# MIT-SPARK/Khronos

Hardware: AMD Instinct MI355X
Metric: active-window frames/sec (+ Mvoxel-updates/sec) at 1280x720 RGB-D+labels, 2 cm voxels (higher is better)
Workload: dtype f32

## Files before the change

khronos_amd/csrc/khr_device.h:

```cpp
#pragma once
#include <hip/hip_runtime.h>
#include <stdint.h>

namespace khr {

constexpr uint64_t kEmptyKey = ~0ull;
constexpr uint32_t kInvalidSlot = 0xffffffffu;

constexpr uint32_t BLK_UPDATED = 1u, BLK_MESH_UPDATED = 2u, BLK_TRACKING_UPDATED = 4u, BLK_HAS_ACTIVE = 8u,
                   BLK_LIVE = 16u,
                   BLK_TRACK_DIRTY = 32u,
                   BLK_ANY_KEEP = 64u,
                   BLK_HAS_NEG = 128u;
constexpr uint8_t VOX_ACTIVE = 1, VOX_EVER_FREE = 2, VOX_TO_REMOVE = 4, VOX_SEM_VALID = 8;
constexpr uint8_t VOX_OCC = 16;
constexpr uint8_t VOX_PUBLIC_MASK = 0x0f;

enum Counter : int {
  C_FREE_HEAD = 0,
  C_N_FREE,
  C_MAX_SLOT,
  C_N_VISIBLE,
  C_N_NEW,
  C_N_EF,
  C_N_LIVE,
  C_POOL_EXHAUSTED,
  C_N_UPD_LO,
  C_N_REMOVED,
  C_N_SEEDS,
  C_N_MESH,
  C_N_BAND,
  C_N_TSDF,
  C_BAND_OVERFLOW,
  C_TSDF_CURSOR,
  C_MESH_OVERFLOW,
  C_N_PROC,
  C_N_EF_A,
  C_N_PROC2,
  C_N_EF2,
  C_MP_DONE,
  C_N_ITEMS0,
  C_N_ITEMS1,
  C_N_ITEMS2,
  C_N_ITEMS3,
  C_COUNT = 32
};
enum Stat64 : int { S_UPD = 0 , S_BAND , S_MESH_VERTS, S_PRUNED, S_CUM_UPD, S_CUM_BAND, S_CUM_VISITED, S_CUM_CALLS, S_COUNT = 8 };

struct MeshDesc {
  uint32_t offset;
  uint32_t count;
};

struct DevMap {
  uint64_t* ht_keys;
  uint32_t* ht_vals;
  uint32_t ht_mask;
  uint32_t capacity;
  int4* blk_index;
  uint32_t* blk_flags;
  float* dist;
  float* weight;
  uint32_t* color;
  uint64_t* last_obs;
  ulonglong2* obs;
  uint64_t* last_occ;
  uint64_t* trk_lim;
  uint8_t* vflags;
  uint32_t* sem_label;
  float* lik;
  uint64_t* freebits;
  uint16_t* blk_band;
  uint32_t* free_slots;
  uint32_t* counters;
  unsigned long long* stats;
  MeshDesc* mesh_desc;
};

constexpr int kBandSlots = 32;
constexpr uint16_t kItemTouched = 0x8000u, kItemNeg = 0x4000u, kItemBandMask = 0x3fffu;
struct FuseList {
  uint4* a;
  uint4* b;
  uint32_t cap;
  uint32_t* counts;
};
__device__ inline uint32_t fuseClass(uint32_t band) { return band > 128u ? 0u : (band > 64u ? 1u : (band > 0u ? 2u : 3u)); }
__device__ inline uint4* fuseDescPtr(const FuseList& l, uint32_t cls, uint32_t pos) {
  uint4* const arr = cls < 2u ? l.a : l.b;
  return arr + ((cls & 1u) ? l.cap - 1u - pos : pos);
}

__host__ __device__ inline int likStride(int K) { return K <= 4 ? K : ((K + 31) & ~31); }

struct DevParams {
  float vs, vs_inv, bs, bs_inv, trunc;
  int vps, nvox, K;
  int KS;
  int with_semantics, with_tracking;
  int use_dropoff, const_weight, interp, range_mode, sem_mode;
  float dropoff_eps, max_weight, adaptive_diff, log_match, log_nomatch;
  float occ_thr;
  double temporal_buffer, temporal_window;
  int nn;
  float mesh_min_weight;
  float mesh_eps;
  int mesh_attr_source;
// ... 161 lines not shown
  if (slot != kInvalidSlot && ignore_epoch != 0 && m.blk_index[slot].w == ignore_epoch) slot = kInvalidSlot;
  if (slot == kInvalidSlot) return ~0ull;
  if (m.vflags[static_cast<size_t>(slot) * p.nvox + lin] & VOX_EVER_FREE) key |= kSeedFlag;
  return key;
}

__device__ inline uint64_t lastObserved(const DevMap& m, size_t slot, uint32_t lin, int nvox) {
  const ulonglong2 w = m.obs[slot * static_cast<size_t>(nvox >> 6) + (lin >> 6)];
  return ((w.x >> (lin & 63u)) & 1ull) ? w.y : m.last_obs[slot * static_cast<size_t>(nvox) + lin];
}

__device__ inline double toSeconds(uint64_t ns) { return static_cast<double>(ns) / 1e9; }

__device__ inline uint32_t laneId() { return __lane_id(); }

__device__ inline uint32_t waveAggInc(uint32_t* counter, bool pred) {
  const unsigned long long mask = __ballot(pred);
  if (mask == 0) return 0;
  const uint32_t lane = laneId();
  const uint32_t rank = __popcll(mask & ((1ull << lane) - 1ull));
  const int leader = __ffsll(static_cast<long long>(mask)) - 1;
  uint32_t base = 0;
  if (lane == static_cast<uint32_t>(leader)) base = atomicAdd(counter, static_cast<uint32_t>(__popcll(mask)));
  base = __shfl(base, leader);
  return base + rank;
}

__device__ inline uint8_t toU8(float f) {
  float r = floorf(f + 0.5f);
  r = fminf(255.f, fmaxf(0.f, r));
  return static_cast<uint8_t>(r);
}

__device__ inline void publishSeedCount(const DevMap& m, volatile uint32_t* host_seed, uint32_t ticket) {
  host_seed[0] = atomicAdd(&m.counters[C_N_SEEDS], 0u);
  __threadfence_system();
  host_seed[1] = ticket;
  __threadfence_system();
}

constexpr int kUpdateStatSlots = 2048;

__device__ inline void beginIntegrate(DevMap m, int nvox, uint32_t* wg_stats) {
  unsigned long long u = 0, b = 0;
  uint2* __restrict__ st = reinterpret_cast<uint2*>(wg_stats);
#pragma unroll 4
  for (int i = threadIdx.x; i < kUpdateStatSlots; i += blockDim.x) {
    const uint2 v = st[i];
    u += v.x;
    b += v.y;
    if (v.x | v.y) st[i] = make_uint2(0u, 0u);
  }
#pragma unroll
  for (int o = 32; o > 0; o >>= 1) {
    u += __shfl_down(u, o);
    b += __shfl_down(b, o);
  }
  if ((threadIdx.x & 63) == 0 && (u | b)) {
    atomicAdd(&m.stats[S_CUM_UPD], u);
    atomicAdd(&m.stats[S_CUM_BAND], b);
  }
  if (threadIdx.x == 0) {
    m.stats[S_CUM_VISITED] += static_cast<unsigned long long>(m.counters[C_N_VISIBLE]) * nvox;
    m.stats[S_CUM_CALLS] += 1ull;
    m.counters[C_N_VISIBLE] = 0u;
    m.counters[C_N_NEW] = 0u;
    m.counters[C_N_TSDF] = 0u;
    m.counters[C_N_ITEMS0] = 0u;
    m.counters[C_N_ITEMS1] = 0u;
    m.counters[C_N_ITEMS2] = 0u;
    m.counters[C_N_ITEMS3] = 0u;
  }
}

__device__ inline uint32_t ufLoad(const uint32_t* parent, uint32_t x) { return __atomic_load_n(parent + x, __ATOMIC_RELAXED); }
__device__ inline uint32_t ufFind(uint32_t* parent, uint32_t x) {
  uint32_t p = ufLoad(parent, x);
  while (p != x) {
    const uint32_t gp = ufLoad(parent, p);
    if (gp != p) atomicMin(parent + x, gp);
    x = p;
    p = gp;
  }
  return x;
}
__device__ inline uint32_t ufFind(const uint32_t* parent, uint32_t x) {
  while (true) {
    const uint32_t p = ufLoad(parent, x);
    if (p == x) return x;
    x = p;
  }
}
__device__ inline void ufUnion(uint32_t* parent, uint32_t a, uint32_t b) {
  a = ufFind(parent, a);
  b = ufFind(parent, b);
  while (a != b) {
    if (a < b) { const uint32_t t = a; a = b; b = t; }
    const uint32_t old = atomicCAS(parent + a, a, b);
    if (old == a) return;
    a = ufFind(parent, old);
  }
}

}
// ... 1 lines not shown
```

khronos_amd/csrc/khr_kernels_aux.h:

```cpp
#pragma once
#include <cstring>

#include "khr_device.h"

namespace khr {

#include "mc_table.inc"
__device__ int8_t g_mc_tri[256][16];
__device__ uint8_t g_mc_ntri[256];

constexpr uint64_t kSeedBit = kSeedFlag;

__global__ __launch_bounds__(256) void k_motion_pixels(DevMap m, DevParams p, DevFrame f, float md_max_range,
                                                      float min_z_world, uint64_t* __restrict__ keys, int ignore_epoch,
                                                      uint32_t* __restrict__ begin_band_count) {
  if (begin_band_count && blockIdx.x == 0) beginIntegrate(m, p.nvox, begin_band_count);
  const int i = blockIdx.x * blockDim.x + threadIdx.x;
  const bool in = i < f.W * f.H;
  uint64_t key = ~0ull;
  if (in)
    key = motionPixelKey(m, p, f.range[i], f.depth[i], i % f.W, i / f.W, f.fx, f.fy, f.cx, f.cy, f.Rw, f.tw, md_max_range,
                         min_z_world, ignore_epoch);
  if (in) keys[i] = key;
  const bool seed = (key != ~0ull) && (key & kSeedBit);
  const int any = __syncthreads_count(seed ? 1 : 0);
  if (any && threadIdx.x == 0) atomicAdd(&m.counters[C_N_SEEDS], static_cast<uint32_t>(any));
}

__global__ __launch_bounds__(1024) void k_publish(const uint32_t* __restrict__ src, volatile uint32_t* __restrict__ dst_host,
                                                 uint32_t rec_words, uint32_t max_recs, volatile uint32_t* __restrict__ ticket_host,
                                                 uint32_t ticket, uint32_t* __restrict__ counters_to_zero) {
  const uint32_t n_words = 4u + min(src[0], max_recs) * rec_words;
  for (uint32_t i = threadIdx.x; i < n_words; i += blockDim.x) dst_host[i] = src[i];
  __threadfence_system();
  __syncthreads();
  if (threadIdx.x < 4) counters_to_zero[threadIdx.x] = 0u;
  if (threadIdx.x == 0) {
    *ticket_host = ticket;
    __threadfence_system();
  }
}

__global__ void k_publish_seed(DevMap m, volatile uint32_t* host_seed, uint32_t ticket) {
  if (blockIdx.x == 0 && threadIdx.x == 0) publishSeedCount(m, host_seed, ticket);
}

__global__ __launch_bounds__(256) void k_md_keys_export(const uint64_t* __restrict__ keys, int n, uint64_t* __restrict__ out) {
  const int i = blockIdx.x * blockDim.x + threadIdx.x;
  if (i < n) out[i] = keys[i] == ~0ull ? 0ull : keys[i];
}
__global__ __launch_bounds__(256) void k_md_keys_import(const uint64_t* __restrict__ in, int n, uint64_t* __restrict__ keys,
                                                       uint32_t* __restrict__ n_seed_px) {
  const int i = blockIdx.x * blockDim.x + threadIdx.x;
  uint64_t k = ~0ull;
  if (i < n) {
    k = in[i] == 0ull ? ~0ull : in[i];
    keys[i] = k;
  }
  const unsigned long long b = __ballot(k != ~0ull && (k & kSeedBit));
  if (b && laneId() == static_cast<uint32_t>(__ffsll(static_cast<long long>(b)) - 1))
    atomicAdd(n_seed_px, static_cast<uint32_t>(__popcll(b)));
}

__global__ __launch_bounds__(256) void k_md_bits_export(const uint64_t* __restrict__ keys, int n, unsigned long long* __restrict__ bits) {
  const int i = blockIdx.x * blockDim.x + threadIdx.x;
  const uint64_t k = i < n ? keys[i] : ~0ull;
  const unsigned long long ex = __ballot(k != ~0ull), sd = __ballot(k != ~0ull && (k & kSeedBit));
  if (laneId() == 0 && (i & ~63) < n) {
    bits[2 * (i >> 6)] = ex;
    bits[2 * (i >> 6) + 1] = sd;
  }
}
__global__ __launch_bounds__(256) void k_md_keys_from_bits(DevParams p, DevFrame f, float md_max_range, float min_z_world,
                                                          const unsigned long long* __restrict__ bits, uint64_t* __restrict__ keys,
                                                          uint32_t* __restrict__ n_seed_px) {
  const int i = blockIdx.x * blockDim.x + threadIdx.x;
  const int n = f.W * f.H;
// ... 1456 lines not shown
}

__global__ __launch_bounds__(256) void k_rehash_clear(DevMap m) {
  if (m.counters[C_N_REMOVED] == 0u) return;
  const uint32_t i = blockIdx.x * blockDim.x + threadIdx.x;
  if (i <= m.ht_mask) m.ht_keys[i] = kEmptyKey;
  if (i == 0) {
    m.counters[C_N_FREE] = 0u;
    m.counters[C_FREE_HEAD] = 0u;
  }
}

__global__ __launch_bounds__(256) void k_rehash(DevMap m) {
  if (m.counters[C_N_REMOVED] == 0u) return;
  const uint32_t s = blockIdx.x * blockDim.x + threadIdx.x;
  const bool live = s < m.counters[C_MAX_SLOT] && (m.blk_flags[s] & BLK_LIVE);
  if (live) {
    const int4 bi = m.blk_index[s];
    htInsertUnique(m, packKey(bi.x, bi.y, bi.z), s);
  }
  const bool is_free = s < m.capacity && !live;
  const uint32_t idx = waveAggInc(&m.counters[C_N_FREE], is_free);
  if (is_free) m.free_slots[idx] = s;
}

__global__ __launch_bounds__(256) void k_reset_map(DevMap m) {
  const uint32_t i = blockIdx.x * blockDim.x + threadIdx.x;
  if (i <= m.ht_mask) m.ht_keys[i] = kEmptyKey;
  if (i < m.capacity) {
    m.blk_flags[i] = 0u;
    m.mesh_desc[i] = MeshDesc{0u, 0u};
    m.free_slots[i] = i;
  }
  if (i < C_COUNT) m.counters[i] = i == C_N_FREE ? m.capacity : 0u;
  if (i < S_COUNT) m.stats[i] = 0ull;
}

__global__ __launch_bounds__(256) void k_block_flag_op(DevMap m, uint32_t and_mask, uint32_t or_mask) {
  const uint32_t s = blockIdx.x * blockDim.x + threadIdx.x;
  if (s >= m.counters[C_MAX_SLOT]) return;
  const uint32_t fl = m.blk_flags[s];
  if (fl & BLK_LIVE) m.blk_flags[s] = (fl & and_mask) | or_mask;
}

struct PackOut {
  float* dist;
  float* weight;
  uint32_t* color;
  uint64_t* last_obs;
  uint8_t* vflags;
  uint32_t* sem_label;
  uint64_t* last_occ;
  float* lik;
  int K, KS;
  uint64_t track_stamp;
};
template <int VPS>
__global__ __launch_bounds__(256) void k_pack_blocks(DevMap m, const uint32_t* __restrict__ slots, int n, PackOut o) {
  constexpr int NV = VPS * VPS * VPS;
  for (int b = blockIdx.x; b < n; b += gridDim.x) {
    const size_t src = static_cast<size_t>(slots[b]) * NV, dst = static_cast<size_t>(b) * NV;
    auto copy16 = [&](const void* s, void* d, size_t bytes) {
      const uint4* s4 = reinterpret_cast<const uint4*>(s);
      uint4* d4 = reinterpret_cast<uint4*>(d);
      for (size_t i = threadIdx.x; i < bytes / 16; i += 256) d4[i] = s4[i];
    };
    if (o.dist) copy16(m.dist + src, o.dist + dst, NV * 4);
// ... 180 lines not shown
```

khronos_amd/csrc/khr_kernels_fusion.h:

```cpp
#pragma once
#include "khr_device.h"

namespace khr {


constexpr int kTile = 16;
constexpr int kMaxTick = 8;

__device__ inline void ingestTile(const float* __restrict__ depth_in, const uint8_t* __restrict__ rgb_in,
                                  const int32_t* __restrict__ label_in, float* __restrict__ depth, float* __restrict__ range,
                                  uint32_t* __restrict__ rgba, int32_t* __restrict__ label, int32_t* __restrict__ dyn,
                                  float* __restrict__ tile_max, int tile, int tw, int W, int H, float fx, float fy, float cx,
                                  float cy, int range_mode, float* d_out, float* r_out) {
  const int tx = tile % tw, ty = tile / tw;
  const int u = tx * kTile + (threadIdx.x & 15), v = ty * kTile + (threadIdx.x >> 4);
  float r = 0.f, d = 0.f;
  if (u < W && v < H) {
    const int i = v * W + u;
    d = depth_in[i];
    if (d > 0.f && isfinite(d)) {
      if (range_mode == 0) {
        r = d;
      } else {
        const float x = (static_cast<float>(u) - cx) / fx, y = (static_cast<float>(v) - cy) / fy;
        r = d * sqrtf((x * x + y * y) + 1.f);
      }
    }
    depth[i] = d;
    range[i] = r;
    dyn[i] = 0;
    if (rgb_in)
      rgba[i] = static_cast<uint32_t>(rgb_in[3 * i]) | (static_cast<uint32_t>(rgb_in[3 * i + 1]) << 8) |
                (static_cast<uint32_t>(rgb_in[3 * i + 2]) << 16) | 0xff000000u;
    if (label_in) label[i] = label_in[i];
  }
  *d_out = d;
  *r_out = r;
  float rm = r;
#pragma unroll
  for (int o = 32; o > 0; o >>= 1) rm = fmaxf(rm, __shfl_down(rm, o));
  __shared__ float s[4];
  if ((threadIdx.x & 63) == 0) s[threadIdx.x >> 6] = rm;
  __syncthreads();
  if (threadIdx.x == 0) tile_max[tile] = fmaxf(fmaxf(s[0], s[1]), fmaxf(s[2], s[3]));
}

__global__ __launch_bounds__(256) void k_frame_ingest(const float* __restrict__ depth_in,
                                                     const uint8_t* __restrict__ rgb_in,
                                                     const int32_t* __restrict__ label_in, float* __restrict__ depth,
                                                     float* __restrict__ range, uint32_t* __restrict__ rgba,
                                                     int32_t* __restrict__ label, int32_t* __restrict__ dyn,
                                                     float* __restrict__ tile_max, int tw, int W, int H, float fx,
                                                     float fy, float cx, float cy, int range_mode, DevMap m, int nvox,
                                                     uint32_t* __restrict__ wg_stats, int do_begin) {
  if (blockIdx.x == 0 && threadIdx.x == 0) m.counters[C_N_SEEDS] = 0u;
  if (do_begin && blockIdx.x == 0) beginIntegrate(m, nvox, wg_stats);
  float d, r;
  ingestTile(depth_in, rgb_in, label_in, depth, range, rgba, label, dyn, tile_max, blockIdx.x, tw, W, H, fx, fy, cx, cy,
             range_mode, &d, &r);
}

struct TickIngest {
  const float* depth_in[kMaxTick];
  const uint8_t* rgb_in[kMaxTick];
  const int32_t* label_in[kMaxTick];
  float* depth[kMaxTick];
  float* range[kMaxTick];
  uint32_t* rgba[kMaxTick];
  int32_t* label[kMaxTick];
  int32_t* dyn[kMaxTick];
  float* tile_max[kMaxTick];
  float Rw[kMaxTick][9], tw[kMaxTick][3], min_z_world[kMaxTick];
};
__global__ __launch_bounds__(256) void k_tick_ingest(TickIngest t, int tw, int W, int H, float fx, float fy, float cx, float cy,
                                                    int range_mode, DevMap m, DevParams p, float md_max_range, int count_seeds,
                                                    uint32_t* __restrict__ seed_counts) {
  const int cam = blockIdx.y;
  if (blockIdx.x == 0 && cam == 0 && threadIdx.x == 0) m.counters[C_N_SEEDS] = 0u;
  float d, r;
  ingestTile(t.depth_in[cam], t.rgb_in[cam], t.label_in[cam], t.depth[cam], t.range[cam], t.rgba[cam], t.label[cam], t.dyn[cam],
             t.tile_max[cam], blockIdx.x, tw, W, H, fx, fy, cx, cy, range_mode, &d, &r);
  if (!count_seeds) return;
  const int u = (blockIdx.x % tw) * kTile + (threadIdx.x & 15), v = (blockIdx.x / tw) * kTile + (threadIdx.x >> 4);
  bool seed = false;
  if (u < W && v < H) {
    const uint64_t key = motionPixelKey(m, p, r, d, u, v, fx, fy, cx, cy, t.Rw[cam], t.tw[cam], md_max_range, t.min_z_world[cam]);
    seed = key != ~0ull && (key & kSeedFlag);
  }
  const unsigned long long b = __ballot(seed);
// ... 66 lines not shown
    dst[i] = depth[i];
    dst[n4 + i] = range[i];
    dst[2 * n4 + i] = rgba ? rgba[i] : z;
    dst[3 * n4 + i] = label ? label[i] : z;
  }
}
__global__ __launch_bounds__(256) void k_rgba_to_rgb(const uint32_t* __restrict__ rgba, uint8_t* __restrict__ rgb, uint32_t n) {
  const uint32_t i = blockIdx.x * blockDim.x + threadIdx.x;
  if (i >= n) return;
  const uint32_t c = rgba[i];
  rgb[3 * i] = static_cast<uint8_t>(c);
  rgb[3 * i + 1] = static_cast<uint8_t>(c >> 8);
  rgb[3 * i + 2] = static_cast<uint8_t>(c >> 16);
}

__global__ __launch_bounds__(256) void k_vertex_map(DevFrame f, float* __restrict__ vertex) {
  const int i = blockIdx.x * blockDim.x + threadIdx.x;
  if (i >= f.W * f.H) return;
  float o[3] = {0.f, 0.f, 0.f};
  if (f.range[i] > 0.f) {
    const float d = f.depth[i];
    const int u = i % f.W, v = i / f.W;
    const float x = ((static_cast<float>(u) - f.cx) / f.fx) * d;
    const float y = ((static_cast<float>(v) - f.cy) / f.fy) * d;
    xform(f.Rw, f.tw, x, y, d, o);
  }
  vertex[3 * i] = o[0];
  vertex[3 * i + 1] = o[1];
  vertex[3 * i + 2] = o[2];
}

__global__ __launch_bounds__(256) void k_alloc_visible(DevMap m, DevParams p, DevFrame f, DevFrustum fr,
                                                      uint32_t* __restrict__ work, uint32_t* __restrict__ new_list,
                                                      volatile uint32_t* host_seed, uint32_t seed_ticket,
                                                      uint32_t* __restrict__ list_count, int epoch) {
  if (seed_ticket && blockIdx.x == 0 && threadIdx.x == 0) publishSeedCount(m, host_seed, seed_ticket);
  const int S = 2 * fr.n_steps + 1;
  const int total = S * S * S;
  const int i = blockIdx.x * blockDim.x + threadIdx.x;
  bool visible = false;
  int bx = 0, by = 0, bz = 0;
  if (i < total) {
    const int dx = i % S - fr.n_steps, dy = (i / S) % S - fr.n_steps, dz = i / (S * S) - fr.n_steps;
    bx = fr.bc.x + dx;
    by = fr.bc.y + dy;
    bz = fr.bc.z + dz;
    const bool in = blockIsCandidate(p, fr, f.R, f.t, f.max_range, bx, by, bz);
    visible = in && ownerOf(bx, by, bz, p.world) == p.rank;
  }
  uint32_t slot = kInvalidSlot;
  const uint64_t key = packKey(bx, by, bz);
  if (visible) slot = htLookup(m, key);
  const bool need = visible && slot == kInvalidSlot;
  const uint32_t fidx = waveAggInc(&m.counters[C_FREE_HEAD], need);
  bool got = false;
  if (need) {
    if (fidx < m.counters[C_N_FREE]) {
      slot = m.free_slots[fidx];
      got = true;
      m.blk_index[slot] = make_int4(bx, by, bz, epoch);
      m.blk_flags[slot] = BLK_LIVE | BLK_TRACK_DIRTY | BLK_ANY_KEEP;
      m.mesh_desc[slot] = MeshDesc{0u, 0u};
      htInsertUnique(m, key, slot);
      atomicMax(&m.counters[C_MAX_SLOT], slot + 1);
    } else {
      atomicAdd(&m.counters[C_POOL_EXHAUSTED], 1u);
      slot = kInvalidSlot;
    }
  }
  const uint32_t nidx = waveAggInc(&m.counters[C_N_NEW], got);
  if (got) new_list[nidx] = slot;
  const bool emit = visible && slot != kInvalidSlot;
  const uint32_t widx = waveAggInc(list_count, emit);
  if (emit) work[widx] = slot;
  if (list_count != &m.counters[C_N_VISIBLE]) waveAggInc(&m.counters[C_N_VISIBLE], emit);
}

struct TickFrusta {
  float R[kMaxTick][9], t[kMaxTick][3], max_range[kMaxTick];
  DevFrustum fr[kMaxTick];
};
constexpr int kTickAllocThreads = 1024;
__global__ __launch_bounds__(kTickAllocThreads) void k_tick_alloc(DevMap m, DevParams p, TickFrusta tf, int ncam, int3 lo, int3 dim,
                                                   uint32_t* __restrict__ work, uint32_t list_stride,
                                                   uint32_t* __restrict__ new_list, uint32_t* __restrict__ tick_counts, int epoch) {
  const int total = dim.x * dim.y * dim.z;
  const int i = blockIdx.x * blockDim.x + threadIdx.x;
  uint32_t seen = 0u;
  int bx = 0, by = 0, bz = 0;
  if (i < total) {
    bx = lo.x + i % dim.x;
    by = lo.y + (i / dim.x) % dim.y;
    bz = lo.z + i / (dim.x * dim.y);
    if (ownerOf(bx, by, bz, p.world) == p.rank) {
      for (int k = 0; k < ncam; ++k) {
        const DevFrustum& fr = tf.fr[k];
        if (abs(bx - fr.bc.x) > fr.n_steps || abs(by - fr.bc.y) > fr.n_steps || abs(bz - fr.bc.z) > fr.n_steps) continue;
        const bool in = blockIsCandidate(p, fr, tf.R[k], tf.t[k], tf.max_range[k], bx, by, bz);
        if (in) seen |= 1u << k;
      }
    }
  }
  const bool visible = seen != 0u;
  uint32_t slot = kInvalidSlot;
  const uint64_t key = packKey(bx, by, bz);
  if (visible) slot = htLookup(m, key);
  const bool need = visible && slot == kInvalidSlot;
  const uint32_t fidx = waveAggInc(&m.counters[C_FREE_HEAD], need);
  bool got = false;
  if (need) {
    if (fidx < m.counters[C_N_FREE]) {
      slot = m.free_slots[fidx];
      got = true;
      m.blk_index[slot] = make_int4(bx, by, bz, epoch);
      m.blk_flags[slot] = BLK_LIVE | BLK_TRACK_DIRTY | BLK_ANY_KEEP;
      m.mesh_desc[slot] = MeshDesc{0u, 0u};
      htInsertUnique(m, key, slot);
      atomicMax(&m.counters[C_MAX_SLOT], slot + 1);
    } else {
      atomicAdd(&m.counters[C_POOL_EXHAUSTED], 1u);
      slot = kInvalidSlot;
    }
  }
  const uint32_t nidx = waveAggInc(&m.counters[C_N_NEW], got);
  if (got) new_list[nidx] = slot;
  if (slot == kInvalidSlot) seen = 0u;
  __shared__ uint32_t s_cnt[kMaxTick], s_base[kMaxTick];
  if (threadIdx.x < kMaxTick) s_cnt[threadIdx.x] = 0u;
  __syncthreads();
  uint32_t loff[kMaxTick];
#pragma unroll
  for (int k = 0; k < kMaxTick; ++k) {
    loff[k] = 0u;
    if (k < ncam) loff[k] = waveAggInc(&s_cnt[k], ((seen >> k) & 1u) != 0u);
  }
  __syncthreads();
  if (threadIdx.x < static_cast<uint32_t>(ncam)) {
    const uint32_t n = s_cnt[threadIdx.x];
    s_base[threadIdx.x] = n ? atomicAdd(&tick_counts[2 * threadIdx.x], n) : 0u;
  }
  if (threadIdx.x == 64) {
    uint32_t tot = 0u;
    for (int k = 0; k < ncam; ++k) tot += s_cnt[k];
    if (tot) atomicAdd(&m.counters[C_N_VISIBLE], tot);
  }
  __syncthreads();
#pragma unroll
  for (int k = 0; k < kMaxTick; ++k)
    if (k < ncam && ((seen >> k) & 1u)) work[static_cast<size_t>(k) * list_stride + s_base[k] + loff[k]] = slot;
}

__global__ void k_begin_integrate(DevMap m, int nvox, uint32_t* wg_stats) {
  if (blockIdx.x == 0) beginIntegrate(m, nvox, wg_stats);
}
__global__ void k_tick_begin(DevMap m, int nvox, uint32_t* wg_stats, uint32_t* tick_counts, uint32_t extra_calls) {
  beginIntegrate(m, nvox, wg_stats);
  if (threadIdx.x < 6 * kMaxTick) tick_counts[threadIdx.x] = 0u;
  if (threadIdx.x == 0) m.stats[S_CUM_CALLS] += extra_calls;
}

__device__ inline void cullBlocks(const DevMap& m, const DevParams& p, const DevFrame& f, const uint32_t* __restrict__ work,
                                  const uint32_t* __restrict__ n_work, FuseList out, uint32_t wpb,
                                  uint32_t* __restrict__ n_tsdf, const float* __restrict__ tile_max, int tw, int th,
                                  uint32_t bid, uint32_t nblk, uint32_t* __restrict__ item_mask = nullptr, uint32_t cam = 0u) {
  constexpr int kPerWg = 8;
  __shared__ uint4 s_blk[kPerWg];
  __shared__ uint16_t s_item[4][kPerWg * kBandSlots];
  __shared__ uint32_t s_nkeep, s_ccnt[4], s_off[4];
  const uint32_t n = *n_work;
  const uint32_t lane = threadIdx.x & 63;
  for (uint32_t base = bid * kPerWg; base < n; base += nblk * kPerWg) {
  if (threadIdx.x == 0) s_nkeep = 0;
  if (threadIdx.x < 4) s_ccnt[threadIdx.x] = 0;
  __syncthreads();
  for (uint32_t wi = base + (threadIdx.x >> 6); wi < min(n, base + kPerWg); wi += 4) {
    const uint32_t slot = work[wi];
    const int4 bi = m.blk_index[slot];
// ... 102 lines not shown
      }
      if (ikeep && sub == 0 && item_mask) {
        const size_t mi = static_cast<size_t>(slot) * wpb + item;
        const uint32_t sh = 8u * static_cast<uint32_t>(mi & 3);
        const uint32_t old = atomicOr(&item_mask[mi >> 2], (1u << cam) << sh);
        if ((old >> sh) & 0xffu) ikeep = false;
      }
      if (ikeep && sub == 0) {
        const uint32_t cls = fuseClass(m.blk_band[static_cast<size_t>(slot) * kBandSlots + item] & kItemBandMask);
        s_item[cls][atomicAdd(&s_ccnt[cls], 1u)] = static_cast<uint16_t>((kslot << 8) | item);
      }
    }
  }
  __syncthreads();
  if (threadIdx.x < 4) s_off[threadIdx.x] = s_ccnt[threadIdx.x] ? atomicAdd(&out.counts[threadIdx.x], s_ccnt[threadIdx.x]) : 0u;
  if (threadIdx.x == 0 && s_nkeep) atomicAdd(n_tsdf, s_nkeep);
  __syncthreads();
#pragma unroll
  for (uint32_t cls = 0; cls < 4; ++cls) {
    for (uint32_t i = threadIdx.x; i < s_ccnt[cls]; i += blockDim.x) {
      const uint32_t it = s_item[cls][i];
      uint4 d = s_blk[it >> 8];
      d.x |= (it & 0xffu) << 24;
      *fuseDescPtr(out, cls, s_off[cls] + i) = d;
    }
  }
  __syncthreads();
  }
}

__global__ __launch_bounds__(256) void k_cull_blocks(DevMap m, DevParams p, DevFrame f,
                                                    const uint32_t* __restrict__ work, FuseList out, uint32_t wpb,
                                                    const float* __restrict__ tile_max, int tw, int th) {
  cullBlocks(m, p, f, work, &m.counters[C_N_VISIBLE], out, wpb, &m.counters[C_N_TSDF], tile_max, tw, th, blockIdx.x, gridDim.x);
}

struct TickFrames {
  DevFrame f[kMaxTick];
  const float* tile_max[kMaxTick];
};
__global__ __launch_bounds__(256) void k_tick_cull(DevMap m, DevParams p, TickFrames t, const uint32_t* __restrict__ work,
                                                  uint32_t list_stride, uint4* __restrict__ desc, uint32_t desc_stride, uint32_t wpb,
                                                  uint32_t* __restrict__ tick_counts, int use_tiles, int tw, int th,
                                                  uint32_t* __restrict__ item_mask) {
  const int cam = blockIdx.y;
  const int lc = item_mask ? 0 : cam;
  FuseList out{desc + static_cast<size_t>(2 * lc) * desc_stride, desc + static_cast<size_t>(2 * lc + 1) * desc_stride, desc_stride,
               &tick_counts[2 * kMaxTick + 4 * lc]};
  cullBlocks(m, p, t.f[cam], work + static_cast<size_t>(cam) * list_stride, &tick_counts[2 * cam], out, wpb, &tick_counts[2 * cam + 1],
             use_tiles ? t.tile_max[cam] : nullptr, tw, th, blockIdx.x, gridDim.x, item_mask, static_cast<uint32_t>(cam));
}

__global__ __launch_bounds__(256) void k_alloc_list(DevMap m, const int* __restrict__ idx, int n,
                                                   uint32_t* __restrict__ new_list) {
  const int i = blockIdx.x * blockDim.x + threadIdx.x;
  bool need = false;
  int bx = 0, by = 0, bz = 0;
  if (i < n) {
    bx = idx[3 * i];
    by = idx[3 * i + 1];
    bz = idx[3 * i + 2];
    need = htLookup(m, packKey(bx, by, bz)) == kInvalidSlot;
  }
  const uint32_t fidx = waveAggInc(&m.counters[C_FREE_HEAD], need);
  bool got = false;
  uint32_t slot = kInvalidSlot;
  if (need) {
    if (fidx < m.counters[C_N_FREE]) {
      slot = m.free_slots[fidx];
      got = true;
      m.blk_index[slot] = make_int4(bx, by, bz, 0);
      m.blk_flags[slot] = BLK_LIVE | BLK_TRACK_DIRTY | BLK_ANY_KEEP;
      m.mesh_desc[slot] = MeshDesc{0u, 0u};
      htInsertUnique(m, packKey(bx, by, bz), slot);
      atomicMax(&m.counters[C_MAX_SLOT], slot + 1);
    } else {
      atomicAdd(&m.counters[C_POOL_EXHAUSTED], 1u);
    }
  }
  const uint32_t nidx = waveAggInc(&m.counters[C_N_NEW], got);
  if (got) new_list[nidx] = slot;
}

__global__ __launch_bounds__(256) void k_list_live(DevMap m, uint32_t* __restrict__ work, uint32_t* counter,
                                                  uint32_t require_flags, FuseList out = FuseList{nullptr, nullptr, 0u, nullptr},
                                                  uint32_t wpb = 0u) {
  const uint32_t s = blockIdx.x * blockDim.x + threadIdx.x;
  bool live = false;
  if (s < m.counters[C_MAX_SLOT]) {
    const uint32_t fl = m.blk_flags[s];
    live = (fl & BLK_LIVE) && ((fl & require_flags) == require_flags);
  }
  const uint32_t idx = waveAggInc(counter, live);
  if (live) work[idx] = s;
  if (out.a) {
    const unsigned long long mask = __ballot(live);
    if (mask) {
      const uint32_t lane = laneId();
      const int leader = __ffsll(static_cast<long long>(mask)) - 1;
      uint32_t base = 0;
      if (lane == static_cast<uint32_t>(leader)) base = atomicAdd(&out.counts[3], static_cast<uint32_t>(__popcll(mask)) * wpb);
      base = __shfl(base, leader) + static_cast<uint32_t>(__popcll(mask & ((1ull << lane) - 1ull))) * wpb;
      if (live) {
        const int4 bi = m.blk_index[s];
        for (uint32_t it = 0; it < wpb; ++it)
          *fuseDescPtr(out, 3u, base + it) =
              make_uint4(s | (it << 24), static_cast<uint32_t>(bi.x), static_cast<uint32_t>(bi.y), static_cast<uint32_t>(bi.z));
      }
    }
  }
}

__device__ inline void initBlocks(const DevMap& m, const DevParams& p, const uint32_t* __restrict__ new_list, uint32_t bid,
                                  uint32_t nblk) {
  const uint32_t n = m.counters[C_N_NEW];
  const int nv = p.nvox;
  for (uint32_t b = bid; b < n; b += nblk) {
    const size_t slot = new_list[b];
    const uint4 z = make_uint4(0, 0, 0, 0);
    uint4* d4 = reinterpret_cast<uint4*>(m.dist + slot * nv);
    uint4* w4 = reinterpret_cast<uint4*>(m.weight + slot * nv);
    uint4* c4 = reinterpret_cast<uint4*>(m.color + slot * nv);
    uint4* l4 = reinterpret_cast<uint4*>(m.sem_label + slot * nv);
    for (int i = threadIdx.x; i < nv / 4; i += blockDim.x) {
      d4[i] = z;
      w4[i] = z;
      c4[i] = z;
      if (p.with_semantics) l4[i] = z;
    }
    uint4* f4 = reinterpret_cast<uint4*>(m.vflags + slot * nv);
    for (int i = threadIdx.x; i < nv / 16; i += blockDim.x) f4[i] = z;
    if (threadIdx.x < kBandSlots) m.blk_band[slot * kBandSlots + threadIdx.x] = 0;
    if (p.with_tracking) {
      uint4* o4 = reinterpret_cast<uint4*>(m.last_obs + slot * nv);
      uint4* q4 = reinterpret_cast<uint4*>(m.last_occ + slot * nv);
      for (int i = threadIdx.x; i < nv / 2; i += blockDim.x) {
        o4[i] = z;
        q4[i] = z;
      }
      uint64_t* fb = m.freebits + slot * (nv / 64);
      for (int i = threadIdx.x; i < nv / 64; i += blockDim.x) {
        fb[i] = 0ull;
        m.obs[slot * (nv / 64) + i] = make_ulonglong2(0ull, 0ull);
      }
    }
  }
}

__global__ __launch_bounds__(256) void k_init_blocks(DevMap m, DevParams p, const uint32_t* __restrict__ new_list) {
  initBlocks(m, p, new_list, blockIdx.x, gridDim.x);
}

__global__ __launch_bounds__(256) void k_init_cull(DevMap m, DevParams p, DevFrame f, const uint32_t* __restrict__ new_list,
                                                  const uint32_t* __restrict__ work, FuseList out, uint32_t wpb,
                                                  const float* __restrict__ tile_max, int tw, int th, uint32_t n_cull) {
  if (blockIdx.x < n_cull)
    cullBlocks(m, p, f, work, &m.counters[C_N_VISIBLE], out, wpb, &m.counters[C_N_TSDF], tile_max, tw, th, blockIdx.x, n_cull);
  else
    initBlocks(m, p, new_list, blockIdx.x - n_cull, gridDim.x - n_cull);
}

__device__ inline uint32_t foldItemRecords(uint32_t* __restrict__ blk_flags, uint16_t* __restrict__ blk_band, uint32_t s) {
  static_assert(kBandSlots == 32, "record row = 4 x 16 bytes");
  uint4* const row = reinterpret_cast<uint4*>(blk_band + static_cast<size_t>(s) * kBandSlots);
  uint32_t any = 0u;
  uint4 r[4];
#pragma unroll
  for (int i = 0; i < 4; ++i) {
    r[i] = row[i];
    any |= r[i].x | r[i].y | r[i].z | r[i].w;
  }
  const uint32_t tm = static_cast<uint32_t>(kItemTouched) * 0x00010001u, nm = static_cast<uint32_t>(kItemNeg) * 0x00010001u;
  uint32_t fl = blk_flags[s];
  if ((any & tm) == 0u) return fl;
  fl |= BLK_UPDATED | BLK_MESH_UPDATED | BLK_TRACKING_UPDATED | ((any & nm) ? BLK_HAS_NEG : 0u);
  blk_flags[s] = fl;
  const uint32_t keep = static_cast<uint32_t>(kItemBandMask) * 0x00010001u;
#pragma unroll
  for (int i = 0; i < 4; ++i) row[i] = make_uint4(r[i].x & keep, r[i].y & keep, r[i].z & keep, r[i].w & keep);
  return fl;
}
__global__ __launch_bounds__(256) void k_tracking_select(DevMap m, uint64_t lim_active, uint64_t lim_free, int force_full,
                                                        uint32_t* __restrict__ proc, uint32_t* __restrict__ ef_list,
                                                        uint32_t* __restrict__ cnt ,
                                                        uint32_t* __restrict__ cnt_next, uint16_t* __restrict__ fold_band) {
  const uint32_t s = blockIdx.x * blockDim.x + threadIdx.x;
  if (s == 0) { cnt_next[0] = 0u; cnt_next[1] = 0u; }
  bool need = false, touched = false, reload = false;
  if (s < m.counters[C_MAX_SLOT]) {
    const uint32_t fl = fold_band ? foldItemRecords(m.blk_flags, fold_band, s) : m.blk_flags[s];
// ... 163 lines not shown

__constant__ int8_t c_nbr26[26][3] = {
    {-1, 0, 0}, {1, 0, 0}, {0, -1, 0}, {0, 1, 0}, {0, 0, -1}, {0, 0, 1},
    {-1, -1, 0}, {-1, 1, 0}, {1, -1, 0}, {1, 1, 0}, {-1, 0, -1}, {-1, 0, 1}, {1, 0, -1}, {1, 0, 1},
    {0, -1, -1}, {0, -1, 1}, {0, 1, -1}, {0, 1, 1},
    {-1, -1, -1}, {-1, -1, 1}, {-1, 1, -1}, {-1, 1, 1}, {1, -1, -1}, {1, -1, 1}, {1, 1, -1}, {1, 1, 1}};

constexpr int kHaloRecWords = 66;

struct RemoteHalo {
  const uint64_t* recs;
  const uint64_t* ht_keys;
  const uint32_t* ht_vals;
  uint32_t ht_mask;
};

template <int VPS>
__global__ __launch_bounds__(256) void k_ever_free(DevMap m, DevParams p, const uint32_t* __restrict__ ef_list,
                                                  const uint32_t* __restrict__ ef_count, RemoteHalo rh) {
  constexpr int NV = VPS * VPS * VPS;
  constexpr int NW = NV / 64;
  constexpr int T = VPS + 2;
  __shared__ uint32_t s_row[T * T];
  __shared__ uint64_t s_bits[27][NW];
  __shared__ const uint64_t* s_src[27];
  const uint32_t n = *ef_count;
  for (uint32_t b = blockIdx.x; b < n; b += gridDim.x) {
    const size_t slot = ef_list[b];
    const int4 bi = m.blk_index[slot];
    __syncthreads();
    if (threadIdx.x < 27) {
      const int dx = threadIdx.x % 3 - 1, dy = (threadIdx.x / 3) % 3 - 1, dz = threadIdx.x / 9 - 1;
      const uint64_t key = packKey(bi.x + dx, bi.y + dy, bi.z + dz);
      const uint32_t ns = (threadIdx.x == 13) ? static_cast<uint32_t>(slot) : htLookup(m, key);
      const uint64_t* src = nullptr;
      if (ns != kInvalidSlot) {
        src = m.freebits + static_cast<size_t>(ns) * NW;
      } else if (rh.recs) {
        uint32_t h = hashKey(key) & rh.ht_mask;
        while (true) {
          const uint64_t k = rh.ht_keys[h];
          if (k == key) {
            src = rh.recs + static_cast<size_t>(rh.ht_vals[h]) * kHaloRecWords + 2;
            break;
          }
          if (k == kEmptyKey) break;
          h = (h + 1) & rh.ht_mask;
        }
      }
      s_src[threadIdx.x] = src;
    }
    __syncthreads();
    for (int i = threadIdx.x; i < 27 * NW; i += 256) {
      const uint64_t* src = s_src[i / NW];
      s_bits[i / NW][i % NW] = src ? src[i % NW] : 0ull;
    }
    __syncthreads();
    for (int r = threadIdx.x; r < T * T; r += 256) {
      const int ty = r % T, tz = r / T;
      int y = ty - 1, z = tz - 1, sy = 1, sz = 1;
      if (y < 0) { y += VPS; sy = 0; } else if (y >= VPS) { y -= VPS; sy = 2; }
      if (z < 0) { z += VPS; sz = 0; } else if (z >= VPS) { z -= VPS; sz = 2; }
      const int lin0 = VPS * (y + VPS * z);
      const uint32_t mid = static_cast<uint32_t>((s_bits[1 + 3 * sy + 9 * sz][lin0 >> 6] >> (lin0 & 63)) & ((1u << VPS) - 1u));
      const uint32_t left = static_cast<uint32_t>((s_bits[0 + 3 * sy + 9 * sz][(lin0 + VPS - 1) >> 6] >> ((lin0 + VPS - 1) & 63)) & 1u);
      const uint32_t right = static_cast<uint32_t>((s_bits[2 + 3 * sy + 9 * sz][lin0 >> 6] >> (lin0 & 63)) & 1u);
      s_row[r] = left | (mid << 1) | (right << (VPS + 1));
// ... 90 lines not shown
```

khronos_amd/csrc/khronos_amd.hip:

```cpp
#include <hip/hip_runtime.h>
#include <hip/hip_ext.h>
#include <hipcub/hipcub.hpp>

#include <algorithm>
#include <array>
#include <atomic>
#include <chrono>
#include <memory>
#include <mutex>
#include <cmath>
#include <cstdarg>
#include <cstdio>
#include <climits>
#include <cstring>
#include <cstdlib>
#include <functional>
#include <map>
#include <string>
#include <thread>
#include <tuple>
#include <unordered_map>
#include <vector>

#include "../../include/khronos_amd.h"
// ... 59 lines not shown
  uint64_t aux_seq = 0;
  std::vector<khr_cluster> sem_clusters;
  std::vector<khr_cluster> clusters;
};

struct TimingRec {
  int which;
  hipEvent_t a, b;
};

constexpr int kNumTimers = 13;
constexpr uint32_t kObjHead = 512;
constexpr uint32_t kCvHead = 8192;
constexpr uint32_t kCompCap = 1024, kCompHead = 64;

}

struct khr_ctx {
  khr_config cfg{};
  DevParams p{};
  DevMap m{};
  int device = 0;
  hipStream_t stream = nullptr;
  bool own_stream = false;
  hipStream_t aux_stream = nullptr;
  hipEvent_t ev_aux = nullptr, ev_aux_done = nullptr;
  uint64_t aux_seq_issued = 0, aux_seq_done = 0, obj_seq = 0, cv_seq[2] = {0, 0};
  std::vector<void*> allocs;
  std::vector<FrameSlot> slots;
  int next_slot = 0;
  std::unique_ptr<std::atomic<int>[]> slot_leases;
  uint32_t* d_work = nullptr;
  uint32_t* d_new = nullptr;
  uint32_t* d_ef = nullptr;
  uint32_t* d_trk_proc = nullptr;
  uint32_t* d_tick_work = nullptr;
  uint32_t* d_tick_counts = nullptr;
  uint32_t* d_tick_seeds = nullptr;
  uint32_t* h_tick = nullptr;
  uint32_t* d_tick_host = nullptr;
  uint32_t tick_ticket = 0;
  std::vector<uint32_t> tick_seed_host;
  int tick_seed_n = 0, tick_seed_collected = 0;
  int tick_epoch = 0, motion_ignore_epoch = 0;
  unsigned long long* d_dbg = nullptr;
  unsigned long long* d_digest = nullptr;
  uint32_t* d_wg_stats = nullptr;
  bool defer_fold = false, fold_pending = false;
  int stream_priority = 0;
  unsigned char* d_fuse_sink = nullptr;
  uint32_t* d_pix_scratch = nullptr;
  size_t pix_words = 0;
  uint8_t* d_inst = nullptr;
  size_t inst_bytes = 0;
  uint4* d_work4 = nullptr;
  uint4* d_tick_work4 = nullptr;
  FuseFrame* d_tick_frames = nullptr;
  uint32_t* d_tick_mask = nullptr;
  bool tick_mask_dirty = false;
  uint32_t item_cap = 0;
  struct SnapArena { uint8_t* ptr; size_t bytes; volatile uint32_t* h_count; uint32_t* d_count_host_view; };
  struct SnapPool {
    std::mutex mu;
    std::vector<SnapArena> free;
    bool dead = false;
  };
// ... 11 lines not shown
  hipEvent_t ev_snap_fork = nullptr, ev_snap_join = nullptr;
  hipStream_t mc_stream = nullptr;
  hipEvent_t ev_mc_fork = nullptr, ev_mc_join = nullptr;
  bool fork_after_select = false;
  uint64_t explicit_blocks = 0;
  uint4* d_multi_list = nullptr;
  uint32_t* d_frame_bits = nullptr;
  size_t frame_bits_words = 0;
  FuseFrame* h_frames = nullptr;
  FuseFrame* d_frames = nullptr;
  hipEvent_t ev_frames = nullptr;
  uint32_t snap_ticket = 0;
  uint32_t wpb = 0;
  int fuse_zsplit = 2;
  uint64_t* d_halo_recs = nullptr;
  const uint64_t* halo_view = nullptr;
  uint64_t* d_halo_keys = nullptr;
  uint32_t* d_halo_vals = nullptr;
  uint32_t halo_cap_total = 0, halo_recs_cap = 0, halo_mask = 0, halo_n = 0;
  uint32_t* d_mh_recs = nullptr;
  const uint32_t* mh_view = nullptr;
  uint64_t* d_mh_keys = nullptr;
  uint32_t* d_mh_vals = nullptr;
  uint32_t mh_cap_total = 0, mh_mask = 0, mh_n = 0;
  uint8_t* d_mh_flag = nullptr;
  uint32_t* d_mh2_scratch = nullptr;
  uint64_t* d_mh2_keys = nullptr;
  uint32_t* d_mh2_offs = nullptr;
  uint32_t mh2_ht = 0;
  bool mh_compact = false;
  uint32_t* h_pinned = nullptr;
  uint32_t* d_pinned = nullptr;
  uint32_t seed_ticket = 0;
  bool seed_publish_pending = false;
  bool seed_by_ticket = false;
  bool begin_in_ingest = false, begun = false;
  uint32_t fetch_ticket = 0;
  bool fetch_pending = false;
  uint32_t* d_fetch_done = nullptr;
  std::vector<uint32_t> fm_order;
  size_t fm_total = 0;
  uint64_t map_gen = 1, counters_gen = 0;
  int last_frame_slot = -1;
  void* h_stage = nullptr;
  size_t h_stage_bytes = 0;
  uint32_t* h_totals = nullptr;
  void* h_up = nullptr;
  size_t h_up_bytes = 0;
  hipEvent_t ev_ingest = nullptr;
  hipEvent_t ev_up = nullptr;
  hipStream_t ingest_stream = nullptr;
  struct AheadEntry { int slot; int ev; bool host; };
  std::vector<AheadEntry> ahead_q;
  hipEvent_t ev_ahead[2] = {nullptr, nullptr};
  hipEvent_t ev_ahead_h2d[2] = {nullptr, nullptr};
  int ahead_ev_next = 0;
  hipEvent_t* h2d_ev_target = nullptr;
  hipStream_t h2d_stream = nullptr;
  hipEvent_t ev_h2d = nullptr;
  bool h2d_pending = false;
  bool host_input_pinned = false;
  uint64_t h2d_bytes = 0;
  int ef_parity = 0, ef_cur = 0;
  hipEvent_t ev_seed = nullptr;
  uint32_t last_removed = 0;
  khr_ctx* dep_src = nullptr;
  hipEvent_t ev_dep = nullptr, ev_dep_aux = nullptr;
  uint64_t last_track_stamp = 0;
  bool removed_pending = false;
// ... 92 lines not shown
  uint32_t* d_slice_count = nullptr;
  uint8_t* d_slice_stage = nullptr;
  uint8_t* h_slice_stage = nullptr;
  uint32_t slice_cap = 0, slice_hint = 0;
  unsigned long long* d_render_stats = nullptr;
  uint8_t* d_render_stage = nullptr;
  uint8_t* h_render_stage = nullptr;
  size_t render_stage_bytes = 0;
  unsigned long long* d_query_stats = nullptr;
  uint8_t* d_query_stage = nullptr;
  uint8_t* h_query_stage = nullptr;
  size_t query_stage_bytes = 0;
  uint8_t* d_ckpt[2] = {nullptr, nullptr};
  uint8_t* h_ckpt[2] = {nullptr, nullptr};
  size_t ckpt_stage_bytes = 0;
  uint32_t* d_ckpt_slots[2] = {nullptr, nullptr};
  uint32_t ckpt_slots_cap = 0;
  uint32_t* d_ckpt_err = nullptr;
  hipEvent_t ev_ckpt_filled[2] = {nullptr, nullptr}, ev_ckpt_drained[2] = {nullptr, nullptr};
  uint32_t timing = 0;
  std::vector<TimingRec> pending;
  std::vector<hipEvent_t> event_pool;
  double t_ms[kNumTimers] = {0};
  uint64_t t_n[kNumTimers] = {0};
};

namespace {

struct ScopedTimer {
  khr_ctx* c;
  int which;
  hipEvent_t a = nullptr, b = nullptr;
  bool on = false;
  ScopedTimer(khr_ctx* ctx, int w) : c(ctx), which(w) {
    on = w >= 0 && ((c->timing >> w) & 1u);
    if (on) {
      auto get = [&]() {
        hipEvent_t e = nullptr;
        if (!c->event_pool.empty()) {
          e = c->event_pool.back();
          c->event_pool.pop_back();
        } else {
          hipEventCreate(&e);
        }
        return e;
      };
      a = get();
      b = get();
      hipEventRecord(a, c->stream);
    }
  }
  ~ScopedTimer() {
    if (on) {
      hipEventRecord(b, c->stream);
      c->pending.push_back({which, a, b});
    }
  }
};

hipEvent_t takeEvent(khr_ctx* c) {
  hipEvent_t e = nullptr;
  if (!c->event_pool.empty()) {
    e = c->event_pool.back();
    c->event_pool.pop_back();
  } else {
    hipEventCreate(&e);
  }
  return e;
}
#define KHR_LAUNCH_TIMED_ON(which, strm, kernel, grid, block, ...)                                     \
  do {                                                                                                 \
    if ((c->timing >> (which)) & 1u) {                                                                 \
      hipEvent_t ev_a = takeEvent(c), ev_b = takeEvent(c);                                             \
      hipExtLaunchKernelGGL(kernel, grid, block, 0, strm, ev_a, ev_b, 0, __VA_ARGS__);                 \
      c->pending.push_back({(which), ev_a, ev_b});                                                     \
    } else {                                                                                           \
      hipLaunchKernelGGL(kernel, grid, block, 0, strm, __VA_ARGS__);                                   \
    }                                                                                                  \
  } while (0)
#define KHR_LAUNCH_TIMED(which, kernel, grid, block, ...) KHR_LAUNCH_TIMED_ON(which, c->stream, kernel, grid, block, __VA_ARGS__)

void resolveTimers(khr_ctx* c) {
  for (auto& r : c->pending) {
    hipEventSynchronize(r.b);
    float ms = 0.f;
    hipEventElapsedTime(&ms, r.a, r.b);
    if (r.which >= 0) {
// ... 76 lines not shown
  return f;
}

DevFrustum makeFrustum(const khr_ctx* c, const DevFrame& f) {
  DevFrustum fr{};
  const float xl = (0.f - f.cx) / f.fx, xr = (static_cast<float>(f.W) - f.cx) / f.fx;
  const float yt = (0.f - f.cy) / f.fy, yb = (static_cast<float>(f.H) - f.cy) / f.fy;
  const float tl[3] = {xl, yt, 1.f}, tr[3] = {xr, yt, 1.f}, bl[3] = {xl, yb, 1.f}, br[3] = {xr, yb, 1.f};
  crossn(bl, tl, fr.n[0]);
  crossn(tr, br, fr.n[1]);
  crossn(tl, tr, fr.n[2]);
  crossn(br, bl, fr.n[3]);
  fr.infl = 0.8660254f * c->p.bs;
  fr.n_steps = static_cast<int>(std::ceil(f.max_range * c->p.bs_inv)) + 1;
  fr.max_steps = static_cast<int>(std::floor((f.max_range + fr.infl) * c->p.bs_inv));
  for (int a = 0; a < 3; ++a) fr.tw[a] = f.tw[a];
  fr.bc = make_int3(static_cast<int>(std::floor(f.tw[0] * c->p.bs_inv)),
                    static_cast<int>(std::floor(f.tw[1] * c->p.bs_inv)),
                    static_cast<int>(std::floor(f.tw[2] * c->p.bs_inv)));
  return fr;
}

int ensureStage(khr_ctx* c, size_t bytes) {
  if (bytes <= c->h_stage_bytes) return KHR_OK;
  if (c->h_stage) HIP_TRY(hipHostFree(c->h_stage));
  c->h_stage = nullptr;
  c->h_stage_bytes = 0;
  const size_t want = std::max<size_t>(bytes + bytes / 2, 1u << 20);
  if (hipHostMalloc(&c->h_stage, want, hipHostMallocDefault) != hipSuccess) return fail(KHR_ENOMEM, "pinned staging of %zu bytes", want);
  c->h_stage_bytes = want;
  return KHR_OK;
}

int readCounters(khr_ctx* c) {
  c->h_counters.resize(C_COUNT);
  HIP_TRY(hipMemcpyAsync(c->h_counters.data(), c->m.counters, sizeof(uint32_t) * C_COUNT, hipMemcpyDeviceToHost,
                         c->stream));
  HIP_TRY(hipStreamSynchronize(c->stream));
  return KHR_OK;
}

int ensureHostIndex(khr_ctx* c) {
  if (c->host_index_valid) return KHR_OK;
  int rc = readCounters(c);
  if (rc) return rc;
  const uint32_t n = c->h_counters[C_MAX_SLOT];
  std::vector<int4> idx(n);
  c->host_flags.resize(n);
  if (n) {
    HIP_TRY(hipMemcpyAsync(idx.data(), c->m.blk_index, sizeof(int4) * n, hipMemcpyDeviceToHost, c->stream));
    HIP_TRY(hipMemcpyAsync(c->host_flags.data(), c->m.blk_flags, sizeof(uint32_t) * n, hipMemcpyDeviceToHost,
                           c->stream));
    HIP_TRY(hipStreamSynchronize(c->stream));
  }
  c->host_index.clear();
  for (uint32_t s = 0; s < n; ++s)
    if (c->host_flags[s] & BLK_LIVE) c->host_index[{idx[s].x, idx[s].y, idx[s].z}] = s;
  c->host_index_valid = true;
  return KHR_OK;
}

inline int gridFor(size_t n, int block = 256) { return static_cast<int>((n + block - 1) / block); }

template <typename F>
int dispatchVps(khr_ctx* c, F&& f) {
  if (c->cfg.voxels_per_side == 16) return f(std::integral_constant<int, 16>());
  if (c->cfg.voxels_per_side == 8) return f(std::integral_constant<int, 8>());
  return fail(KHR_EINVAL, "voxels_per_side must be 8 or 16");
}

constexpr int kUpdateWavesPerCu = 16;
// ... 270 lines not shown
  p.rank = cfg->rank;
  p.world = cfg->world_size;
  p.dbg = std::getenv("KHR_DEBUG") ? std::atoi(std::getenv("KHR_DEBUG")) : 0;

  DevMap& m = c->m;
  const size_t cap = cfg->max_blocks, nv = p.nvox;
  uint32_t ht = 1;
  while (ht < cap * 4) ht <<= 1;
  m.ht_mask = ht - 1;
  m.capacity = static_cast<uint32_t>(cap);
  int rc = KHR_OK;
  auto A = [&](int r) { if (rc == KHR_OK) rc = r; };
  A(devAlloc(c, &m.ht_keys, ht, false));
  A(devAlloc(c, &m.ht_vals, ht));
  A(devAlloc(c, &m.blk_index, cap));
  A(devAlloc(c, &m.blk_flags, cap));
  A(devAlloc(c, &m.dist, cap * nv, false));
  A(devAlloc(c, &m.weight, cap * nv, false));
  A(devAlloc(c, &m.color, cap * nv, false));
  A(devAlloc(c, &m.vflags, cap * nv, false));
  A(devAlloc(c, &m.sem_label, cfg->with_semantics ? cap * nv : 1, false));
  if (devAlloc(c, &m.lik, cfg->with_semantics ? cap * nv * p.KS : 1, false) != KHR_OK) {
    fail(KHR_ENOMEM, "the label-likelihood layer of %zu blocks needs %.2f GB (%d floats per voxel%s); khr_config.packed_likelihood_rows = 1 "
                     "stores %d per voxel, a smaller max_blocks less of everything", static_cast<size_t>(cap),
         1e-9 * static_cast<double>(cap) * nv * p.KS * 4, p.KS, p.KS != p.K ? ": rows padded to 128-byte lines" : "", p.K);
    A(KHR_ENOMEM);
  }
  A(devAlloc(c, &m.last_obs, cfg->with_tracking ? cap * nv : 1, false));
  A(devAlloc(c, &m.last_occ, cfg->with_tracking ? cap * nv : 1, false));
  A(devAlloc(c, &m.trk_lim, cfg->with_tracking ? cap * 2 : 2));
  A(devAlloc(c, &m.freebits, cfg->with_tracking ? cap * (nv / 64) : 1, false));
  A(devAlloc(c, &m.obs, cfg->with_tracking ? cap * (nv / 64) : 1, false));
  A(devAlloc(c, &m.free_slots, cap, false));
  A(devAlloc(c, &m.counters, C_COUNT));
  A(devAlloc(c, &m.stats, S_COUNT));
  A(devAlloc(c, &m.mesh_desc, cap));
  A(devAlloc(c, &c->d_work, cap));
  A(devAlloc(c, &c->d_new, cap));
  A(devAlloc(c, &c->d_ef, cap));
  A(devAlloc(c, &c->d_trk_proc, cap));
  A(devAlloc(c, &c->d_dbg, 4096 * 4 * 12));
  A(devAlloc(c, &c->d_digest, kDigestWords));
  A(devAlloc(c, &c->d_wg_stats, 2 * kUpdateStatSlots));
  A(devAlloc(c, &c->d_fuse_sink, static_cast<size_t>(kUpdateStatSlots) * 16 * 256, false));
  A(devAlloc(c, &c->d_fetch_done, 4));
  {
    const int zs = (cfg->voxels_per_side != 8 && (cfg->world_size >= 4 || cfg->max_frame_pixels <= 640u * 480u)) ? 8 : 4;
    c->fuse_zsplit = zs;
    c->wpb = static_cast<uint32_t>((cfg->voxels_per_side * cfg->voxels_per_side / 64) * zs);
    c->item_cap = static_cast<uint32_t>(cap) * c->wpb;
  }
  A(devAlloc(c, &c->d_work4, 2 * static_cast<size_t>(c->item_cap), false));
  if (cfg->voxels_per_side == 8 && rc == KHR_OK) {
    const size_t bits_words = static_cast<size_t>(c->item_cap) * 4;
    if (hipHostMalloc(reinterpret_cast<void**>(&c->h_frames), sizeof(FuseFrame) * kMaxMultiFrames, hipHostMallocDefault) != hipSuccess ||
        hipMalloc(reinterpret_cast<void**>(&c->d_frames), sizeof(FuseFrame) * kMaxMultiFrames) != hipSuccess ||
        hipEventCreateWithFlags(&c->ev_frames, hipEventDisableTiming) != hipSuccess ||
        hipEventRecord(c->ev_frames, c->stream) != hipSuccess ||
        hipMalloc(reinterpret_cast<void**>(&c->d_frame_bits), bits_words * sizeof(uint32_t)) != hipSuccess ||
        hipMalloc(reinterpret_cast<void**>(&c->d_multi_list), sizeof(uint4) * 2 * c->item_cap + 16) != hipSuccess)
      rc = fail(KHR_ENOMEM, "buffers of the multi-frame update");
    else
      c->frame_bits_words = bits_words;
    if (rc == KHR_OK && (hipHostMalloc(reinterpret_cast<void**>(&c->h_totals), sizeof(uint32_t) * (C_COUNT + 2), hipHostMallocDefault) != hipSuccess ||
                         hipEventCreateWithFlags(&c->ev_up, hipEventDisableTiming) != hipSuccess || hipEventRecord(c->ev_up, c->stream) != hipSuccess ||
                         hipEventCreateWithFlags(&c->ev_dep, hipEventDisableTiming) != hipSuccess ||
                         hipEventCreateWithFlags(&c->ev_dep_aux, hipEventDisableTiming) != hipSuccess))
      rc = fail(KHR_ENOMEM, "page-locked words / events of an object mini-map");
  }
  A(devAlloc(c, &m.blk_band, cap * kBandSlots));
  A(devAlloc(c, &c->d_removed, cap));
  A(devAlloc(c, &c->d_mesh_count, cap + 1));
  A(devAlloc(c, &c->d_mesh_offset, cap + 1));
  A(devAlloc(c, &c->d_regen, cap));
  A(devAlloc(c, &c->d_mesh_old_off, cap + 1));
  A(devAlloc(c, &c->d_mh_flag, cap));
  A(devAlloc(c, &c->d_mesh_nwork, 8));
  const size_t npx = cfg->max_frame_pixels;
  A(devAlloc(c, &c->d_keys, npx, false));
  A(devAlloc(c, &c->d_pix, npx, false));
  {
    uint32_t ts = 1;
    while (ts < 2 * npx) ts <<= 1;
    c->md_mask = ts - 1;
    c->md_list_cap = static_cast<uint32_t>(std::min<size_t>(npx, 1u << 20));
    A(devAlloc(c, &c->d_md_keys, 3 * static_cast<size_t>(ts), false));
    A(devAlloc(c, &c->d_md_counts, 3 * static_cast<size_t>(ts), false));
    A(devAlloc(c, &c->d_md_ids, 3 * static_cast<size_t>(ts), false));
    {
      uint8_t* head = nullptr;
      A(devAlloc(c, &head, 16 + sizeof(CompAcc) * kCompCap));
      c->d_md_n = reinterpret_cast<uint32_t*>(head);
    }
    A(devAlloc(c, &c->d_md_parent, c->md_list_cap, false));
    A(devAlloc(c, &c->d_md_rootidx, c->md_list_cap, false));
    A(devAlloc(c, &c->d_md_edges, c->md_list_cap, false));
    A(devAlloc(c, &c->d_md_comp_acc, c->md_list_cap, false));
// ... 159 lines not shown
    c->snap_pool->free.clear();
  }
  {
    std::lock_guard<std::mutex> lock(c->frame_pool->mu);
    c->frame_pool->dead = true;
    for (auto& b : c->frame_pool->free) hipFree(b.first);
    c->frame_pool->free.clear();
  }
  if (c->d_frame_bits) hipFree(c->d_frame_bits);
  if (c->d_multi_list) hipFree(c->d_multi_list);
  if (c->h_frames) hipHostFree(c->h_frames);
  if (c->d_frames) hipFree(c->d_frames);
  if (c->ev_frames) hipEventDestroy(c->ev_frames);
  if (c->h_pinned) hipHostFree(c->h_pinned);
  if (c->h_removed_early) hipHostFree(c->h_removed_early);
  if (c->h_stage) hipHostFree(c->h_stage);
  if (c->h_totals) hipHostFree(c->h_totals);
  if (c->h_up) hipHostFree(c->h_up);
  if (c->ev_up) hipEventDestroy(c->ev_up);
  if (c->ev_ingest) hipEventDestroy(c->ev_ingest);
  if (c->h_tick) hipHostFree(c->h_tick);
  if (c->h_obj_head) hipHostFree(c->h_obj_head);
  if (c->h_md_acc_pinned) hipHostFree(c->h_md_acc_pinned);
  if (c->ev_obj) hipEventDestroy(c->ev_obj);
  for (int w = 0; w < 2; ++w) {
    if (c->h_cv[w]) hipHostFree(c->h_cv[w]);
    if (c->ev_cv[w]) hipEventDestroy(c->ev_cv[w]);
  }
  if (c->ev_seed) hipEventDestroy(c->ev_seed);
  if (c->ev_dep) hipEventDestroy(c->ev_dep);
  if (c->ev_dep_aux) hipEventDestroy(c->ev_dep_aux);
  if (c->ev_aux) hipEventDestroy(c->ev_aux);
  if (c->ev_aux_done) hipEventDestroy(c->ev_aux_done);
  if (c->aux_stream) hipStreamDestroy(c->aux_stream);
  if (c->own_stream && c->stream) hipStreamDestroy(c->stream);
  delete c;
}

int khr_set_stream(khr_ctx* c, void* hip_stream) {
  if (!c) return fail(KHR_EINVAL, "null ctx");
  HIP_TRY(hipStreamSynchronize(c->stream));
  HIP_TRY(hipStreamSynchronize(c->aux_stream));
  if (c->own_stream) {
    hipStreamDestroy(c->stream);
    c->own_stream = false;
  }
  if (hip_stream) {
    c->stream = static_cast<hipStream_t>(hip_stream);
  } else {
    HIP_TRY(createStream(c, &c->stream));
    c->own_stream = true;
  }
  return KHR_OK;
}

int khr_sync(khr_ctx* c) {
  if (!c) return fail(KHR_EINVAL, "null ctx");
  HIP_TRY(hipStreamSynchronize(c->stream));
  HIP_TRY(hipStreamSynchronize(c->aux_stream));
  return KHR_OK;
}

static int auxAfterMain(khr_ctx* c) {
  HIP_TRY(hipEventRecord(c->ev_aux, c->stream));
  HIP_TRY(hipStreamWaitEvent(c->aux_stream, c->ev_aux, 0));
  return KHR_OK;
// ... 63 lines not shown
    if (pinned) {
      if (!c->h2d_stream) HIP_TRY(createStream(c, &c->h2d_stream));
      hipEvent_t& evh0 = c->h2d_ev_target ? *c->h2d_ev_target : c->ev_h2d;
      if (!evh0) HIP_TRY(hipEventCreateWithFlags(&evh0, hipEventDisableTiming));
      cs = c->h2d_stream;
      if (ist == c->stream) {
        if (!c->ev_ingest) HIP_TRY(hipEventCreateWithFlags(&c->ev_ingest, hipEventDisableTiming));
        HIP_TRY(hipEventRecord(c->ev_ingest, c->stream));
        HIP_TRY(hipStreamWaitEvent(cs, c->ev_ingest, 0));
      }
    }
    HIP_TRY(hipMemcpyAsync(s.depth, frame->depth, n * sizeof(float), kind, cs));
    depth_src = s.depth;
    if (frame->color) {
      HIP_TRY(hipMemcpyAsync(s.rgb_staging, frame->color, n * 3, kind, cs));
      rgb_src = s.rgb_staging;
    }
    if (frame->label) {
      HIP_TRY(hipMemcpyAsync(s.label, frame->label, n * sizeof(int32_t), kind, cs));
      label_src = s.label;
    }
    if (pinned) {
      hipEvent_t& evh = c->h2d_ev_target ? *c->h2d_ev_target : c->ev_h2d;
      HIP_TRY(hipEventRecord(evh, cs));
      HIP_TRY(hipStreamWaitEvent(ist, evh, 0));
      if (!c->h2d_ev_target) c->h2d_pending = true;
      c->h2d_bytes += n * (4u + (frame->color ? 3u : 0u) + (frame->label ? 4u : 0u));
    }
  }
  s.tw = (sensor->width + kTile - 1) / kTile;
  s.th = (sensor->height + kTile - 1) / kTile;
  hipLaunchKernelGGL(k_frame_ingest, dim3(s.tw * s.th), dim3(256), 0, ist, depth_src, rgb_src, label_src, s.depth,
                     s.range, s.rgba, s.label, s.dyn, s.tile_max, s.tw, sensor->width, sensor->height, sensor->fx, sensor->fy,
                     sensor->cx, sensor->cy, c->p.range_mode, c->m, c->p.nvox, c->d_wg_stats, c->begin_in_ingest ? 1 : 0);
  HIP_TRY(hipGetLastError());
  c->begun = c->begin_in_ingest;
  c->begin_in_ingest = false;
  if (!on_device && !pinned) HIP_TRY(hipStreamSynchronize(c->stream));
  s.valid = true;
  s.dyn_clean = true, s.dynw_valid = false;
  return slot;
}

int khr_set_frame_image(khr_ctx* c, int slot, int which, const int32_t* image, int on_device) {
  if (!c || slot < 0 || slot >= static_cast<int>(c->slots.size()) || !c->slots[slot].valid) return fail(KHR_EINVAL, "bad slot");
  FrameSlot& s = c->slots[slot];
  const size_t n = static_cast<size_t>(s.sensor.width) * s.sensor.height;
  int32_t* dst = which == 0 ? s.dyn : s.obj;
  if (image) {
    HIP_TRY(hipMemcpyAsync(dst, image, n * sizeof(int32_t), on_device ? hipMemcpyDeviceToDevice : hipMemcpyHostToDevice, c->stream));
    if (!on_device) HIP_TRY(hipStreamSynchronize(c->stream));
  } else {
    HIP_TRY(hipMemsetAsync(dst, 0, n * sizeof(int32_t), c->stream));
  }
  if (which == 1) s.has_obj = image != nullptr;
  if (which == 0) s.dyn_clean = image == nullptr;
  if (which == 0) s.dynw_valid = false;
  if (which == 1) {
    const int rca = auxAfterMain(c);
    if (rca) return rca;
  }
  return KHR_OK;
}

int khr_download_frame(khr_ctx* c, int slot, float* range, float* vertex_map, int32_t* dynamic_image) {
  if (!c || slot < 0 || slot >= static_cast<int>(c->slots.size()) || !c->slots[slot].valid) return fail(KHR_EINVAL, "bad slot");
  FrameSlot& s = c->slots[slot];
  const size_t n = static_cast<size_t>(s.sensor.width) * s.sensor.height;
  if (range) HIP_TRY(hipMemcpyAsync(range, s.vRange(), n * sizeof(float), hipMemcpyDeviceToHost, c->stream));
// ... 111 lines not shown
int khr_copy_frame_image(khr_ctx* c, int slot, int which, void* device_dst) {
  if (!c || !device_dst || slot < 0 || slot >= static_cast<int>(c->slots.size()) || !c->slots[slot].valid) return fail(KHR_EINVAL, "bad argument");
  if (which != 0 && which != 1) return fail(KHR_EINVAL, "which must be 0 (dynamic) or 1 (object)");
  HIP_TRY(hipSetDevice(c->device));
  FrameSlot& s = c->slots[slot];
  const size_t n = static_cast<size_t>(s.sensor.width) * s.sensor.height;
  if (which == 1 && !s.has_obj) {
    HIP_TRY(hipMemsetAsync(device_dst, 0, n * sizeof(int32_t), c->stream));
    return KHR_OK;
  }
  if (which == 1) {
    HIP_TRY(hipEventRecord(c->ev_aux_done, c->aux_stream));
    HIP_TRY(hipStreamWaitEvent(c->stream, c->ev_aux_done, 0));
  }
  HIP_TRY(hipMemcpyAsync(device_dst, which == 0 ? s.dyn : s.obj, n * sizeof(int32_t), hipMemcpyDeviceToDevice, c->stream));
  return KHR_OK;
}

int khr_download_frame_image(khr_ctx* c, int slot, int which, int32_t* image) {
  if (!c || !image || slot < 0 || slot >= static_cast<int>(c->slots.size()) || !c->slots[slot].valid) return fail(KHR_EINVAL, "bad argument");
  if (which != 0 && which != 1) return fail(KHR_EINVAL, "which must be 0 (dynamic) or 1 (object)");
  FrameSlot& s = c->slots[slot];
  const size_t n = static_cast<size_t>(s.sensor.width) * s.sensor.height;
  if (which == 1 && !s.has_obj) {
    std::memset(image, 0, n * sizeof(int32_t));
    return KHR_OK;
  }
  if (which == 1) HIP_TRY(hipStreamSynchronize(c->aux_stream));
  HIP_TRY(hipMemcpyAsync(image, which == 0 ? s.dyn : s.obj, n * sizeof(int32_t), hipMemcpyDeviceToHost, c->stream));
  HIP_TRY(hipStreamSynchronize(c->stream));
  return KHR_OK;
}

static int integrateAlloc(khr_ctx* c, FrameSlot& s, const DevFrame& f, int allocate_blocks) {
  DevMap& m = c->m;
  if (!c->begun) hipLaunchKernelGGL(k_begin_integrate, dim3(1), dim3(256), 0, c->stream, m, c->p.nvox, c->d_wg_stats);
  c->begun = false;
  if (allocate_blocks) {
    ScopedTimer tm(c, 3);
    const DevFrustum fr = makeFrustum(c, f);
    const int S = 2 * fr.n_steps + 1;
    const size_t total = static_cast<size_t>(S) * S * S;
    hipLaunchKernelGGL(k_alloc_visible, dim3(gridFor(total)), dim3(256), 0, c->stream, m, c->p, f, fr, c->d_work, c->d_new,
                       c->d_pinned + 2, c->seed_publish_pending ? c->seed_ticket : 0u, &m.counters[C_N_VISIBLE], 0);
    c->seed_publish_pending = false;
    hipLaunchKernelGGL(k_init_cull, dim3(1024 + 1024), dim3(256), 0, c->stream, m, c->p, f, c->d_new, c->d_work,
                       FuseList{c->d_work4, c->d_work4 + c->item_cap, c->item_cap, &m.counters[C_N_ITEMS0]}, c->wpb,
                       c->cfg.disable_culling ? nullptr : s.vTileMax(), s.tw, s.th, 1024u);
    c->host_index_valid = false, ++c->map_gen;
  } else {
    hipLaunchKernelGGL(k_list_live, dim3(gridFor(m.capacity)), dim3(256), 0, c->stream, m, c->d_work,
                       &m.counters[C_N_VISIBLE], 0u, FuseList{c->d_work4, c->d_work4 + c->item_cap, c->item_cap, &m.counters[C_N_ITEMS0]},
                       c->wpb);
  }
  HIP_TRY(hipGetLastError());
  return KHR_OK;
}

struct UpdateLists {
  FuseList list{nullptr, nullptr, 0u, nullptr};
};

static int fuseGrid(khr_ctx* c, const void* kernel, int group, int block) {
  static std::map<std::pair<int, const void*>, int> cache;
  static std::mutex cache_mu;
  std::lock_guard<std::mutex> lock(cache_mu);
  const std::pair<int, const void*> key{c->device, kernel};
  auto it = cache.find(key);
  if (it != cache.end()) return it->second;
  int per_cu = 0, cus = 256;
  if (hipOccupancyMaxActiveBlocksPerMultiprocessor(&per_cu, kernel, block, 0) != hipSuccess || per_cu < 1) per_cu = 1;
  per_cu = std::min(per_cu, std::max(1, kUpdateWavesPerCu / (block / 64)));
  hipDeviceProp_t prop;
  if (hipGetDeviceProperties(&prop, c->device) == hipSuccess && prop.multiProcessorCount > 0) cus = prop.multiProcessorCount;
  per_cu = std::min(per_cu, 8);
  int grid = std::min(kUpdateStatSlots, per_cu * cus);
  grid = std::max(8 * group, grid / (8 * group) * (8 * group));
  cache[key] = grid;
  return grid;
}

static int fuse2Grid(khr_ctx* c, const void* kern, int wpw) {
  static std::map<std::pair<int, const void*>, int> cache;
  static std::mutex mu;
  std::lock_guard<std::mutex> lock(mu);
// ... 61 lines not shown
  {
    void* hf_dev = nullptr;
    HIP_TRY(hipHostGetDevicePointer(&hf_dev, c->h_frames, 0));
    const uint32_t n_words = static_cast<uint32_t>(sizeof(FuseFrame) / 4) * static_cast<uint32_t>(n_frames);
    hipLaunchKernelGGL(k_copy_words, dim3((n_words + 255) / 256), dim3(256), 0, c->stream, static_cast<const uint32_t*>(hf_dev),
                       reinterpret_cast<uint32_t*>(c->d_frames), n_words);
  }
  HIP_TRY(hipEventRecord(c->ev_frames, c->stream));
  static_cast<FuseFrame&>(a) = c->h_frames[0];
  a.frames = c->d_frames;
  a.n_frames = n_frames;
  if (c->item_cap > 0) {
    const int n_words = (n_frames + 31) / 32;
    const size_t need = static_cast<size_t>(c->item_cap) * static_cast<size_t>(n_words);
    if (need > c->frame_bits_words) {
      const size_t want = static_cast<size_t>(c->item_cap) * static_cast<size_t>((n_words + 3) / 4 * 4);
      HIP_TRY(hipStreamSynchronize(c->stream));
      if (c->d_frame_bits) HIP_TRY(hipFree(c->d_frame_bits));
      c->d_frame_bits = nullptr;
      c->frame_bits_words = 0;
      if (hipMalloc(reinterpret_cast<void**>(&c->d_frame_bits), want * sizeof(uint32_t)) != hipSuccess)
        return fail(KHR_ENOMEM, "frame bits of the multi-frame update (%zu bytes)", want * sizeof(uint32_t));
      c->frame_bits_words = want;
    }
    const uint64_t tests = static_cast<uint64_t>(c->explicit_blocks > 0 ? std::min<uint64_t>(c->explicit_blocks, c->m.capacity) : c->m.capacity) *
                           c->wpb * static_cast<uint64_t>(n_words) * 32u;
    const unsigned grid = static_cast<unsigned>(std::min<uint64_t>((tests + 255) / 256, 8192));
    hipLaunchKernelGGL((k_multi_cull<8>), dim3(std::max(1u, grid)), dim3(256), 0, c->stream, c->m.blk_flags, c->m.blk_index, &c->m.counters[C_MAX_SLOT],
                       c->p.vs, c->p.bs, c->p.trunc, static_cast<const FuseFrame*>(c->d_frames), n_frames, n_words, c->wpb, BLK_LIVE, c->d_frame_bits);
    HIP_TRY(hipGetLastError());
    a.frame_bits = c->d_frame_bits;
    a.frame_words = n_words;
  }
  FuseList list{c->d_work4, c->d_work4 + c->item_cap, c->item_cap, &c->m.counters[C_N_ITEMS0]};
  if (a.frame_bits != nullptr) {
    if (!c->d_multi_list) {
      HIP_TRY(hipStreamSynchronize(c->stream));
      if (hipMalloc(reinterpret_cast<void**>(&c->d_multi_list), sizeof(uint4) * 2 * c->item_cap + 16) != hipSuccess)
        return fail(KHR_ENOMEM, "item list of the multi-frame update");
    }
    uint32_t* const counts = reinterpret_cast<uint32_t*>(c->d_multi_list + 2 * static_cast<size_t>(c->item_cap));
    HIP_TRY(hipMemsetAsync(counts, 0, 16, c->stream));
    list = FuseList{c->d_multi_list, c->d_multi_list + c->item_cap, c->item_cap, counts};
    const uint64_t n_it = static_cast<uint64_t>(c->explicit_blocks > 0 ? std::min<uint64_t>(c->explicit_blocks, c->m.capacity) : c->m.capacity) * c->wpb;
    hipLaunchKernelGGL(k_multi_order, dim3(static_cast<unsigned>((n_it + 1023) / 1024)), dim3(1024), 0, c->stream, c->m.blk_flags, c->m.blk_index,
                       &c->m.counters[C_MAX_SLOT], static_cast<const uint32_t*>(c->d_frame_bits), a.frame_words, n_frames, c->wpb, BLK_LIVE, list);
    HIP_TRY(hipGetLastError());
  }
  constexpr int WPW = 8;
  auto go = [&](auto kern) {
    static std::map<std::pair<int, const void*>, std::pair<int, int>> per_cu_of;
    static std::mutex per_cu_mu;
    int per_cu = 0, cus = 256;
    {
      std::lock_guard<std::mutex> lock(per_cu_mu);
      const std::pair<int, const void*> key{c->device, reinterpret_cast<const void*>(kern)};
      auto it = per_cu_of.find(key);
      if (it != per_cu_of.end()) {
        per_cu = it->second.first;
        cus = it->second.second;
      } else {
        if (hipOccupancyMaxActiveBlocksPerMultiprocessor(&per_cu, kern, 64 * WPW, 0) != hipSuccess || per_cu < 1) per_cu = 1;
        hipDeviceProp_t prop;
        if (hipGetDeviceProperties(&prop, c->device) == hipSuccess && prop.multiProcessorCount > 0) cus = prop.multiProcessorCount;
        per_cu_of[key] = {per_cu, cus};
      }
    }
    int grid = std::min(kUpdateStatSlots, per_cu * cus) / 8 * 8;
    if (c->explicit_blocks > 0) {
      const uint64_t items = c->explicit_blocks * c->wpb;
      grid = std::max(8, static_cast<int>(std::min<uint64_t>(static_cast<uint64_t>(grid), (items + WPW - 1) / WPW) + 7) / 8 * 8);
    }
    for (int k0 = 0; k0 < n_frames; k0 += kMultiChunk) {
      a.frames = c->d_frames + k0;
      a.n_frames = std::min(kMultiChunk, n_frames - k0);
      a.frame_bit0 = k0;
      KHR_LAUNCH_TIMED(0, kern, dim3(grid), dim3(64 * WPW), a, list);
    }
  };
  if (exactArithmetic(c)) go(&k_fuse2<8, 4, true, true, WPW, 4>);
  else go(&k_fuse2<8, 4, true, false, WPW, 4>);
  HIP_TRY(hipGetLastError());
  return KHR_OK;
}

static int integrateUpdate(khr_ctx* c, FrameSlot& s, const DevFrame& f, int allocate_blocks, int use_mask,
                           int object_id, const UpdateLists* lists = nullptr, const uint32_t* gate = nullptr) {
  DevMap& m = c->m;
  FuseList list{c->d_work4, c->d_work4 + c->item_cap, c->item_cap, &m.counters[C_N_ITEMS0]};
  if (lists) list = lists->list;
  FuseArgs a{};
  fillFuseMap(c, &a);
  fillFuseFrame(c, s, f, use_mask, object_id, &a);
  const bool defcfg = a.range_mode == 0 && a.interp == 2 && a.use_dropoff && !a.const_weight;
  const bool exact = exactArithmetic(c);
  int rc = dispatchVps(c, [&](auto vps) {
    constexpr int V = decltype(vps)::value;
    auto launch = [&](auto zsplit) {
      constexpr int ZS = decltype(zsplit)::value;
      constexpr int G = 1;
      auto go = [&](auto kern, int wpw) {
        int grid = fuseGrid(c, reinterpret_cast<const void*>(kern), G, 64 * wpw);
        if (!allocate_blocks && c->explicit_blocks > 0) {
          const uint64_t items = c->explicit_blocks * c->wpb;
          const int want = static_cast<int>(std::min<uint64_t>(static_cast<uint64_t>(grid), (items + wpw - 1) / wpw));
          grid = std::max(8, (want + 7) / 8 * 8);
        }
        static bool said = false;
        if (!said && std::getenv("KHR_VERBOSE")) { said = true; std::fprintf(stderr, "[khr] k_fuse<%d,%d> %d waves / workgroup, grid %d\n", V, ZS, wpw, grid); }
        KHR_LAUNCH_TIMED(0, kern, dim3(grid), dim3(64 * wpw), a, list);
        if (c->defer_fold) c->fold_pending = true;
        else hipLaunchKernelGGL(k_fuse_fold, dim3((c->m.capacity + 255) / 256), dim3(256), 0, c->stream, m.blk_flags, m.blk_band,
                                &m.counters[C_MAX_SLOT], gate);
      };
      a.gate = gate;
      constexpr int WD = kUpdateWpw;
      if (defcfg && !exact) {
        go(&k_fuse<V, ZS, true, false, WD>, WD);
      } else if (defcfg) {
        go(&k_fuse<V, ZS, true, true, WD>, WD);
      } else {
        go(&k_fuse<V, ZS, false, true, WD>, WD);
// ... 446 lines not shown
  HIP_TRY(hipGetLastError());
  return KHR_OK;
}

int khr_tick_integrate(khr_ctx* c, const int* slots, int n_frames, int use_mask, int object_id, int phases) {
  if (!c || !slots || n_frames < 1 || (phases & 15) == 0) return fail(KHR_EINVAL, "bad argument");
  if (phases & 1) phases |= 12;
  if ((phases & 14) != 14 && n_frames > kMaxTick) return fail(KHR_EINVAL, "split phases take at most %d frames", kMaxTick);
  for (int i = 0; i < n_frames; ++i) {
    if (slots[i] < 0 || slots[i] >= static_cast<int>(c->slots.size()) || !c->slots[slots[i]].valid) return fail(KHR_EINVAL, "bad slot");
    const khr_sensor &a = c->slots[slots[i]].sensor, &b = c->slots[slots[0]].sensor;
    if (a.width != b.width || a.height != b.height) return fail(KHR_EINVAL, "the frames of a tick must come from sensors of one image size");
  }
  HIP_TRY(hipSetDevice(c->device));
  int rc = ensureTick(c);
  if (rc) return rc;
  DevMap& m = c->m;
  const uint32_t cap = m.capacity;
  const bool one_launch = tickUnion(c);
  for (int base = 0; base < n_frames; base += kMaxTick) {
    const int nb = std::min(kMaxTick, n_frames - base);
    TickFrames t{};
    for (int k = 0; k < nb; ++k) {
      FrameSlot& s = c->slots[slots[base + k]];
      t.f[k] = makeDevFrame(c, s);
      t.tile_max[k] = s.vTileMax();
    }
    if (phases & 4) {
      if (++c->tick_epoch <= 0) c->tick_epoch = 1;
      c->motion_ignore_epoch = c->tick_epoch;
      if (std::getenv("KHR_DEBUG_TICK_NO_EPOCH")) c->motion_ignore_epoch = 0;
      hipLaunchKernelGGL(k_tick_begin, dim3(1), dim3(256), 0, c->stream, m, c->p.nvox, c->d_wg_stats, c->d_tick_counts,
                         static_cast<uint32_t>(nb - 1));
      c->begun = false;
      ScopedTimer tm(c, 3);
      TickFrusta tf{};
      int lo[3] = {INT_MAX, INT_MAX, INT_MAX}, hi[3] = {INT_MIN, INT_MIN, INT_MIN};
      size_t cubes = 0;
      for (int k = 0; k < nb; ++k) {
        const DevFrustum fr = makeFrustum(c, t.f[k]);
        tf.fr[k] = fr;
        std::memcpy(tf.R[k], t.f[k].R, sizeof(tf.R[k]));
        std::memcpy(tf.t[k], t.f[k].t, sizeof(tf.t[k]));
        tf.max_range[k] = t.f[k].max_range;
        const int bc[3] = {fr.bc.x, fr.bc.y, fr.bc.z};
        for (int a = 0; a < 3; ++a) lo[a] = std::min(lo[a], bc[a] - fr.n_steps), hi[a] = std::max(hi[a], bc[a] + fr.n_steps);
        const size_t S = static_cast<size_t>(2 * fr.n_steps + 1);
        cubes += S * S * S;
      }
      const size_t box = static_cast<size_t>(hi[0] - lo[0] + 1) * static_cast<size_t>(hi[1] - lo[1] + 1) * static_cast<size_t>(hi[2] - lo[2] + 1);
      if (nb > 1 && box <= cubes && box < (1ull << 31)) {
        hipLaunchKernelGGL(k_tick_alloc, dim3(static_cast<unsigned>((box + kTickAllocThreads - 1) / kTickAllocThreads)), dim3(kTickAllocThreads), 0, c->stream, m, c->p, tf, nb, make_int3(lo[0], lo[1], lo[2]),
                           make_int3(hi[0] - lo[0] + 1, hi[1] - lo[1] + 1, hi[2] - lo[2] + 1), c->d_tick_work, cap, c->d_new,
                           c->d_tick_counts, c->motion_ignore_epoch);
      } else {
        for (int k = 0; k < nb; ++k) {
          const int S = 2 * tf.fr[k].n_steps + 1;
          const size_t total = static_cast<size_t>(S) * S * S;
          hipLaunchKernelGGL(k_alloc_visible, dim3(gridFor(total)), dim3(256), 0, c->stream, m, c->p, t.f[k], tf.fr[k],
                             c->d_tick_work + static_cast<size_t>(k) * cap, c->d_new, c->d_pinned + 2, 0u, &c->d_tick_counts[2 * k],
                             c->motion_ignore_epoch);
        }
      }
      HIP_TRY(hipGetLastError());
    }
    if (phases & 8) {
      ScopedTimer tm(c, 3);
      hipLaunchKernelGGL(k_init_blocks, dim3(2048), dim3(256), 0, c->stream, m, c->p, c->d_new);
      const FrameSlot& s0 = c->slots[slots[base]];
      if (one_launch && c->tick_mask_dirty)
        HIP_TRY(hipMemsetAsync(c->d_tick_mask, 0, sizeof(uint32_t) * (c->item_cap / 4 + 1), c->stream));
      c->tick_mask_dirty = one_launch;
      hipLaunchKernelGGL(k_tick_cull, dim3(256, nb), dim3(256), 0, c->stream, m, c->p, t, c->d_tick_work, cap, c->d_tick_work4, c->item_cap, c->wpb,
                         c->d_tick_counts, c->cfg.disable_culling ? 0 : 1, s0.tw, s0.th, one_launch ? c->d_tick_mask : nullptr);
      c->host_index_valid = false, ++c->map_gen;
      HIP_TRY(hipGetLastError());
    }
    if ((phases & 2) && one_launch) {
      rc = tickUpdateUnion(c, slots + base, t.f, nb, use_mask, object_id);
      if (rc) return rc;
    }
    for (int k = 0; k < nb && (phases & 2) && !one_launch; ++k) {
      FrameSlot& s = c->slots[slots[base + k]];
      UpdateLists lists;
      lists.list = FuseList{c->d_tick_work4 + static_cast<size_t>(2 * k) * c->item_cap, c->d_tick_work4 + static_cast<size_t>(2 * k + 1) * c->item_cap,
                            c->item_cap, &c->d_tick_counts[2 * kMaxTick + 4 * k]};
      rc = integrateUpdate(c, s, t.f[k], 1, use_mask, object_id, &lists);
      if (rc) return rc;
    }
    if (phases & 2) c->motion_ignore_epoch = 0;
  }
  return KHR_OK;
}
// ... 48 lines not shown
    if (c->d_halo_keys) { hipFree(c->d_halo_keys); hipFree(c->d_halo_vals); }
    c->d_halo_keys = nullptr;
    c->d_halo_vals = nullptr;
    c->halo_cap_total = 0;
    HIP_TRY(hipMalloc(&c->d_halo_keys, sizeof(uint64_t) * ht));
    HIP_TRY(hipMalloc(&c->d_halo_vals, sizeof(uint32_t) * ht));
    c->halo_cap_total = static_cast<uint32_t>(n_records);
  }
  if (!on_device && static_cast<uint64_t>(n_records) > c->halo_recs_cap) {
    HIP_TRY(hipStreamSynchronize(c->stream));
    if (c->d_halo_recs) hipFree(c->d_halo_recs);
    c->d_halo_recs = nullptr;
    c->halo_recs_cap = 0;
    HIP_TRY(hipMalloc(&c->d_halo_recs, static_cast<size_t>(n_records) * kHaloRecWords * sizeof(uint64_t)));
    c->halo_recs_cap = static_cast<uint32_t>(n_records);
  }
  c->halo_mask = ht - 1;
  if (on_device) {
    c->halo_view = static_cast<const uint64_t*>(records);
  } else {
    HIP_TRY(hipMemcpyAsync(c->d_halo_recs, records, static_cast<size_t>(n_records) * kHaloRecWords * sizeof(uint64_t),
                           hipMemcpyHostToDevice, c->stream));
    c->halo_view = c->d_halo_recs;
  }
  HIP_TRY(hipMemsetAsync(c->d_halo_keys, 0xff, sizeof(uint64_t) * (static_cast<size_t>(c->halo_mask) + 1), c->stream));
  hipLaunchKernelGGL(k_import_halo, dim3(gridFor(n_records)), dim3(256), 0, c->stream, c->halo_view,
                     static_cast<uint32_t>(n_records), c->cfg.rank, c->cfg.world_size, c->d_halo_keys, c->d_halo_vals, c->halo_mask);
  HIP_TRY(hipGetLastError());
  if (!on_device) HIP_TRY(hipStreamSynchronize(c->stream));
  c->halo_n = static_cast<uint32_t>(n_records);
  return KHR_OK;
}

static int motionLaunch(khr_ctx* c, FrameSlot& s, bool fresh_slot, bool do_begin = false) {
  const size_t n = static_cast<size_t>(s.sensor.width) * s.sensor.height;
  if (!fresh_slot) {
    if (!s.dyn_clean) HIP_TRY(hipMemsetAsync(s.dyn, 0, n * sizeof(int32_t), c->stream));
    HIP_TRY(hipMemsetAsync(&c->m.counters[C_N_SEEDS], 0, sizeof(uint32_t), c->stream));
  }
  c->stats.n_seeds = 0;
  c->h_pinned[0] = 0;
  c->seed_by_ticket = false;
  if (!c->cfg.with_tracking) return KHR_OK;
  DevMap& m = c->m;
  const DevFrame f = makeDevFrame(c, s);
  const float min_z_world = static_cast<float>(s.meta.world_T_sensor[11] + static_cast<double>(c->cfg.md_min_z_coordinate));
  {
    ScopedTimer tm(c, 4);
    ++c->seed_ticket;
    if (c->seed_ticket == 0) ++c->seed_ticket;
    hipLaunchKernelGGL(k_motion_pixels, dim3(gridFor(n)), dim3(256), 0, c->stream, m, c->p, f, c->cfg.md_max_range,
                       min_z_world, c->d_keys, c->motion_ignore_epoch, do_begin ? c->d_wg_stats : nullptr);
    if (do_begin) c->begun = true;
  }
  HIP_TRY(hipGetLastError());
  c->seed_by_ticket = true;
  c->seed_publish_pending = true;
  return KHR_OK;
}

static void seedWaitDone(khr_ctx* c, std::chrono::steady_clock::time_point t0, bool event_path) {
  const uint64_t us = static_cast<uint64_t>(std::chrono::duration_cast<std::chrono::microseconds>(std::chrono::steady_clock::now() - t0).count());
  ++c->n_seed_waits;
  c->seed_wait_max_us = std::max(c->seed_wait_max_us, us);
  static const uint64_t edge[7] = {50, 100, 200, 500, 1000, 2000, 5000};
  int b = 0;
  while (b < 7 && us >= edge[b]) ++b;
  ++c->seed_wait_hist[b];
  if (us > 500) {
    ++c->n_seed_waits_late;
    c->seed_wait_late_us = us;
    c->seed_wait_late_frame = c->n_seed_waits;
    uint64_t st = 0;
    if (hipStreamQuery(c->stream) == hipErrorNotReady) st |= 1u;
    if (c->aux_stream && hipStreamQuery(c->aux_stream) == hipErrorNotReady) st |= 2u;
    if (c->h2d_stream && hipStreamQuery(c->h2d_stream) == hipErrorNotReady) st |= 4u;
    if (c->last_ingest_on_aux) st |= 8u;
    if (event_path) st |= 16u;
    st |= static_cast<uint64_t>(c->ahead_q.size()) << 8;
    c->seed_wait_late_state = st;
  }
}

static int waitSeedCount(khr_ctx* c) {
  const auto t_wait0 = std::chrono::steady_clock::now();
  if (!c->seed_by_ticket) {
    HIP_TRY(hipEventSynchronize(c->ev_seed));
    seedWaitDone(c, t_wait0, true);
    return KHR_OK;
  }
  if (c->seed_publish_pending) {
    hipLaunchKernelGGL(k_publish_seed, dim3(1), dim3(1), 0, c->stream, c->m, c->d_pinned + 2, c->seed_ticket);
    HIP_TRY(hipGetLastError());
    c->seed_publish_pending = false;
  }
  volatile uint32_t* hp = c->h_pinned;
  uint64_t spins = 0;
  while (hp[3] != c->seed_ticket) {
    __builtin_ia32_pause();
    if ((++spins & 0xffffu) == 0) {
      const hipError_t q = hipStreamQuery(c->stream);
      if (q != hipSuccess && q != hipErrorNotReady) return fail(KHR_EDEVICE, "stream failed while waiting for the seed count: %s", hipGetErrorString(q));
      if (q == hipSuccess && hp[3] != c->seed_ticket) return fail(KHR_EDEVICE, "seed count was never published");
    }
  }
  c->h_pinned[0] = hp[2];
  seedWaitDone(c, t_wait0, false);
  return KHR_OK;
}

static int waitTicket(khr_ctx* c, int word, uint32_t ticket, const char* what, hipStream_t stream = nullptr) {
  volatile uint32_t* hp = c->h_pinned;
  uint64_t spins = 0;
  if (!stream) stream = c->stream;
  while (hp[word] != ticket) {
    __builtin_ia32_pause();
    if ((++spins & 0xffffu) == 0) {
      const hipError_t q = hipStreamQuery(stream);
      if (q != hipSuccess && q != hipErrorNotReady) return fail(KHR_EDEVICE, "stream failed while waiting for %s: %s", what, hipGetErrorString(q));
      if (q == hipSuccess && hp[word] != ticket) return fail(KHR_EDEVICE, "%s was never published", what);
    }
  }
  return KHR_OK;
}

static int clusterSummaryLaunch(khr_ctx* c, FrameSlot& s, int max_id) {
  if (c->md_defer_summary) {
// ... 439 lines not shown
  }
  lap("filter + paint launch");
  return n_out;
}

int khr_detect_motion(khr_ctx* c, int slot) {
  if (!c || slot < 0 || slot >= static_cast<int>(c->slots.size()) || !c->slots[slot].valid) return fail(KHR_EINVAL, "bad slot");
  HIP_TRY(hipSetDevice(c->device));
  FrameSlot& s = c->slots[slot];
  int rc = motionLaunch(c, s, false);
  if (rc) return rc;
  return motionFinish(c, s);
}

int khr_motion_keys(khr_ctx* c, int slot, void* keys_out, int on_device, uint32_t* n_seed_pixels) {
  if (!c || !keys_out || slot < 0 || slot >= static_cast<int>(c->slots.size()) || !c->slots[slot].valid) return fail(KHR_EINVAL, "bad argument");
  HIP_TRY(hipSetDevice(c->device));
  FrameSlot& s = c->slots[slot];
  const int n = s.sensor.width * s.sensor.height;
  int rc = motionLaunch(c, s, false);
  if (rc) return rc;
  uint64_t* dst = static_cast<uint64_t*>(keys_out);
  DevTemp holder;
  if (!on_device) {
    HIP_TRY(hipMalloc(&holder.p, sizeof(uint64_t) * n));
    dst = holder.as<uint64_t>();
  }
  hipLaunchKernelGGL(k_md_keys_export, dim3(gridFor(n)), dim3(256), 0, c->stream, c->d_keys, n, dst);
  if (!on_device) {
    HIP_TRY(hipMemcpyAsync(keys_out, dst, sizeof(uint64_t) * n, hipMemcpyDeviceToHost, c->stream));
    HIP_TRY(hipStreamSynchronize(c->stream));
  }
  if (!n_seed_pixels && on_device) {
    c->seed_publish_pending = false;
    c->seed_by_ticket = false;
    return KHR_OK;
  }
  { const int rcw = waitSeedCount(c); if (rcw) return rcw; }
  if (n_seed_pixels) *n_seed_pixels = c->h_pinned[0];
  return KHR_OK;
}

int khr_detect_motion_from_keys(khr_ctx* c, int slot, const void* keys, int on_device) {
  if (!c || !keys || slot < 0 || slot >= static_cast<int>(c->slots.size()) || !c->slots[slot].valid) return fail(KHR_EINVAL, "bad argument");
  HIP_TRY(hipSetDevice(c->device));
  FrameSlot& s = c->slots[slot];
  const int n = s.sensor.width * s.sensor.height;
  const uint64_t* src = static_cast<const uint64_t*>(keys);
  DevTemp holder;
  if (!on_device) {
    HIP_TRY(hipMalloc(&holder.p, sizeof(uint64_t) * n));
    HIP_TRY(hipMemcpyAsync(holder.p, keys, sizeof(uint64_t) * n, hipMemcpyHostToDevice, c->stream));
    src = holder.as<uint64_t>();
  }
  if (!s.dyn_clean) HIP_TRY(hipMemsetAsync(s.dyn, 0, sizeof(int32_t) * n, c->stream));
  s.dyn_clean = true, s.dynw_valid = false;
  HIP_TRY(hipMemsetAsync(&c->m.counters[C_N_SEEDS], 0, sizeof(uint32_t), c->stream));
  hipLaunchKernelGGL(k_md_keys_import, dim3(gridFor(n)), dim3(256), 0, c->stream, src, n, c->d_keys, &c->m.counters[C_N_SEEDS]);
  HIP_TRY(hipMemcpyAsync(&c->h_pinned[0], &c->m.counters[C_N_SEEDS], sizeof(uint32_t), hipMemcpyDeviceToHost, c->stream));
  HIP_TRY(hipEventRecord(c->ev_seed, c->stream));
  c->seed_by_ticket = false;
  return motionFinish(c, s);
}

size_t khr_motion_bits_bytes(int64_t n_pixels) { return n_pixels > 0 ? 16u * static_cast<size_t>((n_pixels + 63) / 64) : 0u; }

int khr_motion_bits(khr_ctx* c, int slot, void* bits_device) {
  if (!c || !bits_device || slot < 0 || slot >= static_cast<int>(c->slots.size()) || !c->slots[slot].valid) return fail(KHR_EINVAL, "bad argument");
  HIP_TRY(hipSetDevice(c->device));
  FrameSlot& s = c->slots[slot];
  const int n = s.sensor.width * s.sensor.height;
  int rc = motionLaunch(c, s, false);
  if (rc) return rc;
  hipLaunchKernelGGL(k_md_bits_export, dim3(gridFor((static_cast<size_t>(n) + 63) / 64 * 64)), dim3(256), 0, c->stream, c->d_keys, n,
                     static_cast<unsigned long long*>(bits_device));
  HIP_TRY(hipGetLastError());
  c->seed_publish_pending = false;
  c->seed_by_ticket = false;
  return KHR_OK;
}

int khr_detect_motion_from_bits(khr_ctx* c, int slot, const void* bits_device) {
  if (!c || !bits_device || slot < 0 || slot >= static_cast<int>(c->slots.size()) || !c->slots[slot].valid) return fail(KHR_EINVAL, "bad argument");
  HIP_TRY(hipSetDevice(c->device));
  FrameSlot& s = c->slots[slot];
  const int n = s.sensor.width * s.sensor.height;
  if (!s.dyn_clean) HIP_TRY(hipMemsetAsync(s.dyn, 0, sizeof(int32_t) * n, c->stream));
  s.dyn_clean = true, s.dynw_valid = false;
  HIP_TRY(hipMemsetAsync(&c->m.counters[C_N_SEEDS], 0, sizeof(uint32_t), c->stream));
  const float min_z_world = static_cast<float>(s.meta.world_T_sensor[11] + static_cast<double>(c->cfg.md_min_z_coordinate));
  hipLaunchKernelGGL(k_md_keys_from_bits, dim3(gridFor(n)), dim3(256), 0, c->stream, c->p, makeDevFrame(c, s), c->cfg.md_max_range, min_z_world,
                     static_cast<const unsigned long long*>(bits_device), c->d_keys, &c->m.counters[C_N_SEEDS]);
  HIP_TRY(hipMemcpyAsync(&c->h_pinned[0], &c->m.counters[C_N_SEEDS], sizeof(uint32_t), hipMemcpyDeviceToHost, c->stream));
  HIP_TRY(hipEventRecord(c->ev_seed, c->stream));
  c->seed_by_ticket = false;
  return motionFinish(c, s);
}

int khr_dynamic_pack_bytes(khr_ctx* c, int slot, void* dst_device) {
  if (!c || !dst_device || slot < 0 || slot >= static_cast<int>(c->slots.size()) || !c->slots[slot].valid) return fail(KHR_EINVAL, "bad argument");
  HIP_TRY(hipSetDevice(c->device));
  FrameSlot& s = c->slots[slot];
  const int n4 = (s.sensor.width * s.sensor.height + 3) / 4;
  hipLaunchKernelGGL(k_dyn_pack_u8, dim3(gridFor(n4)), dim3(256), 0, c->stream, s.dyn, n4, static_cast<uint32_t*>(dst_device));
  HIP_TRY(hipGetLastError());
  return KHR_OK;
}

int khr_dynamic_unpack_bytes(khr_ctx* c, int slot, const void* src_device) {
  if (!c || !src_device || slot < 0 || slot >= static_cast<int>(c->slots.size()) || !c->slots[slot].valid) return fail(KHR_EINVAL, "bad argument");
// ... 472 lines not shown
  HIP_TRY(hipGetLastError());
  std::vector<ObjAcc> acc(n_acc);
  uint32_t flags = 0;
  HIP_TRY(hipMemcpyAsync(acc.data(), d_acc, sizeof(ObjAcc) * n_acc, hipMemcpyDeviceToHost, c->stream));
  HIP_TRY(hipMemcpyAsync(&flags, d_flags, sizeof(flags), hipMemcpyDeviceToHost, c->stream));
  HIP_TRY(hipStreamSynchronize(c->stream));
  s.has_obj = true;
  s.objects_done = true;
  s.sem_clusters.clear();
  if (flags & 1u) return fail(KHR_EINVAL, "an instance id of the label image is outside 1..%d", max_id);
  int present = 0;
  for (size_t id = 0; id < n_acc; ++id) {
    khr_cluster k{};
    const ObjAcc& a = acc[id];
    k.id = static_cast<int32_t>(id);
    k.num_pixels_listed = a.n_pixels;
    k.num_pixels_painted = a.n_pixels;
    k.semantic_id = static_cast<int32_t>(id);
    if (a.n_pixels) {
      ++present;
      for (int d = 0; d < 3; ++d) {
        k.bbox_min[d] = orderedToFloat(a.bmin[d]);
        k.bbox_max[d] = orderedToFloat(a.bmax[d]);
        k.centroid[d] = a.sum[d] / static_cast<float>(a.n_pixels);
      }
    }
    out[id] = k;
  }
  return present;
}

int khr_generate_mesh(khr_ctx* c, int only_mesh_updated, int clear_flag) {
  if (!c) return fail(KHR_EINVAL, "null ctx");
  HIP_TRY(hipSetDevice(c->device));
  DevMap& m = c->m;
  const size_t cap = m.capacity;
  ScopedTimer tm(c, 5);
  HIP_TRY(hipMemsetAsync(c->d_mesh_nwork, 0, sizeof(uint32_t), c->stream));
  hipLaunchKernelGGL(k_mesh_prepare, dim3(gridFor(cap + 1)), dim3(256), 0, c->stream, m, only_mesh_updated ? BLK_MESH_UPDATED : 0u,
                     c->d_work, c->d_mesh_nwork, c->d_regen, c->d_mesh_count, c->d_mesh_old_off);
  MeshBuffers src = c->mesh[c->mesh_cur], dst = c->mesh[c->mesh_cur ^ 1];
  RemoteMeshHalo rmh{};
  if (c->mh_n) {
    rmh.recs = c->mh_view;
    rmh.ht_keys = c->d_mh_keys;
    rmh.ht_vals = c->d_mh_vals;
    rmh.ht_mask = c->mh_mask;
    if (c->mh_compact) {
      rmh.ht_keys = c->d_mh2_keys;
      rmh.ht_offs = c->d_mh2_offs;
    }
  }
  const uint32_t maxv = static_cast<uint32_t>(std::min<uint64_t>(c->cfg.max_mesh_vertices, 0xfffffff0ull));
  int rc = dispatchVps(c, [&](auto vps) {
    constexpr int V = decltype(vps)::value;
    KHR_LAUNCH_TIMED(8, (k_marching_cubes<V, false>), dim3(kStreamGrid), dim3(256), m, c->p, c->d_work,
                     c->d_mesh_nwork, c->d_mesh_count, c->d_mesh_offset, dst, clear_flag, maxv, rmh, 0xffffffffu,
                     static_cast<const uint8_t*>(nullptr), MeshBuffers{}, static_cast<const uint32_t*>(nullptr));
    size_t tb = c->cub_temp_bytes;
    HIP_TRY(hipcub::DeviceScan::ExclusiveSum(c->d_cub_temp, tb, c->d_mesh_count, c->d_mesh_offset,
                                             static_cast<int>(cap + 1), c->stream));
    constexpr uint32_t kMoveWgs = 1024;
    KHR_LAUNCH_TIMED(9, (k_marching_cubes<V, true>), dim3(kStreamGrid + kMoveWgs), dim3(256), m, c->p, c->d_work,
                     c->d_mesh_nwork, c->d_mesh_count, c->d_mesh_offset, dst, clear_flag, maxv, rmh, static_cast<uint32_t>(kStreamGrid),
                     static_cast<const uint8_t*>(c->d_regen), src, static_cast<const uint32_t*>(c->d_mesh_old_off));
    return KHR_OK;
// ... 50 lines not shown
      std::sort(tmp.begin(), tmp.end(), [](const int4& a, const int4& b) {
        return a.x != b.x ? a.x < b.x : (a.y != b.y ? a.y < b.y : a.z < b.z);
      });
      for (int64_t i = 0; i < std::min<int64_t>(ne, cap); ++i) {
        removed[3 * i] = tmp[i].x;
        removed[3 * i + 1] = tmp[i].y;
        removed[3 * i + 2] = tmp[i].z;
      }
    }
    return KHR_OK;
  }
  uint32_t n = 0;
  HIP_TRY(hipMemcpyAsync(&n, &c->m.counters[C_N_REMOVED], sizeof(uint32_t), hipMemcpyDeviceToHost, c->stream));
  HIP_TRY(hipStreamSynchronize(c->stream));
  c->removed_pending = false;
  if (n_removed) *n_removed = n;
  if (n && removed && cap > 0) {
    std::vector<int4> tmp(n);
    HIP_TRY(hipMemcpy(tmp.data(), c->d_removed, sizeof(int4) * n, hipMemcpyDeviceToHost));
    std::sort(tmp.begin(), tmp.end(), [](const int4& a, const int4& b) {
      return a.x != b.x ? a.x < b.x : (a.y != b.y ? a.y < b.y : a.z < b.z);
    });
    for (int64_t i = 0; i < std::min<int64_t>(n, cap); ++i) {
      removed[3 * i] = tmp[i].x;
      removed[3 * i + 1] = tmp[i].y;
      removed[3 * i + 2] = tmp[i].z;
    }
  }
  return KHR_OK;
}

int khr_mesh_halo_requests(khr_ctx* c, void* keys_out, int64_t cap, int only_mesh_updated, int on_device) {
  if (!c || !keys_out || cap < 1) return fail(KHR_EINVAL, "bad argument");
  HIP_TRY(hipSetDevice(c->device));
  DevMap& m = c->m;
  uint64_t* dst = static_cast<uint64_t*>(keys_out);
  DevTemp holder;
  uint64_t* tmp = nullptr;
  if (!on_device) {
    HIP_TRY(hipMalloc(&holder.p, sizeof(uint64_t) * cap));
    dst = tmp = holder.as<uint64_t>();
  }
  HIP_TRY(hipMemsetAsync(dst, 0, sizeof(uint64_t) * cap, c->stream));
  HIP_TRY(hipMemsetAsync(c->d_mesh_nwork + 1, 0, sizeof(uint32_t) * 2, c->stream));
  hipLaunchKernelGGL(k_list_live, dim3(gridFor(m.capacity)), dim3(256), 0, c->stream, m, c->d_work, c->d_mesh_nwork + 1,
                     only_mesh_updated ? BLK_MESH_UPDATED : 0u);
  hipLaunchKernelGGL(k_mesh_halo_requests, dim3(512), dim3(256), 0, c->stream, m, c->p, c->d_work, c->d_mesh_nwork + 1, dst,
                     static_cast<uint32_t>(cap), c->d_mesh_nwork + 2);
  uint32_t n_req = 0;
  HIP_TRY(hipMemcpyAsync(&n_req, c->d_mesh_nwork + 2, sizeof(uint32_t), hipMemcpyDeviceToHost, c->stream));
  if (!on_device) HIP_TRY(hipMemcpyAsync(keys_out, tmp, sizeof(uint64_t) * cap, hipMemcpyDeviceToHost, c->stream));
  HIP_TRY(hipStreamSynchronize(c->stream));
  if (n_req > cap) return fail(KHR_ENOMEM, "%u mesh halo requests exceed the capacity %lld", n_req, static_cast<long long>(cap));
  return static_cast<int>(n_req);
}

int khr_mesh_halo_export(khr_ctx* c, const void* requests, int64_t n_requests, void* records, int64_t cap_records, int on_device) {
  if (!c || !records || cap_records < 1 || n_requests < 0 || (!requests && n_requests > 0)) return fail(KHR_EINVAL, "bad argument");
  HIP_TRY(hipSetDevice(c->device));
  DevMap& m = c->m;
  const size_t words = c->p.vps == 16 ? MeshHalo<16>::kWords : MeshHalo<8>::kWords;
  const size_t bytes = static_cast<size_t>(cap_records) * words * 4;
  const uint64_t* req = static_cast<const uint64_t*>(requests);
  uint32_t* dst = static_cast<uint32_t*>(records);
  DevTemp req_holder, rec_holder;
  uint32_t* rec_tmp = nullptr;
  if (!on_device) {
    if (n_requests) {
      HIP_TRY(hipMalloc(&req_holder.p, sizeof(uint64_t) * n_requests));
      HIP_TRY(hipMemcpyAsync(req_holder.p, requests, sizeof(uint64_t) * n_requests, hipMemcpyHostToDevice, c->stream));
      req = req_holder.as<uint64_t>();
    }
    HIP_TRY(hipMalloc(&rec_holder.p, bytes));
    dst = rec_tmp = rec_holder.as<uint32_t>();
  }
  HIP_TRY(hipMemsetAsync(c->d_mh_flag, 0, m.capacity, c->stream));
  HIP_TRY(hipMemsetAsync(c->d_mesh_nwork + 3, 0, sizeof(uint32_t), c->stream));
  if (n_requests)
    hipLaunchKernelGGL(k_mesh_halo_mark, dim3(gridFor(n_requests)), dim3(256), 0, c->stream, m, c->p, req,
                       static_cast<uint32_t>(n_requests), c->d_mh_flag);
  hipLaunchKernelGGL(k_list_marked, dim3(gridFor(m.capacity)), dim3(256), 0, c->stream, m, c->d_mh_flag, c->d_new, c->d_mesh_nwork + 3);
  int rc = dispatchVps(c, [&](auto vps) {
    hipLaunchKernelGGL((k_mesh_halo_export<decltype(vps)::value>), dim3(static_cast<unsigned>(std::min<int64_t>(cap_records, 2048))),
                       dim3(256), 0, c->stream, m, c->p, c->d_new, c->d_mesh_nwork + 3, dst, static_cast<uint32_t>(cap_records));
    return KHR_OK;
  });
  hipError_t e = hipSuccess;
  uint32_t n_rec = 0;
  if (rc == KHR_OK) e = hipMemcpyAsync(&n_rec, c->d_mesh_nwork + 3, sizeof(uint32_t), hipMemcpyDeviceToHost, c->stream);
  if (e == hipSuccess && rc == KHR_OK && !on_device) e = hipMemcpyAsync(records, rec_tmp, bytes, hipMemcpyDeviceToHost, c->stream);
  if (e == hipSuccess) e = hipStreamSynchronize(c->stream);
// ... 36 lines not shown
                     static_cast<uint32_t>(n_records), static_cast<int>(words), c->cfg.rank, c->cfg.world_size, c->d_mh_keys,
                     c->d_mh_vals, c->mh_mask);
  HIP_TRY(hipGetLastError());
  if (!on_device) HIP_TRY(hipStreamSynchronize(c->stream));
  c->mh_n = static_cast<uint32_t>(n_records);
  return KHR_OK;
}

int khr_mesh_halo_plan(int world, int rank, int vps, const uint64_t* headers, uint64_t* sendcounts, uint64_t* sdispls,
                       uint64_t* recvcounts, uint64_t* rdispls) {
  if (world < 1 || world > kMeshHaloMaxWorld || rank < 0 || rank >= world || (vps != 8 && vps != 16) || !headers || !sendcounts || !sdispls ||
      !recvcounts || !rdispls)
    return fail(KHR_EINVAL, "khr_mesh_halo_plan: bad argument (world <= %d)", kMeshHaloMaxWorld);
  uint64_t so = 0, ro = 0;
  for (int q = 0; q < world; ++q) {
    uint64_t sw = 0, rw = 0;
    for (int sel = 1; sel < 8; ++sel) {
      const uint64_t aw = static_cast<uint64_t>(meshHaloAnswerWords(sel, vps));
      sw += headers[static_cast<size_t>(q) * 8 * world + static_cast<size_t>(rank) * 8 + sel] * aw;
      rw += headers[static_cast<size_t>(rank) * 8 * world + static_cast<size_t>(q) * 8 + sel] * aw;
    }
    sendcounts[q] = sw;
    sdispls[q] = so;
    so += sw;
    recvcounts[q] = rw;
    rdispls[q] = ro;
    ro += rw;
  }
  return KHR_OK;
}

int khr_mesh_halo_requests_sorted(khr_ctx* c, void* requests_device, int64_t cap, int only_mesh_updated) {
  if (!c || !requests_device || cap < 1) return fail(KHR_EINVAL, "bad argument");
  const int world = c->cfg.world_size;
  if (world > kMeshHaloMaxWorld) return fail(KHR_EINVAL, "the compact mesh halo is laid out for at most %d ranks", kMeshHaloMaxWorld);
  HIP_TRY(hipSetDevice(c->device));
  DevMap& m = c->m;
  constexpr int NB = 8 * kMeshHaloMaxWorld;
  if (!c->d_mh2_scratch) HIP_TRY(hipMalloc(reinterpret_cast<void**>(&c->d_mh2_scratch), sizeof(uint32_t) * (3 * NB + 1)));
  uint32_t* const cnt = c->d_mh2_scratch;
  uint32_t* const base = cnt + NB;
  uint32_t* const cursor = base + NB;
  uint32_t* const total = cursor + NB;
  uint64_t* const req = static_cast<uint64_t*>(requests_device);
  const uint32_t hw = 8u * static_cast<uint32_t>(world);
  HIP_TRY(hipMemsetAsync(cnt, 0, sizeof(uint32_t) * NB, c->stream));
  HIP_TRY(hipMemsetAsync(c->d_mesh_nwork + 1, 0, sizeof(uint32_t), c->stream));
  hipLaunchKernelGGL(k_list_live, dim3(gridFor(m.capacity)), dim3(256), 0, c->stream, m, c->d_work, c->d_mesh_nwork + 1,
                     only_mesh_updated ? BLK_MESH_UPDATED : 0u);
  hipLaunchKernelGGL((k_mesh_halo_req_sorted<false>), dim3(512), dim3(256), 0, c->stream, m, c->p, c->d_work, c->d_mesh_nwork + 1, cnt,
                     base, cursor, req, hw, static_cast<uint32_t>(cap));
  hipLaunchKernelGGL(k_mesh_halo_req_plan, dim3(1), dim3(64), 0, c->stream, cnt, base, cursor, req, world, total);
  hipLaunchKernelGGL((k_mesh_halo_req_sorted<true>), dim3(512), dim3(256), 0, c->stream, m, c->p, c->d_work, c->d_mesh_nwork + 1, cnt,
                     base, cursor, req, hw, static_cast<uint32_t>(cap));
  uint32_t n_req = 0;
  HIP_TRY(hipMemcpyAsync(&n_req, total, sizeof(uint32_t), hipMemcpyDeviceToHost, c->stream));
  HIP_TRY(hipStreamSynchronize(c->stream));
  if (n_req > cap) return fail(KHR_ENOMEM, "%u mesh halo requests exceed the capacity %lld", n_req, static_cast<long long>(cap));
  return static_cast<int>(n_req);
}

namespace {
uint64_t bucketBase(const uint64_t* header, int owner, int sel) {
  uint64_t b = 0;
  for (int i = 1; i < owner * 8 + sel; ++i) b += header[i];
  return b;
}
}

int khr_mesh_halo_answer(khr_ctx* c, const void* all_requests_device, int64_t cap, const uint64_t* headers, void* records_device,
                         int64_t cap_words) {
  if (!c || !all_requests_device || cap < 1 || !headers || !records_device || cap_words < 1) return fail(KHR_EINVAL, "bad argument");
  const int world = c->cfg.world_size, rank = c->cfg.rank;
  if (world > kMeshHaloMaxWorld) return fail(KHR_EINVAL, "the compact mesh halo is laid out for at most %d ranks", kMeshHaloMaxWorld);
  HIP_TRY(hipSetDevice(c->device));
  const int vps = c->p.vps;
  const uint64_t stride = 8ull * world + static_cast<uint64_t>(cap);
  MeshHaloRuns runs{};
  uint64_t words = 0, items = 0;
  for (int q = 0; q < world; ++q) {
    const uint64_t* hq = headers + static_cast<size_t>(q) * 8 * world;
    if (hq[0] > static_cast<uint64_t>(cap)) return fail(KHR_ENOMEM, "rank %d listed %llu mesh halo requests, capacity %lld", q,
                                                        static_cast<unsigned long long>(hq[0]), static_cast<long long>(cap));
    for (int sel = 1; sel < 8; ++sel) {
      const uint64_t n = hq[rank * 8 + sel];
      if (!n) continue;
      const uint32_t r = runs.n_runs++;
      runs.first[r] = static_cast<uint32_t>(items);
      runs.req_off[r] = static_cast<uint32_t>(static_cast<uint64_t>(q) * stride + 8ull * world + bucketBase(hq, rank, sel));
      runs.rec_off[r] = static_cast<uint32_t>(words);
      runs.sel[r] = static_cast<uint8_t>(sel);
      if (static_cast<uint64_t>(q) * stride + 8ull * world + bucketBase(hq, rank, sel) >= 0xffffffffull)
        return fail(KHR_EINVAL, "mesh halo: the gathered request lists exceed 2^32 - 1 entries (capacity %lld x %d ranks)", static_cast<long long>(cap), world);
      items += n;
      words += n * static_cast<uint64_t>(meshHaloAnswerWords(sel, vps));
      if (words >= 0xffffffffull || items >= 0xffffffffull)
        return fail(KHR_ENOMEM, "mesh halo: the answers of this output exceed 2^32 - 1 words");
    }
  }
  runs.first[runs.n_runs] = static_cast<uint32_t>(items);
  runs.n_items = static_cast<uint32_t>(items);
  if (words > static_cast<uint64_t>(cap_words))
    return fail(KHR_ENOMEM, "the mesh halo answers of this output need %llu words, the buffer holds %lld", static_cast<unsigned long long>(words),
                static_cast<long long>(cap_words));
  if (!items) return 0;
// ... 165 lines not shown
  if (n_clusters) *n_clusters = 0;
  const bool motion = (flags & KHR_PF_MOTION) != 0;
  const bool objects = (flags & KHR_PF_OBJECTS) != 0;
  const bool ahead = (flags & KHR_PF_INGESTED) != 0;
  if (ahead && (c->ahead_q.empty() || !frame || !motion || !(flags & KHR_PF_INPUT_READY) ||
                c->slots[c->ahead_q.front().slot].meta.timestamp_ns != frame->timestamp_ns)) {
    cancelAhead(c);
    return fail(KHR_ESTATE, "KHR_PF_INGESTED: the oldest frame handed over by khr_ingest_ahead does not carry this stamp (or flags are missing); the handed-over frames were dropped");
  }
  if (!ahead && !c->ahead_q.empty()) return fail(KHR_ESTATE, "the frames handed over by khr_ingest_ahead have to be processed first (khr_ingest_cancel drops them)");
  const bool pinned_in = !on_device && (flags & KHR_PF_INPUT_PINNED) != 0;
  if (pinned_in && !ahead && frame && (!pointerIs(frame->depth, 0) || !pointerIs(frame->color, 0) || !pointerIs(frame->label, 0)))
    return fail(KHR_EINVAL, "KHR_PF_INPUT_PINNED: the frame's buffers must be page-locked host memory (hipHostMalloc / hipHostRegister)");
  struct Leave {
    khr_ctx* c;
    bool ok = false;
    ~Leave() {
      c->defer_fold = false;
      if (!ok && c->fold_pending) {
        hipLaunchKernelGGL(k_fuse_fold, dim3((c->m.capacity + 255) / 256), dim3(256), 0, c->stream, c->m.blk_flags, c->m.blk_band,
                           &c->m.counters[C_MAX_SLOT], static_cast<const uint32_t*>(nullptr));
        c->fold_pending = false;
      }
      if (c->h2d_pending) {
        hipEventSynchronize(c->ev_h2d);
        c->h2d_pending = false;
      }
      if (own_h2d) hipEventSynchronize(own_h2d);
    }
    hipEvent_t own_h2d = nullptr;
  } leave{c};
  const bool early = ahead || ((flags & KHR_PF_INPUT_READY) && (on_device || pinned_in) && motion && c->cfg.with_tracking &&
                               c->slots.size() >= (pinned_in ? 3u : 2u) && peekSlot(c) != c->last_frame_slot);
  int slot;
  int ahead_ev = 0;
  if (ahead) {
    const khr_ctx::AheadEntry e = c->ahead_q.front();
    c->ahead_q.erase(c->ahead_q.begin());
    slot = e.slot;
    ahead_ev = e.ev;
    if (e.host) leave.own_h2d = c->ev_ahead_h2d[e.ev];
    c->slot_leases[slot].fetch_sub(1, std::memory_order_acq_rel);
  } else {
    c->begin_in_ingest = !early;
    c->last_ingest_on_aux = early;
    c->ingest_stream = early ? c->aux_stream : nullptr;
    c->host_input_pinned = pinned_in;
    slot = khr_upload_frame(c, sensor, frame, on_device);
    c->host_input_pinned = false;
    c->ingest_stream = nullptr;
    c->begin_in_ingest = false;
    if (slot < 0) return slot;
  }
  c->last_frame_slot = slot;
  FrameSlot& s = c->slots[slot];
  const DevFrame f = makeDevFrame(c, s);
  int rc = KHR_OK;
  if (ahead) {
    c->begun = false;
    HIP_TRY(hipStreamWaitEvent(c->stream, c->ev_ahead[ahead_ev], 0));
  } else if (early) {
    c->begun = false;
    s.aux_seq = ++c->aux_seq_issued;
    HIP_TRY(hipEventRecord(c->ev_aux_done, c->aux_stream));
    HIP_TRY(hipStreamWaitEvent(c->stream, c->ev_aux_done, 0));
  }
  if (objects && !c->obj_configured) return fail(KHR_ESTATE, "KHR_PF_OBJECTS needs khr_configure_object_detector");
  if (objects && !early) {
    if (!c->ev_ingest) HIP_TRY(hipEventCreateWithFlags(&c->ev_ingest, hipEventDisableTiming));
    HIP_TRY(hipEventRecord(c->ev_ingest, c->stream));
  }
  if (motion && (rc = motionLaunch(c, s, true, early))) return rc;
  if ((rc = integrateAlloc(c, s, f, 1))) return rc;
  HT("pf_alloc_launched");
  if (objects) {
    if (!(ahead && c->obj_pending_slot == slot)) {
      if (!early) HIP_TRY(hipStreamWaitEvent(c->aux_stream, c->ev_ingest, 0));
      if (ahead) HIP_TRY(hipStreamWaitEvent(c->aux_stream, c->ev_ahead[ahead_ev], 0));
      if ((rc = objectsLaunch(c, slot))) return rc;
    }
    HT("pf_objects_launched");
  }
  bool speculated = false;
  size_t spec_timer = static_cast<size_t>(-1), spec_end = 0;
  c->defer_fold = (flags & KHR_PF_TRACKING) && c->cfg.with_tracking;
  if (motion && c->cfg.with_tracking && !(c->md_seed_run && std::getenv("KHR_MD_NO_PRELAUNCH") == nullptr)) {
    const size_t n_pending = c->pending.size();
    rc = integrateUpdate(c, s, f, 1, 0, -1, nullptr, &c->m.counters[C_N_SEEDS]);
    if (rc) return rc;
    if (c->pending.size() > n_pending) spec_timer = n_pending;
    spec_end = c->pending.size();
    speculated = true;
  }
  bool have_seeds = false;
  if (motion) {
    c->md_defer_summary = true;
    c->md_summary_pending = -1;
    const int nc = motionFinish(c, s);
    c->md_defer_summary = false;
    if (nc < 0) return nc;
    if (n_clusters) *n_clusters = nc;
    have_seeds = c->cfg.with_tracking && c->h_pinned[0] != 0;
  }
  HT("pf_motion_done");
  if (speculated && have_seeds && spec_timer != static_cast<size_t>(-1))
    for (size_t i = spec_timer; i < spec_end && i < c->pending.size(); ++i) c->pending[i].which = -1;
// ... 78 lines not shown
  if (!c) return fail(KHR_EINVAL, "null ctx");
  hipLaunchKernelGGL(k_block_flag_op, dim3(gridFor(c->m.capacity)), dim3(256), 0, c->stream, c->m, ~BLK_UPDATED, 0u);
  HIP_TRY(hipGetLastError());
  c->host_index_valid = false, ++c->map_gen;
  return KHR_OK;
}

int khr_allocate_blocks(khr_ctx* c, const int32_t* indices, int64_t n) {
  if (!c || (!indices && n > 0)) return fail(KHR_EINVAL, "null argument");
  if (n <= 0) return KHR_OK;
  HIP_TRY(hipSetDevice(c->device));
  std::vector<std::array<int32_t, 3>> v(n);
  for (int64_t i = 0; i < n; ++i) v[i] = {indices[3 * i], indices[3 * i + 1], indices[3 * i + 2]};
  std::sort(v.begin(), v.end());
  v.erase(std::unique(v.begin(), v.end()), v.end());
  const size_t bytes = sizeof(int32_t) * 3 * v.size();
  HT("ab_enter");
  if (!c->ev_up) HIP_TRY(hipEventCreateWithFlags(&c->ev_up, hipEventDisableTiming));
  else HIP_TRY(hipEventSynchronize(c->ev_up));
  HT("ab_prev_upload_consumed");
  if (bytes > c->h_up_bytes) {
    HIP_TRY(hipStreamSynchronize(c->stream));
    if (c->h_up) hipHostFree(c->h_up);
    c->h_up = nullptr;
    c->h_up_bytes = 0;
    const size_t want = std::max<size_t>(2 * bytes, 1u << 16);
    if (hipHostMalloc(&c->h_up, want, hipHostMallocDefault) != hipSuccess)
      return fail(KHR_ENOMEM, "block index staging of %zu bytes", want);
    c->h_up_bytes = want;
  }
  std::memcpy(c->h_up, v.data(), bytes);
  void* up_dev = nullptr;
  HIP_TRY(hipHostGetDevicePointer(&up_dev, c->h_up, 0));
  HIP_TRY(hipMemsetAsync(&c->m.counters[C_N_NEW], 0, sizeof(uint32_t), c->stream));
  c->explicit_blocks += v.size();
  hipLaunchKernelGGL(k_alloc_list, dim3(gridFor(v.size())), dim3(256), 0, c->stream, c->m, static_cast<const int*>(up_dev),
                     static_cast<int>(v.size()), c->d_new);
  HIP_TRY(hipEventRecord(c->ev_up, c->stream));
  hipLaunchKernelGGL(k_init_blocks, dim3(2048), dim3(256), 0, c->stream, c->m, c->p, c->d_new);
  HIP_TRY(hipGetLastError());
  c->host_index_valid = false, ++c->map_gen;
  return KHR_OK;
}

int khr_object_prune(khr_ctx* c, float min_confidence, float min_observations, int64_t* n_pruned) {
  if (!c) return fail(KHR_EINVAL, "null ctx");
  if (!c->cfg.with_semantics || c->p.K < 2) return fail(KHR_ESTATE, "object pruning needs a binary semantic layer");
  HIP_TRY(hipMemsetAsync(&c->m.stats[S_PRUNED], 0, sizeof(unsigned long long), c->stream));
  int rc = dispatchVps(c, [&](auto vps) {
    hipLaunchKernelGGL((k_object_prune<decltype(vps)::value>), dim3(kStreamGrid), dim3(256), 0, c->stream, c->m, c->p,
                       min_confidence, min_observations);
    return KHR_OK;
  });
  if (rc) return rc;
  if (n_pruned) {
    unsigned long long np = 0;
    HIP_TRY(hipMemcpyAsync(&np, &c->m.stats[S_PRUNED], sizeof(np), hipMemcpyDeviceToHost, c->stream));
    HIP_TRY(hipStreamSynchronize(c->stream));
    *n_pruned = static_cast<int64_t>(np);
  }
  return KHR_OK;
}

static int refreshMeshTotals(khr_ctx* c);

int64_t khr_pool_exhausted(khr_ctx* c) {
  if (!c) return fail(KHR_EINVAL, "null ctx");
// ... 190 lines not shown
  for (uint32_t k = 2 * kSliceSortTile; k <= sort_len; k <<= 1) {
    for (uint32_t j = k / 2; j >= kSliceSortTile; j >>= 1) {
      hipLaunchKernelGGL(k_slice_sort_step, dim3(std::min(gridFor(sort_len / 2), 1024)), dim3(256), 0, c->stream, c->d_slice_keys,
                         c->d_slice_count, k, j);
      HIP_TRY(hipGetLastError());
    }
    hipLaunchKernelGGL(k_slice_sort_tile, dim3(sort_len / kSliceSortTile), dim3(kSliceSortThreads), 0, c->stream, c->d_slice_keys,
                       c->d_slice_count, k);
    HIP_TRY(hipGetLastError());
  }
  return KHR_OK;
}

static int sliceGrow(khr_ctx* c, uint32_t need) {
  const uint32_t cap = std::min<uint32_t>(std::max<uint32_t>(need + need / 2, 64u), c->m.capacity);
  const SliceLayout L(cap, static_cast<size_t>(c->p.vps) * c->p.vps);
  if (c->d_slice_stage) HIP_TRY(hipFree(c->d_slice_stage));
  if (c->h_slice_stage) HIP_TRY(hipHostFree(c->h_slice_stage));
  c->d_slice_stage = c->h_slice_stage = nullptr;
  c->slice_cap = 0;
  if (hipMalloc(reinterpret_cast<void**>(&c->d_slice_stage), L.bytes) != hipSuccess) return fail(KHR_ENOMEM, "slice staging of %zu bytes", L.bytes);
  if (hipHostMalloc(reinterpret_cast<void**>(&c->h_slice_stage), L.bytes, hipHostMallocDefault) != hipSuccess) {
    hipFree(c->d_slice_stage);
    c->d_slice_stage = nullptr;
    return fail(KHR_ENOMEM, "page-locked slice staging of %zu bytes", L.bytes);
  }
  c->slice_cap = cap;
  return KHR_OK;
}

int khr_map_slice(khr_ctx* c, int64_t voxel_z, int64_t cap, int32_t* block_xy, float* positions, float* distance, float* weight,
                  uint64_t* last_observed, uint8_t* voxel_flags, int64_t* n_voxels) {
  if (!c || !n_voxels || cap < 0) return fail(KHR_EINVAL, "bad argument");
  *n_voxels = 0;
  HIP_TRY(hipSetDevice(c->device));
  if (c->m.capacity >= (1u << kSliceSlotBits)) return fail(KHR_EINVAL, "map slices need max_blocks < %u", 1u << kSliceSlotBits);
  const int64_t vps = c->p.vps, np = vps * vps;
  const int64_t bz = (voxel_z >= 0 ? voxel_z : voxel_z - (vps - 1)) / vps, lz = voxel_z - bz * vps;
  if (bz < -(1 << 20) || bz >= (1 << 20)) return KHR_OK;
  {
    const int rc = ensureSortKeys(c);
    if (rc) return rc;
  }
  if (!c->d_slice_stage) {
    const int rc = sliceGrow(c, 64u);
    if (rc) return rc;
  }
  const bool want[6] = {block_xy != nullptr, positions != nullptr, distance != nullptr, weight != nullptr, last_observed != nullptr,
                        voxel_flags != nullptr};
  auto outFor = [&]() {
    const SliceLayout L(c->slice_cap, static_cast<size_t>(np));
    uint8_t* d = c->d_slice_stage;
    SliceOut o{};
    o.block_xy = want[0] ? reinterpret_cast<int32_t*>(d + L.xy) : nullptr;
    o.pos = want[1] ? reinterpret_cast<float*>(d + L.pos) : nullptr;
    o.dist = want[2] ? reinterpret_cast<float*>(d + L.dist) : nullptr;
    o.weight = want[3] ? reinterpret_cast<float*>(d + L.weight) : nullptr;
    o.last_obs = want[4] ? reinterpret_cast<uint64_t*>(d + L.obs) : nullptr;
    o.vflags = want[5] ? d + L.flags : nullptr;
    o.cap_blocks = c->slice_cap;
    return o;
  };
  const int gather_grid = static_cast<int>(std::min<uint32_t>(c->m.capacity, 2048u));
  auto gather = [&]() {
    return dispatchVps(c, [&](auto vps_c) {
      constexpr int V = decltype(vps_c)::value;
// ... 25 lines not shown
  uint32_t n_copied = std::min(c->slice_cap, c->slice_hint);
  HIP_TRY(hipMemcpyAsync(c->h_slice_stage, c->d_slice_count, sizeof(uint32_t), hipMemcpyDeviceToHost, c->stream));
  if ((rc = copies(0, n_copied))) return rc;
  HIP_TRY(hipStreamSynchronize(c->stream));
  const uint32_t n = *reinterpret_cast<const uint32_t*>(c->h_slice_stage);
  if (n > c->slice_cap) {
    if ((rc = sliceGrow(c, n))) return rc;
    if ((rc = gather())) return rc;
    n_copied = 0;
  }
  if (n > n_copied) {
    if ((rc = copies(n_copied, n))) return rc;
    HIP_TRY(hipStreamSynchronize(c->stream));
  }
  c->slice_hint = n + n / 4 + 16;
  *n_voxels = static_cast<int64_t>(n) * np;
  if (*n_voxels > cap)
    return fail(KHR_ENOMEM, "the slice holds %lld voxels, cap %lld", static_cast<long long>(*n_voxels), static_cast<long long>(cap));
  const SliceLayout L(c->slice_cap, static_cast<size_t>(np));
  const uint8_t* h = c->h_slice_stage;
  const size_t nv = static_cast<size_t>(*n_voxels);
  if (block_xy) std::memcpy(block_xy, h + L.xy, static_cast<size_t>(n) * 8);
  if (positions) std::memcpy(positions, h + L.pos, nv * 12);
  if (distance) std::memcpy(distance, h + L.dist, nv * 4);
  if (weight) std::memcpy(weight, h + L.weight, nv * 4);
  if (last_observed) std::memcpy(last_observed, h + L.obs, nv * 8);
  if (voxel_flags) std::memcpy(voxel_flags, h + L.flags, nv);
  return KHR_OK;
}

int khr_render_view(khr_ctx* c, const khr_render_request* rq, int on_device, float* depth, float* normal, uint8_t* color_rgba,
                    uint32_t* label, uint8_t* vflags, uint8_t* status, khr_render_stats* stats) {
  if (!c || !rq) return fail(KHR_EINVAL, "null argument");
  const khr_sensor& sn = rq->sensor;
  for (int i = 0; i < 16; ++i)
    if (!std::isfinite(rq->world_T_sensor[i])) return fail(KHR_EINVAL, "world_T_sensor is not finite");
  if (sn.width <= 0 || sn.height <= 0 || static_cast<int64_t>(sn.width) * sn.height > (int64_t(1) << 30))
    return fail(KHR_EINVAL, "bad image size %d x %d", sn.width, sn.height);
  if (!std::isfinite(sn.fx) || !std::isfinite(sn.fy) || sn.fx == 0.f || sn.fy == 0.f || !std::isfinite(sn.cx) || !std::isfinite(sn.cy))
    return fail(KHR_EINVAL, "bad intrinsics");
  if (!std::isfinite(sn.min_range) || !std::isfinite(sn.max_range) || sn.min_range < 0.f || sn.max_range < sn.min_range)
    return fail(KHR_EINVAL, "bad range limits [%g, %g]", static_cast<double>(sn.min_range), static_cast<double>(sn.max_range));
  if (!(rq->step_voxels >= 0.f) || !std::isfinite(rq->step_voxels)) return fail(KHR_EINVAL, "bad step_voxels %g", static_cast<double>(rq->step_voxels));
  if (!(rq->min_weight >= 0.f)) return fail(KHR_EINVAL, "bad min_weight %g", static_cast<double>(rq->min_weight));
  const float dt = (rq->step_voxels == 0.f ? 0.5f : rq->step_voxels) * c->p.vs;
  const float n_steps = std::floor((sn.max_range - sn.min_range) / dt);
  if (!(n_steps < 65536.f)) return fail(KHR_EINVAL, "more than 65536 samples per ray (step %g m over %g m)", static_cast<double>(dt),
                                        static_cast<double>(sn.max_range - sn.min_range));
  if (c->cfg.world_size > 1) return fail(KHR_ESTATE, "khr_render_view needs the whole map: world_size is %d", c->cfg.world_size);
  HIP_TRY(hipSetDevice(c->device));
  RenderView r{};
  r.W = sn.width;
  r.H = sn.height;
  r.K = static_cast<int>(n_steps) + 1;
  r.fx = sn.fx;
  r.fy = sn.fy;
  r.cx = sn.cx;
  r.cy = sn.cy;
  r.min_range = sn.min_range;
  r.dt = dt;
  r.min_weight = rq->min_weight == 0.f ? c->cfg.mesh_min_weight : rq->min_weight;
  {
    float R[9], t[3];
    makePose(rq->world_T_sensor, R, t, r.Rw, r.tw);
  }
  const size_t n_px = static_cast<size_t>(sn.width) * sn.height;
// ... 32 lines not shown
    if (!c->d_render_stats && hipMalloc(reinterpret_cast<void**>(&c->d_render_stats), sizeof(unsigned long long) * RS_COUNT) != hipSuccess)
      return fail(KHR_ENOMEM, "render counters");
    HIP_TRY(hipMemsetAsync(c->d_render_stats, 0, sizeof(unsigned long long) * RS_COUNT, c->stream));
    r.stats = c->d_render_stats;
  }
  const dim3 grid(static_cast<unsigned>((sn.width + 15) / 16), static_cast<unsigned>((sn.height + 15) / 16));
  int rc = dispatchVps(c, [&](auto vps) {
    hipLaunchKernelGGL((k_render_view<decltype(vps)::value>), grid, dim3(256), 0, c->stream, c->m, c->p, r);
    HIP_TRY(hipGetLastError());
    return KHR_OK;
  });
  if (rc) return rc;
  unsigned long long h_stats[RS_COUNT] = {0, 0, 0, 0};
  if (stats) HIP_TRY(hipMemcpyAsync(h_stats, c->d_render_stats, sizeof(h_stats), hipMemcpyDeviceToHost, c->stream));
  if (!on_device && stage_bytes)
    HIP_TRY(hipMemcpyAsync(c->h_render_stage, c->d_render_stage, stage_bytes, hipMemcpyDeviceToHost, c->stream));
  if (stats || (!on_device && stage_bytes)) HIP_TRY(hipStreamSynchronize(c->stream));
  if (!on_device)
    for (int f = 0; f < 6; ++f)
      if (host[f]) std::memcpy(host[f], c->h_render_stage + off[f], n_px * per_px[f]);
  if (stats) {
    stats->n_hit = h_stats[RS_HIT];
    stats->n_blocked = h_stats[RS_BLOCKED];
    stats->n_samples_total = static_cast<uint64_t>(r.K) * n_px;
    stats->n_samples_evaluated = h_stats[RS_VISITED];
  }
  return KHR_OK;
}

int khr_query_points(khr_ctx* c, int64_t n, const float* points, float min_weight, int on_device, float* distance, float* gradient,
                     float* weight, uint8_t* color_rgba, uint32_t* label, uint8_t* vflags, uint64_t* last_observed, uint8_t* status,
                     khr_query_stats* stats) {
  if (!c) return fail(KHR_EINVAL, "null argument");
  if (n < 0) return fail(KHR_EINVAL, "negative point count %lld", static_cast<long long>(n));
  if (n > 0 && !points) return fail(KHR_EINVAL, "null points");
  if (!(min_weight >= 0.f) || !std::isfinite(min_weight)) return fail(KHR_EINVAL, "bad min_weight %g", static_cast<double>(min_weight));
  if (c->cfg.world_size > 1) return fail(KHR_ESTATE, "khr_query_points needs the whole map: world_size is %d", c->cfg.world_size);
  if (n == 0) {
    if (stats) *stats = khr_query_stats{0, 0, 0};
    return KHR_OK;
  }
  HIP_TRY(hipSetDevice(c->device));
  const size_t np = static_cast<size_t>(n);
  void* const host[8] = {distance, gradient, weight, color_rgba, label, vflags, last_observed, status};
  const size_t per_pt[8] = {4, 12, 4, 4, 4, 1, 8, 1};
  size_t off[8], stage_bytes = (np * 12 + 255) / 256 * 256;
  const size_t out_begin = stage_bytes;
  for (int f = 0; f < 8; ++f) {
    off[f] = stage_bytes;
    if (host[f]) stage_bytes += (np * per_pt[f] + 255) / 256 * 256;
  }
  void* dev[8] = {distance, gradient, weight, color_rgba, label, vflags, last_observed, status};
  const float* d_points = points;
  if (!on_device) {
    if (stage_bytes > c->query_stage_bytes) {
      if (c->d_query_stage) HIP_TRY(hipFree(c->d_query_stage));
      if (c->h_query_stage) HIP_TRY(hipHostFree(c->h_query_stage));
      c->d_query_stage = c->h_query_stage = nullptr;
      c->query_stage_bytes = 0;
      if (hipMalloc(reinterpret_cast<void**>(&c->d_query_stage), stage_bytes) != hipSuccess)
        return fail(KHR_ENOMEM, "query staging of %zu bytes", stage_bytes);
      if (hipHostMalloc(reinterpret_cast<void**>(&c->h_query_stage), stage_bytes, hipHostMallocDefault) != hipSuccess) {
        hipFree(c->d_query_stage);
        c->d_query_stage = nullptr;
        return fail(KHR_ENOMEM, "page-locked query staging of %zu bytes", stage_bytes);
      }
// ... 203 lines not shown
  if (h.header_bytes != KHR_CKPT_HEADER_BYTES) return fail(KHR_EINVAL, "checkpoint: header_bytes %u, expected %d", h.header_bytes, KHR_CKPT_HEADER_BYTES);
  if (h.voxels_per_side != 8 && h.voxels_per_side != 16) return fail(KHR_EINVAL, "checkpoint: voxels_per_side %d (must be 8 or 16)", h.voxels_per_side);
  if (!(h.voxel_size > 0.f) || !(h.truncation_distance > 0.f)) return fail(KHR_EINVAL, "checkpoint: voxel_size / truncation_distance must be > 0");
  if ((h.with_semantics | 1) != 1 || (h.with_tracking | 1) != 1) return fail(KHR_EINVAL, "checkpoint: with_semantics / with_tracking must be 0 or 1");
  if (h.with_semantics ? (h.num_labels < 1 || h.num_labels > 65536) : (h.num_labels != 0 || h.semantic_mode != 0))
    return fail(KHR_EINVAL, "checkpoint: num_labels %d / semantic_mode %d do not fit with_semantics %d", h.num_labels, h.semantic_mode, h.with_semantics);
  if (h.num_blocks > (1ull << 32)) return fail(KHR_EINVAL, "checkpoint: block count %llu", static_cast<unsigned long long>(h.num_blocks));
  uint64_t off[KHR_CKPT_SECTIONS], total = 0;
  ckptOffsets(CkptShape(h.voxels_per_side, h.with_tracking, h.with_semantics, h.num_labels), h.num_blocks, off, &total);
  for (int s = 0; s < KHR_CKPT_SECTIONS; ++s)
    if (h.offset[s] != off[s])
      return fail(KHR_EINVAL, "checkpoint: section %s at offset %llu, expected %llu", kCkptSectionNames[s], static_cast<unsigned long long>(h.offset[s]),
                  static_cast<unsigned long long>(off[s]));
  if (h.total_bytes != total) return fail(KHR_EINVAL, "checkpoint: total_bytes %llu, expected %llu", static_cast<unsigned long long>(h.total_bytes), static_cast<unsigned long long>(total));
  if (n_bytes < total)
    return fail(KHR_EINVAL, "checkpoint: truncated buffer (%llu bytes, the header claims %llu)", static_cast<unsigned long long>(n_bytes), static_cast<unsigned long long>(total));
  *out = h;
  return KHR_OK;
}

int khr_checkpoint_size(khr_ctx* c, uint64_t* n_bytes, int64_t* n_blocks) {
  if (!c) return fail(KHR_EINVAL, "null ctx");
  HIP_TRY(hipSetDevice(c->device));
  const int rc = ensureHostIndex(c);
  if (rc) return rc;
  const khr_checkpoint_header h = ckptHeaderFor(c->cfg, c->host_index.size());
  if (n_bytes) *n_bytes = h.total_bytes;
  if (n_blocks) *n_blocks = static_cast<int64_t>(h.num_blocks);
  return KHR_OK;
}

int khr_checkpoint_save(khr_ctx* c, void* buffer, uint64_t cap_bytes, uint64_t* n_bytes) {
  if (!c || (!buffer && cap_bytes)) return fail(KHR_EINVAL, "null argument");
  HIP_TRY(hipSetDevice(c->device));
  int rc = ensureSortKeys(c);
  if (rc) return rc;
  HIP_TRY(hipMemsetAsync(c->d_slice_count, 0, sizeof(uint32_t), c->stream));
  hipLaunchKernelGGL(k_ckpt_select, dim3(std::min(gridFor(c->m.capacity), 1024)), dim3(256), 0, c->stream, c->m, c->d_slice_count, c->d_slice_keys);
  HIP_TRY(hipGetLastError());
  if ((rc = sortKeys(c))) return rc;
  uint32_t n = 0;
  HIP_TRY(hipMemcpyAsync(&n, c->d_slice_count, sizeof(uint32_t), hipMemcpyDeviceToHost, c->stream));
  HIP_TRY(hipStreamSynchronize(c->stream));
  const khr_checkpoint_header h = ckptHeaderFor(c->cfg, n);
  if (n_bytes) *n_bytes = h.total_bytes;
  if (h.total_bytes > cap_bytes)
    return fail(KHR_ENOMEM, "checkpoint: the stream of %u blocks has %llu bytes, the buffer %llu", n, static_cast<unsigned long long>(h.total_bytes),
                static_cast<unsigned long long>(cap_bytes));
  const CkptShape sh(h.voxels_per_side, h.with_tracking, h.with_semantics, h.num_labels);
  const uint32_t cb = ckptChunkBlocks(sh);
  const bool bounce = !pointerIs(buffer, 0);
  if ((rc = ckptEnsureStage(c, sh, cb, bounce))) return rc;
  const CkptStageLayout L(sh, cb);
  uint8_t* const dst = static_cast<uint8_t*>(buffer);
  std::memset(dst, 0, KHR_CKPT_HEADER_BYTES);
  std::memcpy(dst, &h, sizeof(h));
  for (int s = 0; s < KHR_CKPT_SECTIONS; ++s)
    if (sh.per[s]) {
      const uint64_t end = h.offset[s] + sh.per[s] * n, pad = (64 - end % 64) % 64;
      std::memset(dst + end, 0, pad);
    }
  const uint32_t n_chunks = (n + cb - 1) / cb;
  auto drain = [&](uint32_t chunk) {
    const uint32_t b0 = chunk * cb, nb = std::min(cb, n - b0);
    for (int s = 0; s < KHR_CKPT_SECTIONS; ++s)
      if (sh.per[s]) std::memcpy(dst + h.offset[s] + sh.per[s] * b0, c->h_ckpt[chunk & 1] + L.off[s], sh.per[s] * nb);
// ... 102 lines not shown
      HIP_TRY(hipGetLastError());
      return KHR_OK;
    });
    if (rc) return rc;
    HIP_TRY(hipEventRecord(c->ev_ckpt_drained[buf], c->stream));
  }
  rc = dispatchVps(c, [&](auto vps) {
    hipLaunchKernelGGL((k_ckpt_rebuild<decltype(vps)::value>), dim3(std::max(1u, std::min(c->m.capacity, 4096u))), dim3(256), 0, c->stream, c->m, c->p, c->wpb);
    HIP_TRY(hipGetLastError());
    return KHR_OK;
  });
  if (rc) return rc;
  uint32_t err = 0, live = 0;
  HIP_TRY(hipMemcpyAsync(&err, c->d_ckpt_err, sizeof(uint32_t), hipMemcpyDeviceToHost, c->stream));
  HIP_TRY(hipMemcpyAsync(&live, &c->m.counters[C_N_LIVE], sizeof(uint32_t), hipMemcpyDeviceToHost, c->stream));
  HIP_TRY(hipStreamSynchronize(c->stream));
  HIP_TRY(hipStreamSynchronize(c->copy_stream));
  if (err || live != kept) {
    if ((rc = ckptClearMap(c))) return rc;
    HIP_TRY(hipStreamSynchronize(c->stream));
    if (err & kCkptErrDuplicate) return fail(KHR_EINVAL, "checkpoint: duplicate block index in the stream (met its twin at the hash insert)");
    if (err & kCkptErrIndex) return fail(KHR_EINVAL, "checkpoint: block index out of range");
    if (err & kCkptErrPool) return fail(KHR_ENOMEM, "checkpoint: the block pool (max_blocks %u) ran out during the load", c->m.capacity);
    return fail(KHR_EDEVICE, "checkpoint: %u blocks restored, %llu expected", live, static_cast<unsigned long long>(kept));
  }
  c->host_index_valid = false, ++c->map_gen;
  c->stats = khr_stats{};
  if (n_kept) *n_kept = static_cast<int64_t>(kept);
  return KHR_OK;
}

static int refreshMeshTotals(khr_ctx* c) {
  if (!c->mesh_stale) return KHR_OK;
  if (!c->h_totals && hipHostMalloc(reinterpret_cast<void**>(&c->h_totals), sizeof(uint32_t) * (C_COUNT + 2), hipHostMallocDefault) != hipSuccess)
    return fail(KHR_ENOMEM, "pinned block for the mesh totals");
  uint32_t* hs = c->h_totals;
  HIP_TRY(hipMemcpyAsync(hs, c->d_mesh_offset + c->m.capacity, sizeof(uint32_t), hipMemcpyDeviceToHost, c->stream));
  HIP_TRY(hipMemcpyAsync(hs + 1, c->d_mesh_nwork, sizeof(uint32_t), hipMemcpyDeviceToHost, c->stream));
  HIP_TRY(hipMemcpyAsync(hs + 2, c->m.counters, sizeof(uint32_t) * C_COUNT, hipMemcpyDeviceToHost, c->stream));
  HIP_TRY(hipStreamSynchronize(c->stream));
  const uint32_t total = hs[0], nwork = hs[1];
  c->h_counters.assign(hs + 2, hs + 2 + C_COUNT);
  c->counters_gen = c->map_gen;
  const uint32_t ovf = c->h_counters[C_MESH_OVERFLOW];
  if (ovf) return fail(KHR_ENOMEM, "mesh needs %u vertices, max_mesh_vertices=%llu", total,
                       static_cast<unsigned long long>(c->cfg.max_mesh_vertices));
  c->mesh_total = total;
  c->stats.n_mesh_blocks = nwork;
  c->stats.n_mesh_vertices = total;
  c->mesh_stale = false;
  return KHR_OK;
}

int64_t khr_download_updated(khr_ctx* c, int32_t* indices, float* distance, float* weight, uint8_t* color_rgba,
                             uint64_t* last_observed, uint8_t* voxel_flags, uint32_t* sem_label, int64_t cap_blocks) {
  if (!c) return fail(KHR_EINVAL, "null ctx");
  int rc = ensureHostIndex(c);
  if (rc) return rc;
  std::vector<uint32_t> slots;
  std::vector<int32_t> idx;
  for (auto& kv : c->host_index)
    if (c->host_flags[kv.second] & BLK_UPDATED) {
      slots.push_back(kv.second);
      idx.insert(idx.end(), kv.first.begin(), kv.first.end());
    }
  const int64_t n = static_cast<int64_t>(slots.size());
  if (n > cap_blocks) return fail(KHR_EINVAL, "%lld updated blocks, cap %lld", static_cast<long long>(n), static_cast<long long>(cap_blocks));
  if (n == 0) return 0;
  if (indices) std::memcpy(indices, idx.data(), sizeof(int32_t) * idx.size());
  const size_t nv = c->p.nvox, tot = static_cast<size_t>(n) * nv;
  const bool trk = c->cfg.with_tracking, sem = c->cfg.with_semantics;
  const size_t bytes = tot * ((distance ? 4 : 0) + (weight ? 4 : 0) + (color_rgba ? 4 : 0) + ((last_observed && trk) ? 8 : 0) +
                              (voxel_flags ? 1 : 0) + ((sem_label && sem) ? 4 : 0)) + sizeof(uint32_t) * n + 256;
  uint8_t* stage = nullptr;
  HIP_TRY(hipMalloc(&stage, bytes));
// ... 585 lines not shown
```

Measured before the change: 3996.

## Hoist next frame's block allocation onto aux stream with double-buffered frame counters

Adds a second set of per-frame counters and work/new lists so the next frame's visible-block allocation can run on the auxiliary stream while the current frame is still processing. Newly born blocks are marked unborn and then promoted to live in the motion kernel. The seed-count publish is folded into the motion kernel through a grid-wide completion counter, which removes a separate launch. Neighbour lookups now check the live flag and block index to guard against half-initialised slots. This adds complexity and possible race hazards, and many API entry points reset the front generation, which disables the hoist after any other map access.

New measurement: 3016. -24.5%, worse.

```diff
diff --git a/khronos_amd/csrc/khr_device.h b/khronos_amd/csrc/khr_device.h
--- a/khronos_amd/csrc/khr_device.h
+++ b/khronos_amd/csrc/khr_device.h
@@ -11,7 +11,8 @@
                    BLK_LIVE = 16u,
                    BLK_TRACK_DIRTY = 32u,
                    BLK_ANY_KEEP = 64u,
-                   BLK_HAS_NEG = 128u;
+                   BLK_HAS_NEG = 128u,
+                   BLK_UNBORN = 256u;
 constexpr uint8_t VOX_ACTIVE = 1, VOX_EVER_FREE = 2, VOX_TO_REMOVE = 4, VOX_SEM_VALID = 8;
 constexpr uint8_t VOX_OCC = 16;
 constexpr uint8_t VOX_PUBLIC_MASK = 0x0f;
@@ -45,6 +46,7 @@
   C_N_ITEMS3,
   C_COUNT = 32
 };
+constexpr int kFrameCounterSets = 2;
 enum Stat64 : int { S_UPD = 0 , S_BAND , S_MESH_VERTS, S_PRUNED, S_CUM_UPD, S_CUM_BAND, S_CUM_VISITED, S_CUM_CALLS, S_COUNT = 8 };
 
 struct MeshDesc {
@@ -73,6 +75,8 @@
   uint16_t* blk_band;
   uint32_t* free_slots;
   uint32_t* counters;
+  uint32_t* fc;
+  uint32_t* fc_prev;
   unsigned long long* stats;
   MeshDesc* mesh_desc;
 };
@@ -300,6 +304,7 @@
   return static_cast<uint8_t>(r);
 }
 
+constexpr int kMpGroups = 64, kMpStride = 16;
 __device__ inline void publishSeedCount(const DevMap& m, volatile uint32_t* host_seed, uint32_t ticket) {
   host_seed[0] = atomicAdd(&m.counters[C_N_SEEDS], 0u);
   __threadfence_system();
@@ -309,35 +314,37 @@
 
 constexpr int kUpdateStatSlots = 2048;
 
-__device__ inline void beginIntegrate(DevMap m, int nvox, uint32_t* wg_stats) {
-  unsigned long long u = 0, b = 0;
-  uint2* __restrict__ st = reinterpret_cast<uint2*>(wg_stats);
+__device__ inline void beginIntegrate(DevMap m, int nvox, uint32_t* wg_stats, int what = 3) {
+  if (what & 1) {
+    unsigned long long u = 0, b = 0;
+    uint2* __restrict__ st = reinterpret_cast<uint2*>(wg_stats);
 #pragma unroll 4
-  for (int i = threadIdx.x; i < kUpdateStatSlots; i += blockDim.x) {
-    const uint2 v = st[i];
-    u += v.x;
-    b += v.y;
-    if (v.x | v.y) st[i] = make_uint2(0u, 0u);
-  }
+    for (int i = threadIdx.x; i < kUpdateStatSlots; i += blockDim.x) {
+      const uint2 v = st[i];
+      u += v.x;
+      b += v.y;
+      if (v.x | v.y) st[i] = make_uint2(0u, 0u);
+    }
 #pragma unroll
-  for (int o = 32; o > 0; o >>= 1) {
-    u += __shfl_down(u, o);
-    b += __shfl_down(b, o);
-  }
-  if ((threadIdx.x & 63) == 0 && (u | b)) {
-    atomicAdd(&m.stats[S_CUM_UPD], u);
-    atomicAdd(&m.stats[S_CUM_BAND], b);
-  }
-  if (threadIdx.x == 0) {
-    m.stats[S_CUM_VISITED] += static_cast<unsigned long long>(m.counters[C_N_VISIBLE]) * nvox;
+    for (int o = 32; o > 0; o >>= 1) {
+      u += __shfl_down(u, o);
+      b += __shfl_down(b, o);
+    }
+    if ((threadIdx.x & 63) == 0 && (u | b)) {
+      atomicAdd(&m.stats[S_CUM_UPD], u);
+      atomicAdd(&m.stats[S_CUM_BAND], b);
+    }
+  }
+  if ((what & 2) && threadIdx.x == 0) {
+    m.stats[S_CUM_VISITED] += static_cast<unsigned long long>(m.fc_prev[C_N_VISIBLE]) * nvox;
     m.stats[S_CUM_CALLS] += 1ull;
-    m.counters[C_N_VISIBLE] = 0u;
-    m.counters[C_N_NEW] = 0u;
-    m.counters[C_N_TSDF] = 0u;
-    m.counters[C_N_ITEMS0] = 0u;
-    m.counters[C_N_ITEMS1] = 0u;
-    m.counters[C_N_ITEMS2] = 0u;
-    m.counters[C_N_ITEMS3] = 0u;
+    m.fc[C_N_VISIBLE] = 0u;
+    m.fc[C_N_NEW] = 0u;
+    m.fc[C_N_TSDF] = 0u;
+    m.fc[C_N_ITEMS0] = 0u;
+    m.fc[C_N_ITEMS1] = 0u;
+    m.fc[C_N_ITEMS2] = 0u;
+    m.fc[C_N_ITEMS3] = 0u;
   }
 }
 
diff --git a/khronos_amd/csrc/khr_kernels_aux.h b/khronos_amd/csrc/khr_kernels_aux.h
--- a/khronos_amd/csrc/khr_kernels_aux.h
+++ b/khronos_amd/csrc/khr_kernels_aux.h
@@ -13,8 +13,15 @@
 
 __global__ __launch_bounds__(256) void k_motion_pixels(DevMap m, DevParams p, DevFrame f, float md_max_range,
                                                       float min_z_world, uint64_t* __restrict__ keys, int ignore_epoch,
-                                                      uint32_t* __restrict__ begin_band_count) {
-  if (begin_band_count && blockIdx.x == 0) beginIntegrate(m, p.nvox, begin_band_count);
+                                                      uint32_t* __restrict__ begin_band_count, int begin_what,
+                                                      const uint32_t* __restrict__ born_list, volatile uint32_t* host_seed,
+                                                      uint32_t seed_ticket, uint32_t* __restrict__ mp_done) {
+  if (begin_band_count && blockIdx.x == 0) beginIntegrate(m, p.nvox, begin_band_count, begin_what);
+  if (born_list) {
+    const uint32_t n_born = m.fc[C_N_NEW];
+    for (uint32_t j = blockIdx.x * blockDim.x + threadIdx.x; j < n_born; j += gridDim.x * blockDim.x)
+      m.blk_flags[born_list[j]] = BLK_LIVE | BLK_TRACK_DIRTY | BLK_ANY_KEEP;
+  }
   const int i = blockIdx.x * blockDim.x + threadIdx.x;
   const bool in = i < f.W * f.H;
   uint64_t key = ~0ull;
@@ -24,7 +31,20 @@
   if (in) keys[i] = key;
   const bool seed = (key != ~0ull) && (key & kSeedBit);
   const int any = __syncthreads_count(seed ? 1 : 0);
-  if (any && threadIdx.x == 0) atomicAdd(&m.counters[C_N_SEEDS], static_cast<uint32_t>(any));
+  if (threadIdx.x != 0) return;
+  if (any) atomicAdd(&m.counters[C_N_SEEDS], static_cast<uint32_t>(any));
+  if (!seed_ticket) return;
+  __threadfence();
+  const uint32_t g = blockIdx.x % kMpGroups;
+  const uint32_t g_size = (gridDim.x - g + kMpGroups - 1) / kMpGroups;
+  const uint32_t n_groups = min(gridDim.x, static_cast<uint32_t>(kMpGroups));
+  if (atomicAdd(&mp_done[g * kMpStride], 1u) + 1u != g_size) return;
+  mp_done[g * kMpStride] = 0u;
+  __threadfence();
+  if (atomicAdd(&m.counters[C_MP_DONE], 1u) + 1u != n_groups) return;
+  m.counters[C_MP_DONE] = 0u;
+  __threadfence();
+  publishSeedCount(m, host_seed, seed_ticket);
 }
 
 __global__ __launch_bounds__(1024) void k_publish(const uint32_t* __restrict__ src, volatile uint32_t* __restrict__ dst_host,
@@ -39,10 +59,6 @@
     *ticket_host = ticket;
     __threadfence_system();
   }
-}
-
-__global__ void k_publish_seed(DevMap m, volatile uint32_t* host_seed, uint32_t ticket) {
-  if (blockIdx.x == 0 && threadIdx.x == 0) publishSeedCount(m, host_seed, ticket);
 }
 
 __global__ __launch_bounds__(256) void k_md_keys_export(const uint64_t* __restrict__ keys, int n, uint64_t* __restrict__ out) {
@@ -1565,7 +1581,7 @@
     m.mesh_desc[i] = MeshDesc{0u, 0u};
     m.free_slots[i] = i;
   }
-  if (i < C_COUNT) m.counters[i] = i == C_N_FREE ? m.capacity : 0u;
+  if (i < kFrameCounterSets * C_COUNT) m.counters[i] = i == C_N_FREE ? m.capacity : 0u;
   if (i < S_COUNT) m.stats[i] = 0ull;
 }
 
diff --git a/khronos_amd/csrc/khr_kernels_fusion.h b/khronos_amd/csrc/khr_kernels_fusion.h
--- a/khronos_amd/csrc/khr_kernels_fusion.h
+++ b/khronos_amd/csrc/khr_kernels_fusion.h
@@ -54,7 +54,7 @@
                                                      float fy, float cx, float cy, int range_mode, DevMap m, int nvox,
                                                      uint32_t* __restrict__ wg_stats, int do_begin) {
   if (blockIdx.x == 0 && threadIdx.x == 0) m.counters[C_N_SEEDS] = 0u;
-  if (do_begin && blockIdx.x == 0) beginIntegrate(m, nvox, wg_stats);
+  if (do_begin && blockIdx.x == 0) beginIntegrate(m, nvox, wg_stats, do_begin);
   float d, r;
   ingestTile(depth_in, rgb_in, label_in, depth, range, rgba, label, dyn, tile_max, blockIdx.x, tw, W, H, fx, fy, cx, cy,
              range_mode, &d, &r);
@@ -187,9 +187,7 @@
 
 __global__ __launch_bounds__(256) void k_alloc_visible(DevMap m, DevParams p, DevFrame f, DevFrustum fr,
                                                       uint32_t* __restrict__ work, uint32_t* __restrict__ new_list,
-                                                      volatile uint32_t* host_seed, uint32_t seed_ticket,
-                                                      uint32_t* __restrict__ list_count, int epoch) {
-  if (seed_ticket && blockIdx.x == 0 && threadIdx.x == 0) publishSeedCount(m, host_seed, seed_ticket);
+                                                      uint32_t new_flags, uint32_t* __restrict__ list_count, int epoch) {
   const int S = 2 * fr.n_steps + 1;
   const int total = S * S * S;
   const int i = blockIdx.x * blockDim.x + threadIdx.x;
@@ -214,8 +212,9 @@
       slot = m.free_slots[fidx];
       got = true;
       m.blk_index[slot] = make_int4(bx, by, bz, epoch);
-      m.blk_flags[slot] = BLK_LIVE | BLK_TRACK_DIRTY | BLK_ANY_KEEP;
+      m.blk_flags[slot] = new_flags;
       m.mesh_desc[slot] = MeshDesc{0u, 0u};
+      __threadfence();
       htInsertUnique(m, key, slot);
       atomicMax(&m.counters[C_MAX_SLOT], slot + 1);
     } else {
@@ -223,12 +222,12 @@
       slot = kInvalidSlot;
     }
   }
-  const uint32_t nidx = waveAggInc(&m.counters[C_N_NEW], got);
+  const uint32_t nidx = waveAggInc(&m.fc[C_N_NEW], got);
   if (got) new_list[nidx] = slot;
   const bool emit = visible && slot != kInvalidSlot;
   const uint32_t widx = waveAggInc(list_count, emit);
   if (emit) work[widx] = slot;
-  if (list_count != &m.counters[C_N_VISIBLE]) waveAggInc(&m.counters[C_N_VISIBLE], emit);
+  if (list_count != &m.fc[C_N_VISIBLE]) waveAggInc(&m.fc[C_N_VISIBLE], emit);
 }
 
 struct TickFrusta {
@@ -277,7 +276,7 @@
       slot = kInvalidSlot;
     }
   }
-  const uint32_t nidx = waveAggInc(&m.counters[C_N_NEW], got);
+  const uint32_t nidx = waveAggInc(&m.fc[C_N_NEW], got);
   if (got) new_list[nidx] = slot;
   if (slot == kInvalidSlot) seen = 0u;
   __shared__ uint32_t s_cnt[kMaxTick], s_base[kMaxTick];
@@ -297,7 +296,7 @@
   if (threadIdx.x == 64) {
     uint32_t tot = 0u;
     for (int k = 0; k < ncam; ++k) tot += s_cnt[k];
-    if (tot) atomicAdd(&m.counters[C_N_VISIBLE], tot);
+    if (tot) atomicAdd(&m.fc[C_N_VISIBLE], tot);
   }
   __syncthreads();
 #pragma unroll
@@ -466,7 +465,7 @@
 __global__ __launch_bounds__(256) void k_cull_blocks(DevMap m, DevParams p, DevFrame f,
                                                     const uint32_t* __restrict__ work, FuseList out, uint32_t wpb,
                                                     const float* __restrict__ tile_max, int tw, int th) {
-  cullBlocks(m, p, f, work, &m.counters[C_N_VISIBLE], out, wpb, &m.counters[C_N_TSDF], tile_max, tw, th, blockIdx.x, gridDim.x);
+  cullBlocks(m, p, f, work, &m.fc[C_N_VISIBLE], out, wpb, &m.fc[C_N_TSDF], tile_max, tw, th, blockIdx.x, gridDim.x);
 }
 
 struct TickFrames {
@@ -512,7 +511,7 @@
       atomicAdd(&m.counters[C_POOL_EXHAUSTED], 1u);
     }
   }
-  const uint32_t nidx = waveAggInc(&m.counters[C_N_NEW], got);
+  const uint32_t nidx = waveAggInc(&m.fc[C_N_NEW], got);
   if (got) new_list[nidx] = slot;
 }
 
@@ -547,7 +546,7 @@
 
 __device__ inline void initBlocks(const DevMap& m, const DevParams& p, const uint32_t* __restrict__ new_list, uint32_t bid,
                                   uint32_t nblk) {
-  const uint32_t n = m.counters[C_N_NEW];
+  const uint32_t n = m.fc[C_N_NEW];
   const int nv = p.nvox;
   for (uint32_t b = bid; b < n; b += nblk) {
     const size_t slot = new_list[b];
@@ -589,7 +588,7 @@
                                                   const uint32_t* __restrict__ work, FuseList out, uint32_t wpb,
                                                   const float* __restrict__ tile_max, int tw, int th, uint32_t n_cull) {
   if (blockIdx.x < n_cull)
-    cullBlocks(m, p, f, work, &m.counters[C_N_VISIBLE], out, wpb, &m.counters[C_N_TSDF], tile_max, tw, th, blockIdx.x, n_cull);
+    cullBlocks(m, p, f, work, &m.fc[C_N_VISIBLE], out, wpb, &m.fc[C_N_TSDF], tile_max, tw, th, blockIdx.x, n_cull);
   else
     initBlocks(m, p, new_list, blockIdx.x - n_cull, gridDim.x - n_cull);
 }
@@ -819,7 +818,15 @@
     if (threadIdx.x < 27) {
       const int dx = threadIdx.x % 3 - 1, dy = (threadIdx.x / 3) % 3 - 1, dz = threadIdx.x / 9 - 1;
       const uint64_t key = packKey(bi.x + dx, bi.y + dy, bi.z + dz);
-      const uint32_t ns = (threadIdx.x == 13) ? static_cast<uint32_t>(slot) : htLookup(m, key);
+      uint32_t ns = (threadIdx.x == 13) ? static_cast<uint32_t>(slot) : htLookup(m, key);
+      if (threadIdx.x != 13 && ns != kInvalidSlot) {
+        const uint32_t nfl = __hip_atomic_load(&m.blk_flags[ns], __ATOMIC_RELAXED, __HIP_MEMORY_SCOPE_AGENT);
+        const int* const nbi = reinterpret_cast<const int*>(&m.blk_index[ns]);
+        const int nx = __hip_atomic_load(nbi, __ATOMIC_RELAXED, __HIP_MEMORY_SCOPE_AGENT);
+        const int ny = __hip_atomic_load(nbi + 1, __ATOMIC_RELAXED, __HIP_MEMORY_SCOPE_AGENT);
+        const int nz = __hip_atomic_load(nbi + 2, __ATOMIC_RELAXED, __HIP_MEMORY_SCOPE_AGENT);
+        if (!(nfl & BLK_LIVE) || nx != bi.x + dx || ny != bi.y + dy || nz != bi.z + dz) ns = kInvalidSlot;
+      }
       const uint64_t* src = nullptr;
       if (ns != kInvalidSlot) {
         src = m.freebits + static_cast<size_t>(ns) * NW;
diff --git a/khronos_amd/csrc/khronos_amd.hip b/khronos_amd/csrc/khronos_amd.hip
--- a/khronos_amd/csrc/khronos_amd.hip
+++ b/khronos_amd/csrc/khronos_amd.hip
@@ -115,6 +115,15 @@
   std::unique_ptr<std::atomic<int>[]> slot_leases;
   uint32_t* d_work = nullptr;
   uint32_t* d_new = nullptr;
+  uint32_t* d_work_set[2] = {nullptr, nullptr};
+  uint32_t* d_new_set[2] = {nullptr, nullptr};
+  uint4* d_work4_set[2] = {nullptr, nullptr};
+  int frame_set = 0;
+  uint64_t front_gen = 0;
+  bool front_on_main = false;
+  hipEvent_t ev_front = nullptr;
+  int front_epoch = 0;
+  uint32_t* d_mp_done = nullptr;
   uint32_t* d_ef = nullptr;
   uint32_t* d_trk_proc = nullptr;
   uint32_t* d_tick_work = nullptr;
@@ -192,9 +201,9 @@
   uint32_t* h_pinned = nullptr;
   uint32_t* d_pinned = nullptr;
   uint32_t seed_ticket = 0;
-  bool seed_publish_pending = false;
   bool seed_by_ticket = false;
   bool begin_in_ingest = false, begun = false;
+  bool begin_counters_only = false;
   uint32_t fetch_ticket = 0;
   bool fetch_pending = false;
   uint32_t* d_fetch_done = nullptr;
@@ -353,7 +362,8 @@
   int which;
   hipEvent_t a = nullptr, b = nullptr;
   bool on = false;
-  ScopedTimer(khr_ctx* ctx, int w) : c(ctx), which(w) {
+  hipStream_t st;
+  ScopedTimer(khr_ctx* ctx, int w, hipStream_t on_stream = nullptr) : c(ctx), which(w), st(on_stream ? on_stream : ctx->stream) {
     on = w >= 0 && ((c->timing >> w) & 1u);
     if (on) {
       auto get = [&]() {
@@ -368,12 +378,12 @@
       };
       a = get();
       b = get();
-      hipEventRecord(a, c->stream);
+      hipEventRecord(a, st);
     }
   }
   ~ScopedTimer() {
     if (on) {
-      hipEventRecord(b, c->stream);
+      hipEventRecord(b, st);
       c->pending.push_back({which, a, b});
     }
   }
@@ -516,11 +526,18 @@
   return KHR_OK;
 }
 
+static void foldFrameCounters(const khr_ctx* c, std::vector<uint32_t>& h) {
+  static const int per_frame[] = {C_N_VISIBLE, C_N_NEW, C_N_TSDF, C_N_ITEMS0, C_N_ITEMS1, C_N_ITEMS2, C_N_ITEMS3};
+  for (int k : per_frame) h[k] = h[k + c->frame_set * C_COUNT];
+  h.resize(C_COUNT);
+}
+
 int readCounters(khr_ctx* c) {
-  c->h_counters.resize(C_COUNT);
-  HIP_TRY(hipMemcpyAsync(c->h_counters.data(), c->m.counters, sizeof(uint32_t) * C_COUNT, hipMemcpyDeviceToHost,
+  c->h_counters.resize(kFrameCounterSets * C_COUNT);
+  HIP_TRY(hipMemcpyAsync(c->h_counters.data(), c->m.counters, sizeof(uint32_t) * kFrameCounterSets * C_COUNT, hipMemcpyDeviceToHost,
                          c->stream));
   HIP_TRY(hipStreamSynchronize(c->stream));
+  foldFrameCounters(c, c->h_counters);
   return KHR_OK;
 }
 
@@ -857,7 +874,9 @@
   A(devAlloc(c, &m.freebits, cfg->with_tracking ? cap * (nv / 64) : 1, false));
   A(devAlloc(c, &m.obs, cfg->with_tracking ? cap * (nv / 64) : 1, false));
   A(devAlloc(c, &m.free_slots, cap, false));
-  A(devAlloc(c, &m.counters, C_COUNT));
+  A(devAlloc(c, &m.counters, kFrameCounterSets * C_COUNT));
+  m.fc = m.fc_prev = m.counters;
+  A(devAlloc(c, &c->d_mp_done, kMpGroups * kMpStride));
   A(devAlloc(c, &m.stats, S_COUNT));
   A(devAlloc(c, &m.mesh_desc, cap));
   A(devAlloc(c, &c->d_work, cap));
@@ -876,6 +895,12 @@
     c->item_cap = static_cast<uint32_t>(cap) * c->wpb;
   }
   A(devAlloc(c, &c->d_work4, 2 * static_cast<size_t>(c->item_cap), false));
+  c->d_work_set[0] = c->d_work, c->d_new_set[0] = c->d_new, c->d_work4_set[0] = c->d_work4;
+  if (cfg->with_tracking && cfg->voxels_per_side != 8 && rc == KHR_OK) {
+    A(devAlloc(c, &c->d_work_set[1], cap, false));
+    A(devAlloc(c, &c->d_new_set[1], cap, false));
+    A(devAlloc(c, &c->d_work4_set[1], 2 * static_cast<size_t>(c->item_cap), false));
+  }
   if (cfg->voxels_per_side == 8 && rc == KHR_OK) {
     const size_t bits_words = static_cast<size_t>(c->item_cap) * 4;
     if (hipHostMalloc(reinterpret_cast<void**>(&c->h_frames), sizeof(FuseFrame) * kMaxMultiFrames, hipHostMallocDefault) != hipSuccess ||
@@ -887,7 +912,7 @@
       rc = fail(KHR_ENOMEM, "buffers of the multi-frame update");
     else
       c->frame_bits_words = bits_words;
-    if (rc == KHR_OK && (hipHostMalloc(reinterpret_cast<void**>(&c->h_totals), sizeof(uint32_t) * (C_COUNT + 2), hipHostMallocDefault) != hipSuccess ||
+    if (rc == KHR_OK && (hipHostMalloc(reinterpret_cast<void**>(&c->h_totals), sizeof(uint32_t) * (kFrameCounterSets * C_COUNT + 2), hipHostMallocDefault) != hipSuccess ||
                          hipEventCreateWithFlags(&c->ev_up, hipEventDisableTiming) != hipSuccess || hipEventRecord(c->ev_up, c->stream) != hipSuccess ||
                          hipEventCreateWithFlags(&c->ev_dep, hipEventDisableTiming) != hipSuccess ||
                          hipEventCreateWithFlags(&c->ev_dep_aux, hipEventDisableTiming) != hipSuccess))
@@ -1113,6 +1138,7 @@
   if (c->ev_dep_aux) hipEventDestroy(c->ev_dep_aux);
   if (c->ev_aux) hipEventDestroy(c->ev_aux);
   if (c->ev_aux_done) hipEventDestroy(c->ev_aux_done);
+  if (c->ev_front) hipEventDestroy(c->ev_front);
   if (c->aux_stream) hipStreamDestroy(c->aux_stream);
   if (c->own_stream && c->stream) hipStreamDestroy(c->stream);
   delete c;
@@ -1242,9 +1268,11 @@
   s.th = (sensor->height + kTile - 1) / kTile;
   hipLaunchKernelGGL(k_frame_ingest, dim3(s.tw * s.th), dim3(256), 0, ist, depth_src, rgb_src, label_src, s.depth,
                      s.range, s.rgba, s.label, s.dyn, s.tile_max, s.tw, sensor->width, sensor->height, sensor->fx, sensor->fy,
-                     sensor->cx, sensor->cy, c->p.range_mode, c->m, c->p.nvox, c->d_wg_stats, c->begin_in_ingest ? 1 : 0);
+                     sensor->cx, sensor->cy, c->p.range_mode, c->m, c->p.nvox, c->d_wg_stats,
+                     c->begin_in_ingest ? (c->begin_counters_only ? 2 : 3) : 0);
   HIP_TRY(hipGetLastError());
-  c->begun = c->begin_in_ingest;
+  c->begun = c->begin_in_ingest && !c->begin_counters_only;
+  if (c->begin_in_ingest) c->m.fc_prev = c->m.fc;
   c->begin_in_ingest = false;
   if (!on_device && !pinned) HIP_TRY(hipStreamSynchronize(c->stream));
   s.valid = true;
@@ -1422,25 +1450,41 @@
   return KHR_OK;
 }
 
-static int integrateAlloc(khr_ctx* c, FrameSlot& s, const DevFrame& f, int allocate_blocks) {
+static void useFrameSet(khr_ctx* c, int k) {
+  c->frame_set = k;
+  c->d_work = c->d_work_set[k], c->d_new = c->d_new_set[k], c->d_work4 = c->d_work4_set[k];
+  c->m.fc = c->m.counters + k * C_COUNT;
+}
+static int ensureFrontSets(khr_ctx* c) {
+  if (c->d_work4_set[1]) return KHR_OK;
+  int rc = devAlloc(c, &c->d_work_set[1], c->m.capacity, false);
+  if (!rc) rc = devAlloc(c, &c->d_new_set[1], c->m.capacity, false);
+  if (!rc) rc = devAlloc(c, &c->d_work4_set[1], 2 * static_cast<size_t>(c->item_cap), false);
+  return rc;
+}
+
+static int integrateAlloc(khr_ctx* c, FrameSlot& s, const DevFrame& f, int allocate_blocks, int hoist_epoch = 0) {
   DevMap& m = c->m;
-  if (!c->begun) hipLaunchKernelGGL(k_begin_integrate, dim3(1), dim3(256), 0, c->stream, m, c->p.nvox, c->d_wg_stats);
-  c->begun = false;
+  hipStream_t st = hoist_epoch ? c->aux_stream : c->stream;
+  if (!c->begun && !hoist_epoch) {
+    hipLaunchKernelGGL(k_begin_integrate, dim3(1), dim3(256), 0, c->stream, m, c->p.nvox, c->d_wg_stats);
+    m.fc_prev = m.fc;
+  }
+  if (!hoist_epoch) c->begun = false;
   if (allocate_blocks) {
-    ScopedTimer tm(c, 3);
+    ScopedTimer tm(c, 3, st);
     const DevFrustum fr = makeFrustum(c, f);
     const int S = 2 * fr.n_steps + 1;
     const size_t total = static_cast<size_t>(S) * S * S;
-    hipLaunchKernelGGL(k_alloc_visible, dim3(gridFor(total)), dim3(256), 0, c->stream, m, c->p, f, fr, c->d_work, c->d_new,
-                       c->d_pinned + 2, c->seed_publish_pending ? c->seed_ticket : 0u, &m.counters[C_N_VISIBLE], 0);
-    c->seed_publish_pending = false;
-    hipLaunchKernelGGL(k_init_cull, dim3(1024 + 1024), dim3(256), 0, c->stream, m, c->p, f, c->d_new, c->d_work,
-                       FuseList{c->d_work4, c->d_work4 + c->item_cap, c->item_cap, &m.counters[C_N_ITEMS0]}, c->wpb,
+    hipLaunchKernelGGL(k_alloc_visible, dim3(gridFor(total)), dim3(256), 0, st, m, c->p, f, fr, c->d_work, c->d_new,
+                       (hoist_epoch ? BLK_UNBORN : BLK_LIVE) | BLK_TRACK_DIRTY | BLK_ANY_KEEP, &m.fc[C_N_VISIBLE], hoist_epoch);
+    hipLaunchKernelGGL(k_init_cull, dim3(1024 + 1024), dim3(256), 0, st, m, c->p, f, c->d_new, c->d_work,
+                       FuseList{c->d_work4, c->d_work4 + c->item_cap, c->item_cap, &m.fc[C_N_ITEMS0]}, c->wpb,
                        c->cfg.disable_culling ? nullptr : s.vTileMax(), s.tw, s.th, 1024u);
     c->host_index_valid = false, ++c->map_gen;
   } else {
     hipLaunchKernelGGL(k_list_live, dim3(gridFor(m.capacity)), dim3(256), 0, c->stream, m, c->d_work,
-                       &m.counters[C_N_VISIBLE], 0u, FuseList{c->d_work4, c->d_work4 + c->item_cap, c->item_cap, &m.counters[C_N_ITEMS0]},
+                       &m.fc[C_N_VISIBLE], 0u, FuseList{c->d_work4, c->d_work4 + c->item_cap, c->item_cap, &m.fc[C_N_ITEMS0]},
                        c->wpb);
   }
   HIP_TRY(hipGetLastError());
@@ -1568,7 +1612,7 @@
     a.frame_bits = c->d_frame_bits;
     a.frame_words = n_words;
   }
-  FuseList list{c->d_work4, c->d_work4 + c->item_cap, c->item_cap, &c->m.counters[C_N_ITEMS0]};
+  FuseList list{c->d_work4, c->d_work4 + c->item_cap, c->item_cap, &c->m.fc[C_N_ITEMS0]};
   if (a.frame_bits != nullptr) {
     if (!c->d_multi_list) {
       HIP_TRY(hipStreamSynchronize(c->stream));
@@ -1623,7 +1667,7 @@
 static int integrateUpdate(khr_ctx* c, FrameSlot& s, const DevFrame& f, int allocate_blocks, int use_mask,
                            int object_id, const UpdateLists* lists = nullptr, const uint32_t* gate = nullptr) {
   DevMap& m = c->m;
-  FuseList list{c->d_work4, c->d_work4 + c->item_cap, c->item_cap, &m.counters[C_N_ITEMS0]};
+  FuseList list{c->d_work4, c->d_work4 + c->item_cap, c->item_cap, &m.fc[C_N_ITEMS0]};
   if (lists) list = lists->list;
   FuseArgs a{};
   fillFuseMap(c, &a);
@@ -2136,6 +2180,7 @@
       if (std::getenv("KHR_DEBUG_TICK_NO_EPOCH")) c->motion_ignore_epoch = 0;
       hipLaunchKernelGGL(k_tick_begin, dim3(1), dim3(256), 0, c->stream, m, c->p.nvox, c->d_wg_stats, c->d_tick_counts,
                          static_cast<uint32_t>(nb - 1));
+      c->m.fc_prev = c->m.fc;
       c->begun = false;
       ScopedTimer tm(c, 3);
       TickFrusta tf{};
@@ -2162,7 +2207,7 @@
           const int S = 2 * tf.fr[k].n_steps + 1;
           const size_t total = static_cast<size_t>(S) * S * S;
           hipLaunchKernelGGL(k_alloc_visible, dim3(gridFor(total)), dim3(256), 0, c->stream, m, c->p, t.f[k], tf.fr[k],
-                             c->d_tick_work + static_cast<size_t>(k) * cap, c->d_new, c->d_pinned + 2, 0u, &c->d_tick_counts[2 * k],
+                             c->d_tick_work + static_cast<size_t>(k) * cap, c->d_new, BLK_LIVE | BLK_TRACK_DIRTY | BLK_ANY_KEEP, &c->d_tick_counts[2 * k],
                              c->motion_ignore_epoch);
         }
       }
@@ -2277,7 +2322,7 @@
   return KHR_OK;
 }
 
-static int motionLaunch(khr_ctx* c, FrameSlot& s, bool fresh_slot, bool do_begin = false) {
+static int motionLaunch(khr_ctx* c, FrameSlot& s, bool fresh_slot, int do_begin = 0, int born_epoch = 0) {
   const size_t n = static_cast<size_t>(s.sensor.width) * s.sensor.height;
   if (!fresh_slot) {
     if (!s.dyn_clean) HIP_TRY(hipMemsetAsync(s.dyn, 0, n * sizeof(int32_t), c->stream));
@@ -2295,12 +2340,13 @@
     ++c->seed_ticket;
     if (c->seed_ticket == 0) ++c->seed_ticket;
     hipLaunchKernelGGL(k_motion_pixels, dim3(gridFor(n)), dim3(256), 0, c->stream, m, c->p, f, c->cfg.md_max_range,
-                       min_z_world, c->d_keys, c->motion_ignore_epoch, do_begin ? c->d_wg_stats : nullptr);
+                       min_z_world, c->d_keys, born_epoch ? born_epoch : c->motion_ignore_epoch, do_begin ? c->d_wg_stats : nullptr,
+                       do_begin, born_epoch ? c->d_new : nullptr, c->d_pinned + 2, c->seed_ticket, c->d_mp_done);
     if (do_begin) c->begun = true;
+    if (do_begin & 2) c->m.fc_prev = c->m.fc;
   }
   HIP_TRY(hipGetLastError());
   c->seed_by_ticket = true;
-  c->seed_publish_pending = true;
   return KHR_OK;
 }
 
@@ -2333,11 +2379,6 @@
     HIP_TRY(hipEventSynchronize(c->ev_seed));
     seedWaitDone(c, t_wait0, true);
     return KHR_OK;
-  }
-  if (c->seed_publish_pending) {
-    hipLaunchKernelGGL(k_publish_seed, dim3(1), dim3(1), 0, c->stream, c->m, c->d_pinned + 2, c->seed_ticket);
-    HIP_TRY(hipGetLastError());
-    c->seed_publish_pending = false;
   }
   volatile uint32_t* hp = c->h_pinned;
   uint64_t spins = 0;
@@ -2843,7 +2884,6 @@
     HIP_TRY(hipStreamSynchronize(c->stream));
   }
   if (!n_seed_pixels && on_device) {
-    c->seed_publish_pending = false;
     c->seed_by_ticket = false;
     return KHR_OK;
   }
@@ -2886,7 +2926,6 @@
   hipLaunchKernelGGL(k_md_bits_export, dim3(gridFor((static_cast<size_t>(n) + 63) / 64 * 64)), dim3(256), 0, c->stream, c->d_keys, n,
                      static_cast<unsigned long long*>(bits_device));
   HIP_TRY(hipGetLastError());
-  c->seed_publish_pending = false;
   c->seed_by_ticket = false;
   return KHR_OK;
 }
@@ -3425,6 +3464,7 @@
 
 int khr_generate_mesh(khr_ctx* c, int only_mesh_updated, int clear_flag) {
   if (!c) return fail(KHR_EINVAL, "null ctx");
+  c->front_gen = 0;
   HIP_TRY(hipSetDevice(c->device));
   DevMap& m = c->m;
   const size_t cap = m.capacity;
@@ -3541,6 +3581,7 @@
 
 int khr_mesh_halo_requests(khr_ctx* c, void* keys_out, int64_t cap, int only_mesh_updated, int on_device) {
   if (!c || !keys_out || cap < 1) return fail(KHR_EINVAL, "bad argument");
+  c->front_gen = 0;
   HIP_TRY(hipSetDevice(c->device));
   DevMap& m = c->m;
   uint64_t* dst = static_cast<uint64_t*>(keys_out);
@@ -3566,6 +3607,7 @@
 
 int khr_mesh_halo_export(khr_ctx* c, const void* requests, int64_t n_requests, void* records, int64_t cap_records, int on_device) {
   if (!c || !records || cap_records < 1 || n_requests < 0 || (!requests && n_requests > 0)) return fail(KHR_EINVAL, "bad argument");
+  c->front_gen = 0;
   HIP_TRY(hipSetDevice(c->device));
   DevMap& m = c->m;
   const size_t words = c->p.vps == 16 ? MeshHalo<16>::kWords : MeshHalo<8>::kWords;
@@ -3668,6 +3710,7 @@
 
 int khr_mesh_halo_requests_sorted(khr_ctx* c, void* requests_device, int64_t cap, int only_mesh_updated) {
   if (!c || !requests_device || cap < 1) return fail(KHR_EINVAL, "bad argument");
+  c->front_gen = 0;
   const int world = c->cfg.world_size;
   if (world > kMeshHaloMaxWorld) return fail(KHR_EINVAL, "the compact mesh halo is laid out for at most %d ranks", kMeshHaloMaxWorld);
   HIP_TRY(hipSetDevice(c->device));
@@ -3707,6 +3750,7 @@
 int khr_mesh_halo_answer(khr_ctx* c, const void* all_requests_device, int64_t cap, const uint64_t* headers, void* records_device,
                          int64_t cap_words) {
   if (!c || !all_requests_device || cap < 1 || !headers || !records_device || cap_words < 1) return fail(KHR_EINVAL, "bad argument");
+  c->front_gen = 0;
   const int world = c->cfg.world_size, rank = c->cfg.rank;
   if (world > kMeshHaloMaxWorld) return fail(KHR_EINVAL, "the compact mesh halo is laid out for at most %d ranks", kMeshHaloMaxWorld);
   HIP_TRY(hipSetDevice(c->device));
@@ -3938,6 +3982,17 @@
   } leave{c};
   const bool early = ahead || ((flags & KHR_PF_INPUT_READY) && (on_device || pinned_in) && motion && c->cfg.with_tracking &&
                                c->slots.size() >= (pinned_in ? 3u : 2u) && peekSlot(c) != c->last_frame_slot);
+  if (objects && !c->obj_configured) return fail(KHR_ESTATE, "KHR_PF_OBJECTS needs khr_configure_object_detector");
+  const bool hoist = early && !ahead && c->front_gen != 0 && c->front_gen == c->map_gen;
+  int hoist_epoch = 0;
+  if (hoist) {
+    int rcs = ensureFrontSets(c);
+    if (rcs) return rcs;
+    if (c->front_on_main) HIP_TRY(hipStreamWaitEvent(c->aux_stream, c->ev_front, 0));
+    useFrameSet(c, c->frame_set ^ 1);
+    if (--c->front_epoch >= 0) c->front_epoch = -1;
+    hoist_epoch = c->front_epoch;
+  }
   int slot;
   int ahead_ev = 0;
   if (ahead) {
@@ -3948,7 +4003,8 @@
     if (e.host) leave.own_h2d = c->ev_ahead_h2d[e.ev];
     c->slot_leases[slot].fetch_sub(1, std::memory_order_acq_rel);
   } else {
-    c->begin_in_ingest = !early;
+    c->begin_in_ingest = !early || hoist;
+    c->begin_counters_only = hoist;
     c->last_ingest_on_aux = early;
     c->ingest_stream = early ? c->aux_stream : nullptr;
     c->host_input_pinned = pinned_in;
@@ -3956,7 +4012,11 @@
     c->host_input_pinned = false;
     c->ingest_stream = nullptr;
     c->begin_in_ingest = false;
-    if (slot < 0) return slot;
+    c->begin_counters_only = false;
+    if (slot < 0) {
+      if (hoist) useFrameSet(c, c->frame_set ^ 1);
+      return slot;
+    }
   }
   c->last_frame_slot = slot;
   FrameSlot& s = c->slots[slot];
@@ -3968,16 +4028,28 @@
   } else if (early) {
     c->begun = false;
     s.aux_seq = ++c->aux_seq_issued;
+    if (hoist && (rc = integrateAlloc(c, s, f, 1, hoist_epoch))) return rc;
     HIP_TRY(hipEventRecord(c->ev_aux_done, c->aux_stream));
     HIP_TRY(hipStreamWaitEvent(c->stream, c->ev_aux_done, 0));
   }
-  if (objects && !c->obj_configured) return fail(KHR_ESTATE, "KHR_PF_OBJECTS needs khr_configure_object_detector");
   if (objects && !early) {
     if (!c->ev_ingest) HIP_TRY(hipEventCreateWithFlags(&c->ev_ingest, hipEventDisableTiming));
     HIP_TRY(hipEventRecord(c->ev_ingest, c->stream));
   }
-  if (motion && (rc = motionLaunch(c, s, true, early))) return rc;
-  if ((rc = integrateAlloc(c, s, f, 1))) return rc;
+  if (motion && (rc = motionLaunch(c, s, true, early ? (hoist ? 1 : 3) : 0, hoist_epoch))) return rc;
+  bool front_marked = hoist;
+  if (hoist) {
+    c->begun = false;
+  } else {
+    if ((rc = integrateAlloc(c, s, f, 1))) return rc;
+    if (c->cfg.with_tracking && c->slots.size() >= 2) {
+      if (!c->ev_front) HIP_TRY(hipEventCreateWithFlags(&c->ev_front, hipEventDisableTiming));
+      HIP_TRY(hipEventRecord(c->ev_front, c->stream));
+      front_marked = true;
+    }
+  }
+  c->front_on_main = !hoist;
+  c->front_gen = front_marked ? c->map_gen : 0;
   HT("pf_alloc_launched");
   if (objects) {
     if (!(ahead && c->obj_pending_slot == slot)) {
@@ -4122,7 +4194,7 @@
   std::memcpy(c->h_up, v.data(), bytes);
   void* up_dev = nullptr;
   HIP_TRY(hipHostGetDevicePointer(&up_dev, c->h_up, 0));
-  HIP_TRY(hipMemsetAsync(&c->m.counters[C_N_NEW], 0, sizeof(uint32_t), c->stream));
+  HIP_TRY(hipMemsetAsync(&c->m.fc[C_N_NEW], 0, sizeof(uint32_t), c->stream));
   c->explicit_blocks += v.size();
   hipLaunchKernelGGL(k_alloc_list, dim3(gridFor(v.size())), dim3(256), 0, c->stream, c->m, static_cast<const int*>(up_dev),
                      static_cast<int>(v.size()), c->d_new);
@@ -4379,6 +4451,7 @@
 int khr_map_slice(khr_ctx* c, int64_t voxel_z, int64_t cap, int32_t* block_xy, float* positions, float* distance, float* weight,
                   uint64_t* last_observed, uint8_t* voxel_flags, int64_t* n_voxels) {
   if (!c || !n_voxels || cap < 0) return fail(KHR_EINVAL, "bad argument");
+  c->front_gen = 0;
   *n_voxels = 0;
   HIP_TRY(hipSetDevice(c->device));
   if (c->m.capacity >= (1u << kSliceSlotBits)) return fail(KHR_EINVAL, "map slices need max_blocks < %u", 1u << kSliceSlotBits);
@@ -4470,6 +4543,7 @@
 int khr_render_view(khr_ctx* c, const khr_render_request* rq, int on_device, float* depth, float* normal, uint8_t* color_rgba,
                     uint32_t* label, uint8_t* vflags, uint8_t* status, khr_render_stats* stats) {
   if (!c || !rq) return fail(KHR_EINVAL, "null argument");
+  c->front_gen = 0;
   const khr_sensor& sn = rq->sensor;
   for (int i = 0; i < 16; ++i)
     if (!std::isfinite(rq->world_T_sensor[i])) return fail(KHR_EINVAL, "world_T_sensor is not finite");
@@ -4568,6 +4642,7 @@
                      float* weight, uint8_t* color_rgba, uint32_t* label, uint8_t* vflags, uint64_t* last_observed, uint8_t* status,
                      khr_query_stats* stats) {
   if (!c) return fail(KHR_EINVAL, "null argument");
+  c->front_gen = 0;
   if (n < 0) return fail(KHR_EINVAL, "negative point count %lld", static_cast<long long>(n));
   if (n > 0 && !points) return fail(KHR_EINVAL, "null points");
   if (!(min_weight >= 0.f) || !std::isfinite(min_weight)) return fail(KHR_EINVAL, "bad min_weight %g", static_cast<double>(min_weight));
@@ -4837,6 +4912,7 @@
 
 int khr_checkpoint_save(khr_ctx* c, void* buffer, uint64_t cap_bytes, uint64_t* n_bytes) {
   if (!c || (!buffer && cap_bytes)) return fail(KHR_EINVAL, "null argument");
+  c->front_gen = 0;
   HIP_TRY(hipSetDevice(c->device));
   int rc = ensureSortKeys(c);
   if (rc) return rc;
@@ -5005,15 +5081,16 @@
 
 static int refreshMeshTotals(khr_ctx* c) {
   if (!c->mesh_stale) return KHR_OK;
-  if (!c->h_totals && hipHostMalloc(reinterpret_cast<void**>(&c->h_totals), sizeof(uint32_t) * (C_COUNT + 2), hipHostMallocDefault) != hipSuccess)
+  if (!c->h_totals && hipHostMalloc(reinterpret_cast<void**>(&c->h_totals), sizeof(uint32_t) * (kFrameCounterSets * C_COUNT + 2), hipHostMallocDefault) != hipSuccess)
     return fail(KHR_ENOMEM, "pinned block for the mesh totals");
   uint32_t* hs = c->h_totals;
   HIP_TRY(hipMemcpyAsync(hs, c->d_mesh_offset + c->m.capacity, sizeof(uint32_t), hipMemcpyDeviceToHost, c->stream));
   HIP_TRY(hipMemcpyAsync(hs + 1, c->d_mesh_nwork, sizeof(uint32_t), hipMemcpyDeviceToHost, c->stream));
-  HIP_TRY(hipMemcpyAsync(hs + 2, c->m.counters, sizeof(uint32_t) * C_COUNT, hipMemcpyDeviceToHost, c->stream));
+  HIP_TRY(hipMemcpyAsync(hs + 2, c->m.counters, sizeof(uint32_t) * kFrameCounterSets * C_COUNT, hipMemcpyDeviceToHost, c->stream));
   HIP_TRY(hipStreamSynchronize(c->stream));
   const uint32_t total = hs[0], nwork = hs[1];
-  c->h_counters.assign(hs + 2, hs + 2 + C_COUNT);
+  c->h_counters.assign(hs + 2, hs + 2 + kFrameCounterSets * C_COUNT);
+  foldFrameCounters(c, c->h_counters);
   c->counters_gen = c->map_gen;
   const uint32_t ovf = c->h_counters[C_MESH_OVERFLOW];
   if (ovf) return fail(KHR_ENOMEM, "mesh needs %u vertices, max_mesh_vertices=%llu", total,
```
